# Yuer867/EMO-Disentanger

Measured on AMD Instinct MI355X. Metric: train tokens/sec (+ AR gen tokens/sec in "gen"), stage2 Performer d512 L12 seq2048, higher is better.
Workload: dtype bf16; 1 GPU; BASELINE configs[1]: stage2 Performer d_model=512 n_layer=12 n_head=8 favor_dims=128 seq=2048, B=64/GPU, dropout 0.1, omega redraw every_forward, fwd+bwd+allreduce+clip+Adam; global_batch=64, seq_len=2048, parallelism=dp1

## Files before the change

emo-disentanger_amd/_lib.py:

```python
import ctypes
import os

import torch

_HERE = os.path.dirname(os.path.abspath(__file__))
LIB_PATH = os.path.join(_HERE, 'libemo_hip.so')

F32, BF16, I64 = 0, 1, 2
ACT_NONE, ACT_RELU, ACT_GELU_NEW, ACT_GELU = 0, 1, 2, 3
MUL_NONE, MUL_NONZERO, MUL_DGELU_NEW, MUL_BITMASK, MUL_DGELU = 0, 1, 2, 3, 4

if not os.path.exists(LIB_PATH):
    raise ImportError('libemo_hip.so not built: run `python -c "import __graft_entry__ as g; g.build()"` '
                      'or `make -C emo-disentanger_amd/csrc` (hipcc --offload-arch=gfx950)')
lib = ctypes.CDLL(LIB_PATH)

c_p, c_i, c_l, c_f, c_u64 = ctypes.c_void_p, ctypes.c_int, ctypes.c_int64, ctypes.c_float, ctypes.c_uint64


class Epilogue(ctypes.Structure):
    _fields_ = [('bias', c_p), ('act', c_i), ('aux_out', c_p), ('mul_aux', c_p), ('mul_mode', c_i), ('mul_scale', c_f),
                ('p_drop', c_f), ('seed', c_u64), ('offset', c_u64), ('residual', c_p),
                ('ln_c1', c_p), ('ln_eps', c_f), ('ln_stats_out', c_p), ('rln_x', c_p), ('rln_stats', c_p), ('rln_gamma', c_p), ('rln_beta', c_p), ('a_rowsum', c_p), ('b_rowsum', c_p),
                ('mask_out', c_p), ('workspace', c_p), ('workspace_bytes', c_l),
                ('lna_gamma', c_p), ('lna_beta', c_p), ('lna_out', c_p), ('lna_mean', c_p), ('lna_rstd', c_p), ('hdiv', c_p), ('hdiv_T', c_l)]


_SIG = {
    'emo_version': (c_i, []),
    'emo_build_flags': (c_i, []),
    'emo_last_error': (ctypes.c_char_p, []),
    'emo_device_cus': (c_i, []),
    'emo_gemm': (c_i, [c_p, c_i, c_l, c_p, c_i, c_l, c_p, c_l, c_l, c_l, c_l, c_i, c_i, c_i, ctypes.POINTER(Epilogue), c_p]),
    'emo_gemm_last_kernel': (c_i, []),
    'emo_epilogue_size': (c_i, []),
    'emo_gemm_workspace_bytes': (c_l, [c_l, c_l, c_l, c_i, c_i]),
    'emo_ffn_fwd_supported': (c_i, [c_i, c_l, c_l, c_l]),
    'emo_ffn_fwd': (c_i, [c_p, c_p, c_p, c_f, c_p, c_p, c_p, c_p, c_p, c_p, c_p, c_p, c_p, c_p, c_l, c_l, c_l, c_i, c_f, c_u64, c_u64, c_u64, c_p]),
    'emo_colsum': (c_i, [c_p, c_i, c_l, c_l, c_l, c_p, c_i, c_p]),
    'emo_embed_fwd': (c_i, [c_p, c_p, c_p, c_p, c_p, c_p, c_i, c_l, c_l, c_l, c_l, c_l, c_l, c_p, c_f, c_f, c_u64, c_u64, c_p]),
    'emo_embed_bwd': (c_i, [c_p, c_p, c_p, c_i, c_p, c_p, c_l, c_l, c_l, c_l, c_l, c_f, c_f, c_u64, c_u64, c_p]),
    'emo_layernorm_fwd': (c_i, [c_p, c_p, c_p, c_p, c_p, c_p, c_i, c_l, c_l, c_f, c_p]),
    'emo_layernorm_bwd': (c_i, [c_p, c_p, c_p, c_p, c_p, c_p, c_p, c_p, c_p, c_p, c_p, c_i, c_l, c_l, c_f, c_u64, c_u64, c_p]),
    'emo_layernorm_bwd_workspace_bytes': (c_l, [c_i, c_l, c_l]),
    'emo_layernorm_bwd_ws': (c_i, [c_p, c_p, c_p, c_p, c_p, c_p, c_p, c_p, c_p, c_p, c_p, c_i, c_l, c_l, c_f, c_u64, c_u64, c_p, c_l, c_p]),
    'emo_dropout_apply': (c_i, [c_p, c_p, c_i, c_l, c_f, c_u64, c_u64, c_p]),
    'emo_favor_attn_workspace_bytes': (c_l, [c_l, c_l, c_l, c_l, c_l]),
    'emo_favor_attn_fwd': (c_i, [c_p, c_p, c_p, c_l, c_p, c_p, c_l, c_p, c_p, c_p, c_i, c_l, c_l, c_l, c_l, c_l, c_f, c_p, c_l, c_p]),
    'emo_favor_attn_bwd': (c_i, [c_p, c_p, c_p, c_l, c_p, c_p, c_p, c_l, c_p, c_p, c_p, c_p, c_l, c_i, c_l, c_l, c_l, c_l, c_l, c_f, c_p, c_l, c_p]),
    'emo_favor_attn_bwd_kstate': (c_i, [c_p, c_p, c_p, c_l, c_p, c_p, c_p, c_l, c_p, c_p, c_p, c_p, c_l, c_i, c_l, c_l, c_l, c_l, c_l, c_f, c_p, c_l, c_i, c_p]),
    'emo_favor_attn_bwd_dn_supported': (c_i, [c_i, c_l, c_l, c_l, c_l, c_l]),
    'emo_favor_attn_bwd_dn': (c_i, [c_p, c_p, c_p, c_l, c_p, c_p, c_p, c_l, c_p, c_p, c_p, c_l, c_i, c_l, c_l, c_l, c_l, c_l, c_f, c_p]),
    'emo_favor_decode_step': (c_i, [c_p, c_p, c_p, c_l, c_p, c_p, c_p, c_p, c_l, c_i, c_l, c_l, c_l, c_l, c_f, c_p]),
    'emo_performer_decode_step_workspace_bytes': (c_l, []),
    'emo_performer_decode_step_supported': (c_i, []),
    'emo_performer_decode_step': (c_i, [c_p, c_l, c_p, c_p, c_p, c_p, c_p, c_f, c_l, c_p, c_p, c_p, c_l, c_p, c_l, c_l, c_l, c_l, c_l, c_p, c_l, c_f, c_f, c_p, c_p]),
    'emo_performer_decode_step_sampled': (c_i, [c_p, c_l, c_p, c_p, c_p, c_p, c_f, c_l, c_p, c_p, c_l, c_p, c_l, c_l, c_l, c_l, c_l, c_l, c_p, c_l, c_f, c_f,
                                                c_f, c_f, c_p, c_p, c_p, c_l, c_l, c_p, c_p]),
    'emo_gpt2_decode_step_supported': (c_i, []),
    'emo_gpt2_decode_step': (c_i, [c_p, c_l, c_p, c_p, c_p, c_p, c_p, c_f, c_l, c_p, c_p, c_l, c_p, c_p, c_l, c_p, c_l, c_l, c_l, c_l, c_p, c_l, c_f, c_p, c_p]),
    'emo_gpt2_decode_step_sampled': (c_i, [c_p, c_l, c_p, c_p, c_p, c_p, c_f, c_l, c_p, c_l, c_p, c_p, c_l, c_p, c_l, c_l, c_l, c_l, c_l, c_p, c_l, c_f,
                                           c_f, c_f, c_p, c_p, c_p, c_l, c_l, c_p, c_p]),
    'emo_favor_draw_omega': (c_i, [c_p, c_p, c_l, c_l, c_l, c_p]),
    'emo_softmax_attn_fwd': (c_i, [c_p, c_p, c_p, c_l, c_p, c_l, c_p, c_i, c_l, c_l, c_l, c_l, c_f, c_u64, c_u64, c_p]),
    'emo_softmax_attn_bwd': (c_i, [c_p, c_p, c_p, c_l, c_p, c_p, c_l, c_p, c_p, c_p, c_p, c_p, c_l, c_i, c_l, c_l, c_l, c_l, c_f, c_u64, c_u64, c_p]),
    'emo_softmax_attn_keep_bytes': (c_l, [c_i, c_l, c_l, c_l, c_l, c_f]),
    'emo_softmax_attn_fwd_keep': (c_i, [c_p, c_p, c_p, c_l, c_p, c_l, c_p, c_i, c_l, c_l, c_l, c_l, c_f, c_u64, c_u64, c_p, c_l, c_p]),
    'emo_softmax_attn_bwd_keep': (c_i, [c_p, c_p, c_p, c_l, c_p, c_p, c_l, c_p, c_p, c_p, c_p, c_p, c_l, c_i, c_l, c_l, c_l, c_l, c_f, c_u64, c_u64, c_p, c_l, c_p]),
    'emo_relpos_attn_fwd': (c_i, [c_p, c_p, c_p, c_l, c_p, c_l, c_l, c_p, c_p, c_p, c_l, c_p, c_p, c_i, c_l, c_l, c_l, c_l, c_f, c_u64, c_u64, c_p]),
    'emo_relpos_attn_bwd_kv': (c_i, [c_p, c_p, c_l, c_p, c_p, c_l, c_p, c_l, c_l, c_p, c_l, c_p, c_p, c_p, c_p, c_p, c_l, c_i, c_l, c_l, c_l, c_l, c_f, c_u64, c_u64, c_p]),
    'emo_relpos_attn_bwd': (c_i, [c_p, c_p, c_p, c_l, c_p, c_l, c_l, c_p, c_p, c_p, c_p, c_l, c_p, c_p, c_p, c_l, c_p, c_l, c_p, c_i, c_l, c_l, c_l, c_l, c_f, c_u64, c_u64, c_p]),
    'emo_relpos_attn_bwd_r': (c_i, [c_p, c_p, c_l, c_p, c_p, c_l, c_p, c_l, c_l, c_p, c_l, c_p, c_p, c_p, c_p, c_l, c_p, c_l, c_i, c_l, c_l, c_l, c_l, c_f, c_u64, c_u64, c_p]),
    'emo_relpos_attn_bwd_r_workspace_bytes': (c_l, [c_l, c_l, c_l, c_l]),
    'emo_relpos_attn_decode': (c_i, [c_p, c_l, c_p, c_p, c_l, c_p, c_l, c_l, c_p, c_p, c_l, c_p, c_l, c_l, c_p, c_p, c_p, c_l, c_i, c_l, c_l, c_l, c_p]),
    'emo_softmax_attn_decode': (c_i, [c_p, c_l, c_p, c_p, c_l, c_p, c_l, c_p, c_p, c_l, c_p, c_l, c_i, c_l, c_l, c_l, c_p]),
    'emo_softmax_attn_decode_layout': (c_i, [c_p, c_l, c_p, c_p, c_l, c_p, c_l, c_p, c_p, c_l, c_p, c_l, c_i, c_l, c_l, c_l, c_i, c_p]),
    'emo_xent_fwd': (c_i, [c_p, c_p, c_l, c_l, c_l, c_p, c_p, c_p]),
    'emo_xent_bwd': (c_i, [c_p, c_p, c_p, c_p, c_p, c_l, c_i, c_l, c_l, c_l, c_p]),
    'emo_argmax': (c_i, [c_p, c_l, c_l, c_p, c_p]),
    'emo_sample_nucleus': (c_i, [c_p, c_l, c_l, c_f, c_f, c_p, c_p, c_p]),
    'emo_sample_nucleus_step': (c_i, [c_p, c_l, c_l, c_f, c_f, c_p, c_p, c_p, c_l, c_l, c_p, c_p]),
    'emo_txl_grammar_step': (c_i, [c_p, c_l, c_l, c_f, c_f, c_f, c_f, c_p, c_l, c_p, c_p, c_p, c_p, c_p, c_l, c_p, c_p, c_p]),
    'emo_acc_grammar_step': (c_i, [c_p, c_l, c_l, c_f, c_f, c_p, c_l, c_p, c_p, c_p, c_p, c_p, c_p, c_p, c_p, c_l, c_l, c_l, c_l, c_p, c_p, c_p, c_p]),
    'emo_accuracy_counts': (c_i, [c_p, c_p, c_p, c_p, c_l, c_l, c_l, c_p, c_p]),
    'emo_sumsq': (c_i, [c_p, c_l, c_p, c_p]),
    'emo_clip_coef': (c_i, [c_p, c_f, c_f, c_p, c_p, c_p]),
    'emo_adam_step': (c_i, [c_p, c_p, c_p, c_p, c_p, c_l, c_f, c_f, c_f, c_f, c_l, c_p, c_p]),
    'emo_cast': (c_i, [c_p, c_i, c_p, c_i, c_l, c_p]),
    'emo_add_bias2': (c_i, [c_p, c_l, c_p, c_p, c_p, c_p, c_i, c_l, c_l, c_p]),
    'emo_transpose_batch': (c_i, [c_p, c_i, c_l, c_p]),
    'emo_stream_wait': (c_i, [c_p, c_p]),
    'emo_comm_bind': (c_i, []),
    'emo_comm_unique_id': (c_i, [c_p]),
    'emo_comm_init': (c_i, [c_p, c_i, c_i]),
    'emo_comm_world': (c_i, []),
    'emo_comm_rank': (c_i, []),
    'emo_comm_allreduce': (c_i, [c_p, c_l, c_i, c_p]),
    'emo_comm_broadcast': (c_i, [c_p, c_l, c_i, c_i, c_p]),
    'emo_comm_destroy': (c_i, []),
}
for _name, (_res, _args) in _SIG.items():
    _fn = getattr(lib, _name)
    _fn.restype, _fn.argtypes = _res, _args
if lib.emo_epilogue_size() != ctypes.sizeof(Epilogue):
    raise ImportError('libemo_hip.so was built with an emo_epilogue_t of %d bytes, this binding has %d: rebuild (python -c "import __graft_entry__ as g; g.build()")'
                      % (lib.emo_epilogue_size(), ctypes.sizeof(Epilogue)))


class EmoError(RuntimeError):
    pass


def check(rc):
    if rc != 0:
        raise EmoError('libemo_hip error %d: %s' % (rc, lib.emo_last_error().decode()))


def dtype_code(t):
    if t == torch.float32:
        return F32
    if t == torch.bfloat16:
        return BF16
    raise EmoError('unsupported dtype %s (float32 / bfloat16 only)' % t)


def ptr(t):
    if t is None:
        return None
    if not t.is_cuda:
        raise EmoError('emo-disentanger_amd ops need GPU tensors (the HIP path has no CPU fallback)')
    return t.data_ptr()


def stream():
    return _raw_stream(_cur_device())


_raw_stream = getattr(torch._C, '_cuda_getCurrentRawStream', None)
_cur_device = getattr(torch._C, '_cuda_getDevice', None)
if _raw_stream is None or _cur_device is None:
    def stream():
        return torch.cuda.current_stream().cuda_stream
```

emo-disentanger_amd/csrc/emo_favor.hip:

```cpp
#include "emo_common.h"

#include "emo_lds_mma.h"

constexpr int FT = 512, FW = FT / 64;
#ifndef FAVOR_CFB
#define FAVOR_CFB 64
#endif
#ifndef FAVOR_CQB
#define FAVOR_CQB 64
#endif
#ifndef FAVOR_CKB
#define FAVOR_CKB 64
#endif
#ifndef FAVOR_PAD16
#define FAVOR_PAD16 0
#endif

template <typename CT, int DH, int C>
__device__ __forceinline__ void row_offsets(const CT* X, int ld, float* off, float c2, float half_ln_f, int tid) {
    constexpr int TPR = FT / C;
    constexpr int EPT = CMax<DH / TPR, 1>::v;
    const int r = tid / TPR, part = tid % TPR;
    float s = 0.f;
    if constexpr (sizeof(CT) == 2 && EPT == 8 && DH % 8 == 0) {
// ... 840 lines not shown
        }
        __syncthreads();
        zero_adiff_pad<CT, MF, MFP, C>(Adiff, LDM, tid);
        if (!(abl & 32)) {
            constexpr int NP = (MF / 16) * (C / 16);
            const int jt = wave % (C / 16);
            Frags<CT, CP> pmf;
            Frags<CT, DHP> vrf;
            pmf.load(PmT, LDC, jt * 16, lane);
            vrf.load(Vr, LDX, jt * 16, lane);
            _Pragma("unroll") for (int pr_i = 0; pr_i < (NP + FW - 1) / FW; ++pr_i) {
            const int pr = wave + FW * pr_i;
            if (NP % FW != 0 && pr >= NP) break;
                const int ft = pr / (C / 16);
                f32x4 aP = {0.f, 0.f, 0.f, 0.f}, aM = {0.f, 0.f, 0.f, 0.f};
                mm16_c<CT, CP>(aP, QfT, LDC, ft * 16, pmf, lane);
                mm16_c<CT, DHP>(aP, RF, LDX, ft * 16, vrf, lane);
                mm16_c<CT, CP>(aM, QfT, LDC, MF + ft * 16, pmf, lane);
                mm16_c<CT, DHP>(aM, RF, LDX, MF + ft * 16, vrf, lane);
                const int j = jt * 16 + (lane & 15), m0 = ft * 16 + (lane >> 4) * 4;
                jac_epilogue<CT, MF>(aP, aM, Kf, LDF, Adiff, LDM, sumA, rr, 1.f, j, m0, lane);
            }
        }
        if (!(abl & 2)) {
            constexpr int NT = (DH / 16) * (C / 16);
            const int jt = wave % (C / 16);
            Frags<CT, CP> amf;
            Frags<CT, F> kff;
            amf.load(AmT, LDC, jt * 16, lane);
            kff.load(Kf, LDF, jt * 16, lane);
            _Pragma("unroll") for (int tile_i = 0; tile_i < (NT + FW - 1) / FW; ++tile_i) {
            const int tile = wave + FW * tile_i;
            if (NT % FW != 0 && tile >= NT) break;
                const int dt = tile / (C / 16);
                f32x4 acc = {0.f, 0.f, 0.f, 0.f};
                mm16_c<CT, CP>(acc, GT, LDC, dt * 16, amf, lane);
                mm16_c<CT, F>(acc, RT, LDF, dt * 16, kff, lane);
                const int j = jt * 16 + (lane & 15), d0 = dt * 16 + (lane >> 4) * 4;
                if (j < valid) Img<CT>::store4(dvb + (t0 + j) * ld_d + d0, acc[0], acc[1], acc[2], acc[3]);
            }
        }
        __syncthreads();
        if (!(abl & 64)) dx_from_adiff<CT, DH, MFP, C>(W, LDM, Adiff, LDM, sumA, kb + t0 * ld, ld, dkb + t0 * ld_d, ld_d, cs, valid, wave, lane);
        }
        if (!(abl & 128)) {
        constexpr bool SH = FW % (F / 16) == 0;
        Frags<CT, CP> qtf;
        if constexpr (SH) qtf.load(QfT, LDC, (wave % (F / 16)) * 16, lane);
#pragma unroll
        for (int i = 0; i < NTS_W; ++i) {
            const int tile = wave + FW * i;
            if (tile < NTS) {
                const int dt = tile / (F / 16), ft = tile % (F / 16);
                if constexpr (SH) mm16_c<CT, CP>(racc[i], GT, LDC, dt * 16, qtf, lane);
                else mm16<CT, CP>(racc[i], GT, LDC, dt * 16, QfT, LDC, ft * 16, lane);
            }
        }
        }
        if constexpr (!SO) {
        __syncthreads();
#pragma unroll
        for (int i = 0; i < NTS_W; ++i) {
            const int tile = wave + FW * i;
            if (tile < NTS) {
                const int dt = tile / (F / 16), ft = tile % (F / 16);
                const int f = ft * 16 + (lane & 15), d0 = dt * 16 + (lane >> 4) * 4;
                Img<CT>::store4(RF + f * LDX + d0, racc[i][0], racc[i][1], racc[i][2], racc[i][3]);
#pragma unroll
                for (int r = 0; r < 4; ++r) RT[(d0 + r) * LDF + f] = from_f32<CT>(racc[i][r]);
            }
        }
        }
        if constexpr (sizeof(CT) == 2 && C == 64 && 4 * F <= FT) {
            const int f = tid >> 2, part = tid & 3;
            if (f < F) {
                float s = dot_contig<CT, 16>(QfT + f * LDC + part * 16, dD + part * 16);
                s += __shfl_xor(s, 1, 64);
                s += __shfl_xor(s, 2, 64);
                if (part == 0) rr[f] += s;
            }
        } else {
            for (int f = tid; f < F; f += FT) {
                float s = 0.f;
                for (int t = 0; t < C; ++t) s += to_f32<CT>(QfT[f * LDC + t]) * dD[t];
                rr[f] += s;
            }
        }
    }
    if constexpr (SO) {
        __syncthreads();
        float* Ro = R_ws + (bh * P + p_seg) * (int64_t)F * DH;
#pragma unroll
        for (int i = 0; i < NTS_W; ++i) {
            const int tile = wave + FW * i;
            if (tile < NTS) {
                const int dt = tile / (F / 16), ft = tile % (F / 16);
                const int f = ft * 16 + (lane & 15), d0 = dt * 16 + (lane >> 4) * 4;
                *(f32x4*)(Ro + f * DH + d0) = racc[i];
            }
        }
        for (int f = tid; f < F; f += FT) r_ws[(bh * P + p_seg) * (int64_t)F + f] = rr[f];
    }
}

template <typename CT>
__global__ __launch_bounds__(256) void favor_decode_kernel(const CT* __restrict__ q, const CT* __restrict__ k, const CT* __restrict__ v, int64_t ld,
                                                           const float* __restrict__ omega, float* __restrict__ state_S, float* __restrict__ state_z,
                                                           CT* __restrict__ out, int64_t ld_out, int64_t H, int dh, int mf, float eps) {
    __shared__ float xq[64], xk[64], xv[64], fq[128], fk[128], num[16][64], dpart[4];
    const int tid = threadIdx.x, F = 2 * mf;
    const int64_t sh = blockIdx.x, s = sh / H, h = sh % H;
    if (tid < dh) {
        xq[tid] = to_f32<CT>(q[s * ld + h * dh + tid]);
        xk[tid] = to_f32<CT>(k[s * ld + h * dh + tid]);
        xv[tid] = to_f32<CT>(v[s * ld + h * dh + tid]);
    }
    __syncthreads();
    const float cs = rsqrtf(sqrtf((float)dh)), half_ln_f = 0.5f * logf((float)F);
    float dn = 0.f;
    if (tid < F) {
        const int m = tid % mf;
        const float sgn = tid < mf ? 1.f : -1.f;
        float uq = 0.f, uk = 0.f, nq = 0.f, nk = 0.f;
        for (int d = 0; d < dh; ++d) {
            const float w = omega[d * mf + m];
            uq += xq[d] * w; uk += xk[d] * w;
            nq += xq[d] * xq[d]; nk += xk[d] * xk[d];
        }
        const float pq = __expf(sgn * cs * uq - (0.5f * cs * cs * nq + half_ln_f));
        const float pk = __expf(sgn * cs * uk - (0.5f * cs * cs * nk + half_ln_f));
        fq[tid] = pq;
        fk[tid] = pk;
        const float z = state_z[sh * F + tid] + pk;
        state_z[sh * F + tid] = z;
        dn = pq * z;
    }
    dn = wave_sum(dn);
    if ((tid & 63) == 0) dpart[tid >> 6] = dn;
    __syncthreads();
    const int G = 256 / dh, d = tid % dh, g = tid / dh;
    float acc = 0.f;
    float* Sb = state_S + sh * F * dh;
    const float vd = xv[d];
    for (int f = g; f < F; f += G) {
        const float sv = Sb[f * dh + d] + fk[f] * vd;
        Sb[f * dh + d] = sv;
        acc += fq[f] * sv;
    }
    num[g][d] = acc;
    __syncthreads();
    if (tid < dh) {
        float a = 0.f;
        for (int p = 0; p < G; ++p) a += num[p][tid];
        out[s * ld_out + h * dh + tid] = from_f32<CT>(a / (dpart[0] + dpart[1] + dpart[2] + dpart[3] + eps));
    }
}

template <typename CT, int DH, int MF>
__global__ __launch_bounds__(256) void favor_decode_fast_kernel(const CT* __restrict__ q, const CT* __restrict__ k, const CT* __restrict__ v, int64_t ld,
                                                                const float* __restrict__ omega, float* __restrict__ state_S,
                                                                float* __restrict__ state_z, CT* __restrict__ out, int64_t ld_out, int64_t H, float eps) {
    constexpr int F = 2 * MF, TPRW = DH / 4, R = 256 / TPRW, NP = (F + R - 1) / R;
    __shared__ float xq[DH], xk[DH], xv[DH], fq[F], fk[F], dpart[4];
    __shared__ f32x4 num[R][TPRW];
    const int tid = threadIdx.x;
    const int64_t sh = blockIdx.x, s = sh / H, h = sh % H;
    const int d4 = (tid % TPRW) * 4, g = tid / TPRW;
    float* Sb = state_S + sh * F * DH;
    f32x4 st[NP];
#pragma unroll
    for (int i = 0; i < NP; ++i) {
        const int f = g + R * i;
        st[i] = f < F ? *(const f32x4*)(Sb + f * DH + d4) : (f32x4){0.f, 0.f, 0.f, 0.f};
    }
    float wcol[DH], zold = 0.f;
    if (tid < F) {
#pragma unroll
        for (int d = 0; d < DH; ++d) wcol[d] = omega[d * MF + (tid % MF)];
        zold = state_z[sh * F + tid];
    }
    if (tid < DH) {
        xq[tid] = to_f32<CT>(q[s * ld + h * DH + tid]);
        xk[tid] = to_f32<CT>(k[s * ld + h * DH + tid]);
        xv[tid] = to_f32<CT>(v[s * ld + h * DH + tid]);
    }
    __syncthreads();
    const float cs = rsqrtf(sqrtf((float)DH)), half_ln_f = 0.5f * logf((float)F);
    float dn = 0.f;
    if (tid < F) {
        const float sgn = tid < MF ? 1.f : -1.f;
        float uq = 0.f, uk = 0.f, nq = 0.f, nk = 0.f;
#pragma unroll
        for (int d = 0; d < DH; ++d) {
            const float w = wcol[d];
            uq += xq[d] * w; uk += xk[d] * w;
            nq += xq[d] * xq[d]; nk += xk[d] * xk[d];
        }
        const float pq = __expf(sgn * cs * uq - (0.5f * cs * cs * nq + half_ln_f));
        const float pk = __expf(sgn * cs * uk - (0.5f * cs * cs * nk + half_ln_f));
        fq[tid] = pq;
        fk[tid] = pk;
        const float z = zold + pk;
        state_z[sh * F + tid] = z;
        dn = pq * z;
    }
    dn = wave_sum(dn);
    if ((tid & 63) == 0) dpart[tid >> 6] = dn;
    __syncthreads();
    const f32x4 vd = {xv[d4], xv[d4 + 1], xv[d4 + 2], xv[d4 + 3]};
    f32x4 acc = {0.f, 0.f, 0.f, 0.f};
#pragma unroll
    for (int i = 0; i < NP; ++i) {
        const int f = g + R * i;
        if (f < F) {
            const f32x4 sv = st[i] + fk[f] * vd;
            *(f32x4*)(Sb + f * DH + d4) = sv;
            acc += fq[f] * sv;
        }
    }
    num[g][tid % TPRW] = acc;
    __syncthreads();
    if (tid < DH) {
        float a = 0.f;
#pragma unroll
        for (int p = 0; p < R; ++p) a += num[p][tid >> 2][tid & 3];
        out[s * ld_out + h * DH + tid] = from_f32<CT>(a / (dpart[0] + dpart[1] + dpart[2] + dpart[3] + eps));
    }
}

__global__ __launch_bounds__(64) void favor_omega_kernel(const float* __restrict__ gauss, float* __restrict__ omega, int dh, int cols, int nblocks) {
    constexpr int LD = 68;
    __shared__ __attribute__((aligned(16))) float Qr[64 * LD];
    __shared__ __attribute__((aligned(16))) float Qc[64 * LD];
    __shared__ __attribute__((aligned(16))) float v[64], cf[64];
    const int lane = threadIdx.x;
    const int layer = blockIdx.x / nblocks, blk = blockIdx.x % nblocks;
    const float* G = gauss + (int64_t)blockIdx.x * dh * dh;
    for (int e = lane; e < 64 * LD; e += 64) { Qr[e] = 0.f; Qc[e] = 0.f; }
    float rn = 0.f;
    if (lane < dh)
        for (int b = 0; b < dh; ++b) { const float g = G[lane * dh + b]; rn += g * g; }
    rn = sqrtf(rn);
    const int start = blk * dh;
    const int ncol = (cols - start) < dh ? (cols - start) : dh;
    __syncthreads();
    for (int j = 0; j < ncol; ++j) {
        float x = lane < dh ? G[lane * dh + j] : 0.f;
        const int j4 = (j + 3) >> 2;
        for (int pass = 0; pass < 2; ++pass) {
            v[lane] = x;
            __syncthreads();
            f32x4 c4 = {0.f, 0.f, 0.f, 0.f};
#pragma unroll 4
            for (int a = 0; a < 16; ++a) c4 += *(const f32x4*)(Qc + lane * LD + 4 * a) * *(const f32x4*)(v + 4 * a);
            cf[lane] = (c4[0] + c4[1]) + (c4[2] + c4[3]);
            __syncthreads();
            f32x4 s4 = {0.f, 0.f, 0.f, 0.f};
            for (int i = 0; i < j4; ++i) s4 += *(const f32x4*)(cf + 4 * i) * *(const f32x4*)(Qr + lane * LD + 4 * i);
            x -= (s4[0] + s4[1]) + (s4[2] + s4[3]);
            __syncthreads();
        }
        const float nrm = sqrtf(wave_sum(lane < dh ? x * x : 0.f));
        const float qv = x / nrm;
        if (lane < dh) { Qr[lane * LD + j] = qv; Qc[j * LD + lane] = qv; }
        const float scale = __shfl(rn, j, 64);
        if (lane < dh) omega[((int64_t)layer * dh + lane) * cols + start + j] = qv * scale;
        __syncthreads();
    }
}

extern "C" int emo_favor_draw_omega(const float* gauss, float* omega, int64_t n_layers, int64_t dh, int64_t n_feat, emo_stream_t stream) {
    EMO_CHECK(gauss && omega && dh > 0 && dh <= 64 && n_feat % 2 == 0, "emo_favor_draw_omega: bad args (d_head <= 64)");
    const int cols = (int)(n_feat / 2);
    const int nblocks = (cols + (int)dh - 1) / (int)dh;
    hipLaunchKernelGGL(favor_omega_kernel, dim3((unsigned)(n_layers * nblocks)), dim3(64), 0, (hipStream_t)stream, gauss, omega, (int)dh, cols, nblocks);
    EMO_LAUNCH_CHECK();
    return EMO_OK;
}

template <typename CT, int DH, int MF, int C> static size_t fwd_lds() {
    typedef FavorDims<CT, DH, MF, C, 0> D;
    if (sizeof(CT) == 2 && C == 64)
        return sizeof(CT) * (size_t)(MF * D::LDX + C * CMax<D::LDX, D::LDC>::v + C * D::LDX + 2 * C * D::LDF + DH * D::LDF) + sizeof(float) * (size_t)(3 * C + D::F);
    return sizeof(CT) * (size_t)(MF * D::LDX + C * CMax<D::LDX, D::LDC>::v + C * D::LDX + DH * D::LDC + 2 * C * D::LDF + D::F * D::LDC + C * D::LDC + DH * D::LDF) +
           sizeof(float) * (size_t)(3 * C + D::F);
}
template <typename CT, int DH, int MF, int C> static size_t dq_lds() {
    typedef FavorDims<CT, DH, MF, C, 1> D;
    return sizeof(CT) * (size_t)(MF * D::LDX + DH * D::LDM + C * D::LDX + C * CMax<D::LDX, D::LDM>::v + C * D::LDX + DH * D::LDC + C * D::LDX +
                                 C * D::LDF + D::F * D::LDC + C * D::LDC + D::F * D::LDX) +
           sizeof(float) * (size_t)(4 * C + D::F);
}
template <typename CT, int DH, int MF, int C> static size_t dkv_lds() {
    typedef FavorDims<CT, DH, MF, C, 2> D;
    return sizeof(CT) * (size_t)(MF * D::LDX + DH * D::LDM + 2 * C * CMax<D::LDX, D::LDC>::v + C * D::LDX + C * CMax<D::LDX, D::LDM>::v + DH * D::LDC +
                                 2 * C * D::LDF + D::F * D::LDC + D::F * D::LDX + DH * D::LDF) +
           sizeof(float) * (size_t)(4 * C + D::F);
}

#define EMO_MAX_LDS (160 * 1024)

int emo_favor_fs_try(int which, int stage, const bf16_t* q, const bf16_t* k, const bf16_t* v, int64_t ld, const float* omega, bf16_t* out, int64_t ld_out,
                     float* den, float* sS, float* sz, const bf16_t* dout, bf16_t* dq, bf16_t* dk, bf16_t* dv, int64_t ld_d, int64_t B, int64_t T, int64_t H,
                     float eps, const float* ws_S, const float* ws_z, int P, int64_t Ts, hipStream_t st);

#define EMO_FAVOR_SEG_ALIGN 64
#define EMO_FAVOR_MAX_SEGMENTS 16
static void favor_segments(int64_t B, int64_t T, int64_t H, int* P_out, int64_t* Ts_out) {
    int64_t want = 1;
    const char* e = getenv("EMO_FAVOR_SEGMENTS");
    if (e && atoi(e) > 0) want = atoi(e);
    else if (B * H < 256) want = (256 + B * H - 1) / (B * H);
    if (want > EMO_FAVOR_MAX_SEGMENTS) want = EMO_FAVOR_MAX_SEGMENTS;
    const int64_t max_p = T / (2 * EMO_FAVOR_SEG_ALIGN);
    if (want > max_p) want = max_p;
    if (want < 1) want = 1;
    int64_t Ts = (T + want - 1) / want;
    Ts = (Ts + EMO_FAVOR_SEG_ALIGN - 1) / EMO_FAVOR_SEG_ALIGN * EMO_FAVOR_SEG_ALIGN;
    if (Ts < EMO_FAVOR_SEG_ALIGN) Ts = EMO_FAVOR_SEG_ALIGN;
    const int64_t P = T > 0 ? (T + Ts - 1) / Ts : 1;
    *P_out = (int)(P < 1 ? 1 : P);
    *Ts_out = Ts;
}

extern "C" int64_t emo_favor_attn_workspace_bytes(int64_t B, int64_t T, int64_t H, int64_t dh, int64_t n_feat) {
    int P; int64_t Ts;
    favor_segments(B, T, H, &P, &Ts);
    if (P <= 1) return 0;
    return B * H * P * (n_feat * dh + n_feat) * (int64_t)sizeof(float);
}

template <typename CT, int DH, int MF, int CF, int CQ, int CK>
static int run_favor(int which, const void* q, const void* k, const void* v, int64_t ld, const float* omega, void* out, int64_t ld_out, float* den,
                     float* sS, float* sz, const void* dout, void* dq, void* dk, void* dv, int64_t ld_d, int64_t B, int64_t T, int64_t H, float eps,
                     void* workspace, int64_t workspace_bytes, hipStream_t st, bool kstate_valid = false) {
    constexpr int F = 2 * MF;
    int P = 1; int64_t Ts = T > 0 ? T : 1;
    if (workspace) {
        favor_segments(B, T, H, &P, &Ts);
        const int64_t need = P > 1 ? B * H * P * (int64_t)(F * DH + F) * (int64_t)sizeof(float) : 0;
        EMO_CHECK(workspace_bytes >= need, "favor attention: workspace %lld B < %lld B (emo_favor_attn_workspace_bytes)", (long long)workspace_bytes,
                  (long long)need);
        EMO_CHECK(((uintptr_t)workspace & 15) == 0, "favor attention: workspace must be 16-B aligned");
    }
    if (P <= 1) { P = 1; Ts = T > 0 ? T : 1; }
    float* wsS = (float*)workspace;
    float* wsz = wsS ? wsS + B * H * P * (int64_t)F * DH : nullptr;
    dim3 grid((unsigned)(B * H * P));
    constexpr bool FS = sizeof(CT) == 2 && DH == 64 && MF == 64;
    auto fs_try = [&](int stage) -> bool {
        if constexpr (FS) {
            if (emo_favor_fs_try(which, stage, (const bf16_t*)q, (const bf16_t*)k, (const bf16_t*)v, ld, omega, (bf16_t*)out, ld_out, den, sS, sz, (const bf16_t*)dout,
                                 (bf16_t*)dq, (bf16_t*)dk, (bf16_t*)dv, ld_d, B, T, H, eps, wsS, wsz, P, Ts, st))
                return true;
        }
        const char* e = getenv("EMO_FAVOR_FS");
        if (e && atoi(e) == 2) emo_set_error("favor attention: EMO_FAVOR_FS=2 but the slice kernels do not cover this call");
        return false;
    };
    auto fs_required_failed = [&]() { const char* e = getenv("EMO_FAVOR_FS"); return e && atoi(e) == 2; };
    if (which == 0) {
        const size_t lds = fwd_lds<CT, DH, MF, CF>();
        EMO_CHECK(lds <= EMO_MAX_LDS, "favor fwd: LDS %zu too large", lds);
        auto kf = favor_fwd_kernel<CT, DH, MF, CF, false>;
        auto ks = favor_fwd_kernel<CT, DH, MF, CF, true>;
        static bool attr = false;
        if (!attr) {
            (void)hipFuncSetAttribute((const void*)kf, hipFuncAttributeMaxDynamicSharedMemorySize, (int)lds);
            (void)hipFuncSetAttribute((const void*)ks, hipFuncAttributeMaxDynamicSharedMemorySize, (int)lds);
            attr = true;
        }
        if (P > 1)
            hipLaunchKernelGGL(ks, grid, dim3(FT), lds, st, (const CT*)q, (const CT*)k, (const CT*)v, ld, omega, (CT*)out, ld_out, den, sS, sz, T, H, eps, wsS,
                               wsz, P, Ts);
        const char* ab = getenv("EMO_FAVOR_ABLATE");
        if (!fs_try(0)) {
            if (fs_required_failed()) return EMO_ERR_INVALID;
            hipLaunchKernelGGL(kf, grid, dim3(FT), lds, st, (const CT*)q, (const CT*)k, (const CT*)v, ld, omega, (CT*)out, ld_out, den, sS, sz, T, H, eps, wsS, wsz,
                               P | (ab ? atoi(ab) << 8 : 0), Ts);
        }
    } else {
        const size_t l0 = fwd_lds<CT, DH, MF, CF>(), l1 = dq_lds<CT, DH, MF, CQ>(), l2 = dkv_lds<CT, DH, MF, CK>();
        EMO_CHECK(l0 <= EMO_MAX_LDS && l1 <= EMO_MAX_LDS && l2 <= EMO_MAX_LDS, "favor bwd: LDS %zu / %zu / %zu too large", l0, l1, l2);
        auto k0 = favor_fwd_kernel<CT, DH, MF, CF, true>;
        auto k1 = favor_bwd_dq_kernel<CT, DH, MF, CQ>;
        auto k2 = favor_bwd_dkv_kernel<CT, DH, MF, CK, false>;
        auto k2s = favor_bwd_dkv_kernel<CT, DH, MF, CK, true>;
        static bool attr = false;
        if (!attr) {
            (void)hipFuncSetAttribute((const void*)k0, hipFuncAttributeMaxDynamicSharedMemorySize, (int)l0);
            (void)hipFuncSetAttribute((const void*)k1, hipFuncAttributeMaxDynamicSharedMemorySize, (int)l1);
            (void)hipFuncSetAttribute((const void*)k2, hipFuncAttributeMaxDynamicSharedMemorySize, (int)l2);
            (void)hipFuncSetAttribute((const void*)k2s, hipFuncAttributeMaxDynamicSharedMemorySize, (int)l2);
            attr = true;
        }
        if (den == nullptr) {
            EMO_CHECK(FS && P == 1, "emo_favor_attn_bwd_dn: needs bf16, d_head 64, 128 features and a single-segment scan (B * H >= 256): emo_favor_attn_bwd_dn_supported()");
            if (!fs_try(1) || !fs_try(2)) {
                emo_set_error("emo_favor_attn_bwd_dn: the slice kernels refused this call (T %% 32, 16-B alignment, EMO_FAVOR_FS / EMO_FAVOR_FS_BWD = 0)");
                return EMO_ERR_UNSUPPORTED;
            }
            EMO_LAUNCH_CHECK();
            return EMO_OK;
        }
        if (P > 1 && !kstate_valid)
            hipLaunchKernelGGL(k0, grid, dim3(FT), l0, st, (const CT*)q, (const CT*)k, (const CT*)v, ld, omega, (CT*)nullptr, ld_out, (float*)nullptr,
                               (float*)nullptr, (float*)nullptr, T, H, eps, wsS, wsz, P, Ts);
        if (!fs_try(1)) {
            if (fs_required_failed()) return EMO_ERR_INVALID;
            hipLaunchKernelGGL(k1, grid, dim3(FT), l1, st, (const CT*)q, (const CT*)k, (const CT*)v, ld, omega, (const CT*)out, (const CT*)dout, ld_out, den,
                               (CT*)dq, ld_d, T, H, (const float*)wsS, (const float*)wsz, P | (getenv("EMO_FAVOR_ABLATE_DQ") ? atoi(getenv("EMO_FAVOR_ABLATE_DQ")) << 8 : 0), Ts);
        }
        if (P > 1)
            hipLaunchKernelGGL(k2s, grid, dim3(FT), l2, st, (const CT*)q, (const CT*)k, (const CT*)v, ld, omega, (const CT*)out, (const CT*)dout, ld_out, den,
                               (CT*)dk, (CT*)dv, ld_d, T, H, wsS, wsz, P, Ts);
        if (!fs_try(2)) {
            if (fs_required_failed()) return EMO_ERR_INVALID;
            hipLaunchKernelGGL(k2, grid, dim3(FT), l2, st, (const CT*)q, (const CT*)k, (const CT*)v, ld, omega, (const CT*)out, (const CT*)dout, ld_out, den,
                               (CT*)dk, (CT*)dv, ld_d, T, H, wsS, wsz, P | (getenv("EMO_FAVOR_ABLATE_DKV") ? atoi(getenv("EMO_FAVOR_ABLATE_DKV")) << 8 : 0), Ts);
        }
    }
    EMO_LAUNCH_CHECK();
    return EMO_OK;
}

static int dispatch_favor(int which, int dtype, int64_t dh, int64_t mf, const void* q, const void* k, const void* v, int64_t ld, const float* omega,
                          void* out, int64_t ld_out, float* den, float* sS, float* sz, const void* dout, void* dq, void* dk, void* dv, int64_t ld_d,
                          int64_t B, int64_t T, int64_t H, float eps, void* ws, int64_t ws_bytes, hipStream_t st, bool kstate_valid = false) {
#define FAVOR_CASE(DHv, MFv, CFb, CQb, CKb, CFf, CQf, CKf)                                                                                   \
    if (dh == DHv && mf == MFv) {                                                                                                            \
        if (dtype == EMO_BF16)                                                                                                               \
            return run_favor<bf16_t, DHv, MFv, CFb, CQb, CKb>(which, q, k, v, ld, omega, out, ld_out, den, sS, sz, dout, dq, dk, dv, ld_d, B, T, H, eps, ws, \
                                                              ws_bytes, st, kstate_valid);                                                   \
        return run_favor<float, DHv, MFv, CFf, CQf, CKf>(which, q, k, v, ld, omega, out, ld_out, den, sS, sz, dout, dq, dk, dv, ld_d, B, T, H, eps, ws,      \
                                                         ws_bytes, st, kstate_valid);                                                        \
    }
    FAVOR_CASE(64, 64, FAVOR_CFB, FAVOR_CQB, FAVOR_CKB, 32, 32, 16)
    FAVOR_CASE(32, 64, 64, 64, 64, 32, 32, 32)
    FAVOR_CASE(32, 32, 64, 64, 64, 32, 32, 32)
    FAVOR_CASE(16, 16, 64, 64, 64, 32, 32, 32)
    FAVOR_CASE(16, 32, 64, 64, 64, 32, 32, 32)
#undef FAVOR_CASE
    emo_set_error("favor attention: unsupported (d_head=%lld, n_feat=%lld); built: (64,128) (32,128) (32,64) (16,32) (16,64)", (long long)dh,
                  (long long)(2 * mf));
    return EMO_ERR_UNSUPPORTED;
}

static int favor_check(const void* q, const void* k, const void* v, int64_t ld, int64_t ld_out, int dtype, int64_t dh, int64_t n_feat) {
    EMO_CHECK(q && k && v, "favor attention: null pointer");
    EMO_CHECK(dtype == EMO_F32 || dtype == EMO_BF16, "favor attention: bad dtype");
    const int64_t ve = dtype == EMO_BF16 ? 8 : 4;
    EMO_CHECK(ld % ve == 0 && ld_out % 4 == 0 && dh % ve == 0, "favor attention: ld/dh must keep rows 16-B aligned");
    EMO_CHECK(((uintptr_t)q & 15) == 0 && ((uintptr_t)k & 15) == 0 && ((uintptr_t)v & 15) == 0, "favor attention: q/k/v must be 16-B aligned");
    EMO_CHECK(n_feat % 2 == 0, "favor attention: n_feat must be even");
    return EMO_OK;
}

extern "C" int emo_favor_attn_fwd(const void* q, const void* k, const void* v, int64_t ld, const float* omega, void* out, int64_t ld_out, float* den,
                                  float* state_S, float* state_z, int dtype, int64_t B, int64_t T, int64_t H, int64_t dh, int64_t n_feat, float eps,
                                  void* workspace, int64_t workspace_bytes, emo_stream_t stream) {
    int rc = favor_check(q, k, v, ld, ld_out, dtype, dh, n_feat);
    if (rc) return rc;
    EMO_CHECK(omega && out && den, "emo_favor_attn_fwd: null pointer");
    EMO_CHECK(((uintptr_t)out & 15) == 0, "emo_favor_attn_fwd: out must be 16-B aligned");
    EMO_CHECK(!(state_S && !state_z), "emo_favor_attn_fwd: state_S without state_z");
    return dispatch_favor(0, dtype, dh, n_feat / 2, q, k, v, ld, omega, out, ld_out, den, state_S, state_z, nullptr, nullptr, nullptr, nullptr, 0, B, T, H,
                          eps, workspace, workspace_bytes, (hipStream_t)stream);
}

extern "C" int emo_favor_attn_bwd_kstate(const void* q, const void* k, const void* v, int64_t ld, const float* omega, const void* out, const void* dout,
                                         int64_t ld_out, const float* den, void* dq, void* dk, void* dv, int64_t ld_d, int dtype, int64_t B, int64_t T, int64_t H,
                                         int64_t dh, int64_t n_feat, float eps, void* workspace, int64_t workspace_bytes, int kstate_valid, emo_stream_t stream) {
    int rc = favor_check(q, k, v, ld, ld_out, dtype, dh, n_feat);
    if (rc) return rc;
    EMO_CHECK(omega && out && dout && den && dq && dk && dv, "emo_favor_attn_bwd: null pointer");
    EMO_CHECK(ld_d % 4 == 0, "emo_favor_attn_bwd: ld_d must be a multiple of 4");
    EMO_CHECK((((uintptr_t)dq | (uintptr_t)dk | (uintptr_t)dv | (uintptr_t)out | (uintptr_t)dout) & 15) == 0, "emo_favor_attn_bwd: pointers must be 16-B aligned");
    return dispatch_favor(1, dtype, dh, n_feat / 2, q, k, v, ld, omega, (void*)out, ld_out, (float*)den, nullptr, nullptr, dout, dq, dk, dv, ld_d, B, T, H,
                          eps, workspace, workspace_bytes, (hipStream_t)stream, kstate_valid != 0 && workspace != nullptr);
}
extern "C" int emo_favor_attn_bwd_dn_supported(int dtype, int64_t B, int64_t T, int64_t H, int64_t dh, int64_t n_feat) {
    if (dtype != EMO_BF16 || dh != 64 || n_feat != 128 || T < 32 || (T % 32) != 0 || B * H <= 0) return 0;
    const char* e = getenv("EMO_FAVOR_FS");
    const char* e2 = getenv("EMO_FAVOR_FS_BWD");
    if ((e && atoi(e) == 0) || (e2 && atoi(e2) == 0)) return 0;
    int P; int64_t Ts;
    favor_segments(B, T, H, &P, &Ts);
    return P <= 1 ? 1 : 0;
}
extern "C" int emo_favor_attn_bwd_dn(const void* q, const void* k, const void* v, int64_t ld, const float* omega, const void* out, const void* dn,
                                     int64_t ld_out, void* dq, void* dk, void* dv, int64_t ld_d, int dtype, int64_t B, int64_t T, int64_t H,
                                     int64_t dh, int64_t n_feat, float eps, emo_stream_t stream) {
    int rc = favor_check(q, k, v, ld, ld_out, dtype, dh, n_feat);
    if (rc) return rc;
    EMO_CHECK(omega && out && dn && dq && dk && dv, "emo_favor_attn_bwd_dn: null pointer");
    EMO_CHECK(emo_favor_attn_bwd_dn_supported(dtype, B, T, H, dh, n_feat), "emo_favor_attn_bwd_dn: problem not in the supported class (emo_favor_attn_bwd_dn_supported)");
    EMO_CHECK(ld_d % 4 == 0, "emo_favor_attn_bwd_dn: ld_d must be a multiple of 4");
    EMO_CHECK((((uintptr_t)dq | (uintptr_t)dk | (uintptr_t)dv | (uintptr_t)out | (uintptr_t)dn) & 15) == 0, "emo_favor_attn_bwd_dn: pointers must be 16-B aligned");
    return dispatch_favor(1, dtype, dh, n_feat / 2, q, k, v, ld, omega, (void*)out, ld_out, (float*)nullptr, nullptr, nullptr, dn, dq, dk, dv, ld_d, B, T, H,
                          eps, nullptr, 0, (hipStream_t)stream, false);
}
extern "C" int emo_favor_attn_bwd(const void* q, const void* k, const void* v, int64_t ld, const float* omega, const void* out, const void* dout,
                                  int64_t ld_out, const float* den, void* dq, void* dk, void* dv, int64_t ld_d, int dtype, int64_t B, int64_t T, int64_t H,
                                  int64_t dh, int64_t n_feat, float eps, void* workspace, int64_t workspace_bytes, emo_stream_t stream) {
    return emo_favor_attn_bwd_kstate(q, k, v, ld, omega, out, dout, ld_out, den, dq, dk, dv, ld_d, dtype, B, T, H, dh, n_feat, eps, workspace, workspace_bytes, 0, stream);
}

extern "C" int emo_favor_decode_step(const void* q, const void* k, const void* v, int64_t ld, const float* omega, float* state_S, float* state_z, void* out,
                                     int64_t ld_out, int dtype, int64_t n_streams, int64_t H, int64_t dh, int64_t n_feat, float eps, emo_stream_t stream) {
    EMO_CHECK(q && k && v && omega && state_S && state_z && out, "emo_favor_decode_step: null pointer");
    EMO_CHECK(dh <= 64 && dh >= 16 && 256 % dh == 0 && n_feat <= 128 && n_feat % 2 == 0, "emo_favor_decode_step: needs 16<=d_head<=64 dividing 256, n_feat<=128");
    dim3 grid((unsigned)(n_streams * H));
    hipStream_t st = (hipStream_t)stream;
#define DECODE_LAUNCH(CTv, DHv, MFv)                                                                                                            \
    hipLaunchKernelGGL((favor_decode_fast_kernel<CTv, DHv, MFv>), grid, dim3(256), 0, st, (const CTv*)q, (const CTv*)k, (const CTv*)v, ld, omega,             \
                       state_S, state_z, (CTv*)out, ld_out, H, eps)
#define DECODE_CASE(DHv, MFv)                                                                                                                   \
    if (dh == DHv && n_feat == 2 * MFv) {                                                                                                       \
        if (dtype == EMO_F32) DECODE_LAUNCH(float, DHv, MFv); else DECODE_LAUNCH(bf16_t, DHv, MFv);                                             \
        EMO_LAUNCH_CHECK();                                                                                                                     \
        return EMO_OK;                                                                                                                          \
    }
    if (getenv("EMO_FAVOR_DECODE_GENERIC") == nullptr && (((uintptr_t)state_S) & 15) == 0) {
        DECODE_CASE(64, 64)
        DECODE_CASE(32, 64)
        DECODE_CASE(32, 32)
        DECODE_CASE(16, 16)
        DECODE_CASE(16, 32)
    }
#undef DECODE_CASE
#undef DECODE_LAUNCH
    if (dtype == EMO_F32)
        hipLaunchKernelGGL(favor_decode_kernel<float>, grid, dim3(256), 0, st, (const float*)q, (const float*)k, (const float*)v, ld, omega, state_S, state_z,
                           (float*)out, ld_out, H, (int)dh, (int)(n_feat / 2), eps);
    else
        hipLaunchKernelGGL(favor_decode_kernel<bf16_t>, grid, dim3(256), 0, st, (const bf16_t*)q, (const bf16_t*)k, (const bf16_t*)v, ld, omega, state_S,
                           state_z, (bf16_t*)out, ld_out, H, (int)dh, (int)(n_feat / 2), eps);
    EMO_LAUNCH_CHECK();
    return EMO_OK;
}
```

emo-disentanger_amd/csrc/emo_favor_fs.hip:

```cpp
#include "emo_common.h"

#include "emo_lds_mma.h"

#ifdef EMO_DIAG
__device__ unsigned long long emo_fs_diag[64];
extern "C" int emo_diag_fetch(unsigned long long* host, int n, int reset) {
    if (hipMemcpyFromSymbol(host, HIP_SYMBOL(emo_fs_diag), sizeof(unsigned long long) * n) != hipSuccess) return -1;
    if (reset) { unsigned long long z[64] = {}; (void)hipMemcpyToSymbol(HIP_SYMBOL(emo_fs_diag), z, sizeof(z)); }
    return 0;
}
#define FSD_BEGIN uint64_t tc_[16] = {}, ts_ = __builtin_readcyclecounter(), tstart_ = ts_;
#define FSD(k) do { const uint64_t tn_ = __builtin_readcyclecounter(); tc_[k] += tn_ - ts_; ts_ = tn_; } while (0)
#define FSD_END(base, nk) do { if (lane == 0) { for (int k_ = 0; k_ < nk; ++k_) atomicAdd(&emo_fs_diag[base + k_], (unsigned long long)tc_[k_]); \
    atomicAdd(&emo_fs_diag[base + 14], (unsigned long long)(__builtin_readcyclecounter() - tstart_)); atomicAdd(&emo_fs_diag[base + 15], 1ull); } } while (0)
#else
#define FSD_BEGIN
#define FSD(k) do {} while (0)
#define FSD_END(base, nk) do {} while (0)
#endif

namespace {
constexpr int FS_NT = 256;
constexpr int FS_C = 32;
constexpr int FS_LDF = 136;
// ... 88 lines not shown
    for (int h = 0; h < 2; ++h) {
        const int row = h * 16 + kc * 4 + (i >> 2), col = col0 + (i & 3) * 4;
        const char* p = tile + row * FS_ROWB + ((((col >> 3)) ^ fs_sw(row)) << 4) + (col & 7) * 2;
        const short4v t = __builtin_amdgcn_ds_read_tr16_b64_v4i16((__attribute__((address_space(3))) short4v*)p);
        const bf16x4 tb = __builtin_bit_cast(bf16x4, t);
        v[h * 4 + 0] = tb[0]; v[h * 4 + 1] = tb[1]; v[h * 4 + 2] = tb[2]; v[h * 4 + 3] = tb[3];
    }
    return v;
}
__device__ __forceinline__ uint32_t fs_lds_addr(const void* p) { return (uint32_t)(uintptr_t)(const __attribute__((address_space(3))) char*)p; }

typedef uint32_t u32x2 __attribute__((ext_vector_type(2)));
__device__ __forceinline__ u32x2 fs_rd8(uint32_t addr, int off) {
    u32x2 r;
    asm volatile("ds_read_b64 %0, %1 offset:%2" : "=v"(r) : "v"(addr), "i"(off));
    return r;
}
__device__ __forceinline__ bf16x8 fs_join(u32x2 lo, u32x2 hi) { return __builtin_bit_cast(bf16x8, (u32x4){lo[0], lo[1], hi[0], hi[1]}); }
template <int N> __device__ __forceinline__ void fs_pin(bf16x8& a, bf16x8& b, bf16x8& c, bf16x8& d) {
    static_assert(N == 0 || N == 4 || N == 8 || N == 12 || N >= 15, "");
    if constexpr (N == 0) asm volatile("s_waitcnt lgkmcnt(0)" : "+v"(a), "+v"(b), "+v"(c), "+v"(d));
    else if constexpr (N == 4) asm volatile("s_waitcnt lgkmcnt(4)" : "+v"(a), "+v"(b), "+v"(c), "+v"(d));
    else if constexpr (N == 8) asm volatile("s_waitcnt lgkmcnt(8)" : "+v"(a), "+v"(b), "+v"(c), "+v"(d));
    else if constexpr (N == 12) asm volatile("s_waitcnt lgkmcnt(12)" : "+v"(a), "+v"(b), "+v"(c), "+v"(d));
    else asm volatile("s_waitcnt lgkmcnt(15)" : "+v"(a), "+v"(b), "+v"(c), "+v"(d));
}
__device__ __forceinline__ uint32_t fs_lp_lane(int g, int c) { return (uint32_t)((c * FS_LDF + 4 * g) * 2); }
__device__ __forceinline__ bf16x8 fs_lp_asm(uint32_t base, int img_off, int row0, int step) {
    const int o = img_off + (row0 * FS_LDF + 32 * step) * 2;
    return fs_join(fs_rd8(base, o), fs_rd8(base, o + 32));
}
__device__ __forceinline__ void fs_rp_lane(int g, int c, uint32_t (&l)[2][2]) {
    const int P = (g >> 1) ^ fs_sw(c);
#pragma unroll
    for (int s_ = 0; s_ < 2; ++s_)
#pragma unroll
        for (int h = 0; h < 2; ++h) l[s_][h] = (uint32_t)(c * FS_ROWB + (g & 1) * 8 + ((P ^ (4 * s_ + 2 * h)) << 4));
}
__device__ __forceinline__ bf16x8 fs_rp_asm(const uint32_t (&rp)[2][2], int tensor, int row0, int s_) {
    const int o = tensor * FS_TILEB + row0 * FS_ROWB;
    return fs_join(fs_rd8(rp[s_][0], o), fs_rd8(rp[s_][1], o));
}

__global__ __launch_bounds__(FS_NT, 2) void favor_fs_fwd_kernel(const bf16_t* __restrict__ q, const bf16_t* __restrict__ k, const bf16_t* __restrict__ v,
                                                                int64_t ld, const float* __restrict__ omega, bf16_t* __restrict__ out, int64_t ld_out,
                                                                float* __restrict__ den_g, float* __restrict__ state_S, float* __restrict__ state_z,
                                                                int64_t Tfull, int64_t H, float eps, const float* __restrict__ S_ws,
                                                                const float* __restrict__ z_ws, int P, int64_t Ts) {
    extern __shared__ __attribute__((aligned(16))) char smem[];
    char* QKr = smem;
    char* Vr = QKr + 3 * 2 * FS_TILEB;
    bf16_t* QFb = (bf16_t*)(Vr + 4 * FS_TILEB);
    bf16_t* KFb = QFb + 2 * FS_C * FS_LDF;
    const int tid = threadIdx.x, lane = tid & 63, g = lane >> 4, c = lane & 15;
    const int w = __builtin_amdgcn_readfirstlane(tid >> 6);
    const int64_t bh = blockIdx.x / P, b = bh / H, h = bh % H;
    const int p_seg = (int)(blockIdx.x % P);
    const int64_t tbeg = (int64_t)p_seg * Ts, T = (tbeg + Ts < Tfull) ? Ts : Tfull - tbeg;
    const bf16_t* qb = q + (b * Tfull + tbeg) * ld + h * 64;
    const bf16_t* kb = k + (b * Tfull + tbeg) * ld + h * 64;
    const bf16_t* vb = v + (b * Tfull + tbeg) * ld + h * 64;
    bf16_t* ob = out + (b * Tfull + tbeg) * ld_out + h * 64;
    float* dg = den_g + bh * Tfull + tbeg;
    const float cs = rsqrtf(sqrtf(64.f));
    const float cs2 = cs * FS_LOG2E, c2h = 0.5f * cs * cs * FS_LOG2E, hl = 0.5f * logf(128.f) * FS_LOG2E;

    bf16x8 wop[2];
#pragma unroll
    for (int s = 0; s < 2; ++s)
#pragma unroll
        for (int e = 0; e < 8; ++e) wop[s][e] = (bf16_t)omega[(32 * s + 8 * g + e) * 64 + 16 * w + c];
    bf16x8 oneop;
#pragma unroll
    for (int e = 0; e < 8; ++e) oneop[e] = (bf16_t)(c == 0 ? 1.f : 0.f);

    f32x4 S[8][2];
#pragma unroll
    for (int ft = 0; ft < 8; ++ft) { S[ft][0] = zero4(); S[ft][1] = zero4(); }
    for (int pp = 0; pp < p_seg; ++pp) {
        const float* Sp = S_ws + (bh * P + pp) * (int64_t)(128 * 64);
        const float* zp = z_ws + (bh * P + pp) * (int64_t)128;
        float ts[8][4];
        f32x4 tz[8];
#pragma unroll
        for (int ft = 0; ft < 8; ++ft) {
#pragma unroll
            for (int r = 0; r < 4; ++r) ts[ft][r] = Sp[(16 * ft + 4 * g + r) * 64 + 16 * w + c];
            tz[ft] = *(const f32x4*)(zp + 16 * ft + 4 * g);
        }
        const float zm = c == 0 ? 1.f : 0.f;
#pragma unroll
        for (int ft = 0; ft < 8; ++ft)
#pragma unroll
            for (int r = 0; r < 4; ++r) { S[ft][0][r] += ts[ft][r]; S[ft][1][r] += zm * tz[ft][r]; }
    }

    const int nch = (int)(T / FS_C);
    const uint32_t qk_lds = __builtin_amdgcn_readfirstlane(fs_lds_addr(QKr)), vr_lds = __builtin_amdgcn_readfirstlane(fs_lds_addr(Vr));
    const int64_t src_off = (int64_t)(8 * w + (lane >> 3)) * ld + (((lane & 7) ^ fs_sw(8 * w + (lane >> 3))) << 3);
    auto issue = [&](int n) {
        const int64_t o = (int64_t)n * FS_C * ld + src_off;
        const uint32_t qk = qk_lds + (n % 3) * 2 * FS_TILEB + w * 1024;
        fs_dma16(qb + o, qk);
        fs_dma16(kb + o, qk + FS_TILEB);
        fs_dma16(vb + o, vr_lds + (n & 3) * FS_TILEB + w * 1024);
    };
    issue(0);
    if (nch > 1) issue(1);
    if (nch > 2) issue(2);
    if (nch > 2) fs_wait<6>(); else if (nch > 1) fs_wait<3>(); else fs_wait<0>();
    __builtin_amdgcn_s_barrier();
    asm volatile("" ::: "memory");
    bf16x4 o_prev[2] = {};
    float d_prev[2] = {0.f, 0.f};
    const uint32_t lpb0 = fs_lds_addr(QFb) + fs_lp_lane(g, c);
    constexpr int KFO = 2 * FS_C * FS_LDF * 2;
#ifdef EMO_DIAG
    uint64_t tc[8] = {}, ts = __builtin_readcyclecounter(), tstart = ts;
#define FS_STAMP(k) do { const uint64_t tn_ = __builtin_readcyclecounter(); tc[k] += tn_ - ts; ts = tn_; } while (0)
#else
#define FS_STAMP(k) do {} while (0)
#endif
    for (int i = 0; i < nch; ++i) {
        const int64_t t0 = (int64_t)i * FS_C;
        bf16_t* QF = QFb + (i & 1) * FS_C * FS_LDF;
        bf16_t* KF = KFb + (i & 1) * FS_C * FS_LDF;
        const char* Xq = QKr + (i % 3) * 2 * FS_TILEB;
        const char* Xk = Xq + FS_TILEB;
        const char* VB = Vr + (i & 3) * FS_TILEB;
        {
            bf16x8 x[4][2];
#pragma unroll
            for (int j = 0; j < 4; ++j)
#pragma unroll
                for (int s = 0; s < 2; ++s) x[j][s] = fs_ring_frag(j < 2 ? Xq : Xk, 16 * (j & 1), s, g, c);
            float p[4][4], n[4][4];
            fs_features<4>(wop, x, cs2, c2h, hl, g, c, p, n);
#pragma unroll
            for (int j = 0; j < 4; ++j) {
                bf16_t* dst = (j < 2 ? QF : KF) + (16 * (j & 1) + c) * FS_LDF + 16 * w + 4 * g;
                st4(dst, p[j][0], p[j][1], p[j][2], p[j][3]);
                st4(dst + 64, n[j][0], n[j][1], n[j][2], n[j][3]);
            }
        }
        FS_STAMP(0);
        if (i + 2 < nch) fs_wait<3>(); else fs_wait<0>();
        FS_STAMP(1);
        if (i > 0) {
#pragma unroll
            for (int tt = 0; tt < 2; ++tt) {
                *(bf16x4*)(ob + (t0 - FS_C + 16 * tt + c) * ld_out + 16 * w + 4 * g) = o_prev[tt];
                if (w == 0 && g == 0) dg[t0 - FS_C + 16 * tt + c] = d_prev[tt];
            }
        }
        fs_barrier();
        FS_STAMP(2);
        if (i + 3 < nch) issue(i + 3);
#ifdef EMO_DIAG
        FS_STAMP(6);
#endif
        bf16x8 qf[2][4], kf[2][4];
        const uint32_t lpb = lpb0 + (i & 1) * (FS_C * FS_LDF * 2);
#pragma unroll
        for (int hs = 0; hs < 2; ++hs)
#pragma unroll
            for (int u = 0; u < 2; ++u)
#pragma unroll
                for (int tt = 0; tt < 2; ++tt) { qf[tt][2 * hs + u] = fs_lp_asm(lpb, 0, 16 * tt, 2 * hs + u); kf[tt][2 * hs + u] = fs_lp_asm(lpb, KFO, 16 * tt, 2 * hs + u); }
        const bf16x8 vop = fs_ring_perm_tr(VB, 16 * w, lane);
        fs_pin<24>(qf[0][0], kf[0][0], qf[1][0], kf[1][0]);
        fs_pin<16>(qf[0][1], kf[0][1], qf[1][1], kf[1][1]);
#ifdef EMO_DIAG
        asm volatile("s_waitcnt lgkmcnt(0)" ::: "memory");
        asm volatile("" :: "v"(vop), "v"(qf[0][0]), "v"(qf[1][3]), "v"(kf[0][0]), "v"(kf[1][3]));
        FS_STAMP(7);
#endif
        f32x4 aa[3][2];
#pragma unroll
        for (int u = 0; u < 2; ++u) {
            aa[0][u] = mma32(kf[0][u], qf[0][u], zero4());
            aa[1][u] = mma32(kf[0][u], qf[1][u], zero4());
            aa[2][u] = mma32(kf[1][u], qf[1][u], zero4());
        }
        fs_pin<8>(qf[0][2], kf[0][2], qf[1][2], kf[1][2]);
        fs_pin<0>(qf[0][3], kf[0][3], qf[1][3], kf[1][3]);
#pragma unroll
        for (int u = 0; u < 2; ++u) {
            aa[0][u] = mma32(kf[0][2 + u], qf[0][2 + u], aa[0][u]);
            aa[1][u] = mma32(kf[0][2 + u], qf[1][2 + u], aa[1][u]);
            aa[2][u] = mma32(kf[1][2 + u], qf[1][2 + u], aa[2][u]);
        }
        f32x4 a00 = aa[0][0] + aa[0][1], a11 = aa[2][0] + aa[2][1];
        const f32x4 a01 = aa[1][0] + aa[1][1];
#pragma unroll
        for (int r = 0; r < 4; ++r) {
            const bool keep = (4 * g + r) <= c;
            a00[r] = keep ? a00[r] : 0.f;
            a11[r] = keep ? a11[r] : 0.f;
        }
        bf16x8 at[2];
        at[0] = pack8(a00, zero4());
        at[1] = pack8(a01, a11);
#ifdef EMO_DIAG
        asm volatile("" :: "v"(at[0]), "v"(at[1]));
#endif
        FS_STAMP(3);
        f32x4 nm[2][2];
#pragma unroll
        for (int tt = 0; tt < 2; ++tt) { nm[tt][0] = mma32(vop, at[tt], zero4()); nm[tt][1] = mma32(oneop, at[tt], zero4()); }
#pragma unroll
        for (int s = 0; s < 4; ++s) {
            const bf16x8 s0 = pack8(S[2 * s][0], S[2 * s + 1][0]), s1 = pack8(S[2 * s][1], S[2 * s + 1][1]);
#pragma unroll
            for (int tt = 0; tt < 2; ++tt) { nm[tt][0] = mma32(s0, qf[tt][s], nm[tt][0]); nm[tt][1] = mma32(s1, qf[tt][s], nm[tt][1]); }
        }
#pragma unroll
        for (int tt = 0; tt < 2; ++tt) {
            const float dn = __shfl(nm[tt][1][0], c, 64) + eps;
            const float inv = 1.f / dn;
            o_prev[tt] = (bf16x4){(bf16_t)(nm[tt][0][0] * inv), (bf16_t)(nm[tt][0][1] * inv), (bf16_t)(nm[tt][0][2] * inv), (bf16_t)(nm[tt][0][3] * inv)};
            d_prev[tt] = dn;
        }
#ifdef EMO_DIAG
        asm volatile("" :: "v"(o_prev[0]), "v"(o_prev[1]));
#endif
        FS_STAMP(4);
#pragma unroll
        for (int ft = 0; ft < 8; ++ft) {
            const bf16x8 kT = load_perm_tr(KF, FS_LDF, 16 * ft, 0, lane);
            S[ft][0] = mma32(kT, vop, S[ft][0]);
            S[ft][1] = mma32(kT, oneop, S[ft][1]);
        }
#ifdef EMO_DIAG
        asm volatile("" :: "v"(S[0][0]), "v"(S[7][1]), "v"(S[3][0]), "v"(S[5][1]));
#endif
        FS_STAMP(5);
    }
#ifdef EMO_DIAG
    if (state_S && lane == 0) {
        unsigned long long* dgp = (unsigned long long*)state_S;
        for (int k_ = 0; k_ < 8; ++k_) atomicAdd(dgp + k_, (unsigned long long)tc[k_]);
        atomicAdd(dgp + 8, (unsigned long long)(__builtin_readcyclecounter() - tstart));
        atomicAdd(dgp + 9, 1ull);
    }
    if (state_S) return;
#endif
    {
        const int64_t t0 = (int64_t)nch * FS_C;
#pragma unroll
        for (int tt = 0; tt < 2; ++tt) {
            *(bf16x4*)(ob + (t0 - FS_C + 16 * tt + c) * ld_out + 16 * w + 4 * g) = o_prev[tt];
            if (w == 0 && g == 0) dg[t0 - FS_C + 16 * tt + c] = d_prev[tt];
        }
    }
    if (state_S && p_seg == P - 1) {
        float* So = state_S + bh * (int64_t)(128 * 64);
#pragma unroll
        for (int ft = 0; ft < 8; ++ft)
#pragma unroll
            for (int r = 0; r < 4; ++r) So[(16 * ft + 4 * g + r) * 64 + 16 * w + c] = S[ft][0][r];
        if (w == 0 && c == 0) {
            float* zo = state_z + bh * 128;
#pragma unroll
            for (int ft = 0; ft < 8; ++ft)
#pragma unroll
                for (int r = 0; r < 4; ++r) zo[16 * ft + 4 * g + r] = S[ft][1][r];
        }
    }
}

constexpr int FS_SLOTB = 5 * FS_TILEB;
template <> __device__ __forceinline__ void fs_wait<12>() { asm volatile("s_waitcnt vmcnt(12)" ::: "memory"); }
__device__ __forceinline__ void fs_dma4(const void* gsrc, uint32_t lds_dst) {
    uint32_t keep;
    asm volatile("s_mov_b32 %0, m0\n\ts_mov_b32 m0, %2\n\ts_nop 0\n\tglobal_load_lds_dword %1, off\n\ts_mov_b32 m0, %0"
                 : "=&s"(keep) : "v"(gsrc), "s"(lds_dst) : "memory");
}
__device__ __forceinline__ f32x4 mma16(bf16x4 a, bf16x4 b, f32x4 c) {
    return __builtin_amdgcn_mfma_f32_16x16x16bf16_1k(__builtin_bit_cast(short4v, a), __builtin_bit_cast(short4v, b), c, 0, 0, 0);
}
__device__ __forceinline__ bf16x8 fs_ring_perm(const char* tile, int row0, int s, int g, int c) {
    const int row = row0 + c, ch = 4 * s + (g >> 1), sw = fs_sw(row);
    const char* base = tile + fs_opaque(row0 * FS_ROWB) + c * FS_ROWB + (g & 1) * 8;
    const bf16x4 lo = *(const bf16x4*)(base + ((ch ^ sw) << 4)), hi = *(const bf16x4*)(base + (((ch + 2) ^ sw) << 4));
    return (bf16x8){lo[0], lo[1], lo[2], lo[3], hi[0], hi[1], hi[2], hi[3]};
}
__device__ __forceinline__ float fs_diag_sum_rows(const f32x4& gm, int g, int c) {
    const int r = c & 3;
    const float d = r == 0 ? gm[0] : r == 1 ? gm[1] : r == 2 ? gm[2] : gm[3];
    return fs_sum_rows(g == (c >> 2) ? d : 0.f);
}
__device__ __forceinline__ bf16x8 fs_scale8(const bf16x8& x, float a) {
    bf16x8 r;
#pragma unroll
    for (int e = 0; e < 8; ++e) r[e] = (bf16_t)((float)x[e] * a);
    return r;
}

template <bool PRE>
__global__ __launch_bounds__(FS_NT, 2) void favor_fs_dq_kernel(const bf16_t* __restrict__ q, const bf16_t* __restrict__ k, const bf16_t* __restrict__ v,
                                                               int64_t ld, const float* __restrict__ omega, const bf16_t* __restrict__ out,
                                                               const bf16_t* __restrict__ dout, int64_t ld_out, const float* __restrict__ den_g,
                                                               bf16_t* __restrict__ dq, int64_t ld_d, int64_t Tfull, int64_t H,
                                                               const float* __restrict__ S_ws, const float* __restrict__ z_ws, int P, int64_t Ts) {
    extern __shared__ __attribute__((aligned(16))) char smem[];
    char* RING = smem;
    char* DEN = RING + 3 * FS_SLOTB;
    char* KP = DEN + 3 * 256;
    char* DU = KP + 4 * 2048;
    float* SA = (float*)(DU + 2 * FS_TILEB);
    const int tid = threadIdx.x, lane = tid & 63, g = lane >> 4, c = lane & 15;
    const int w = __builtin_amdgcn_readfirstlane(tid >> 6);
    const int64_t bh = blockIdx.x / P, b = bh / H, h = bh % H;
    const int p_seg = (int)(blockIdx.x % P);
    const int64_t tbeg = (int64_t)p_seg * Ts, T = (tbeg + Ts < Tfull) ? Ts : Tfull - tbeg;
    const bf16_t* qb = q + (b * Tfull + tbeg) * ld + h * 64;
    const bf16_t* kb = k + (b * Tfull + tbeg) * ld + h * 64;
    const bf16_t* vb = v + (b * Tfull + tbeg) * ld + h * 64;
    const bf16_t* ob = out + (b * Tfull + tbeg) * ld_out + h * 64;
    const bf16_t* gb = dout + (b * Tfull + tbeg) * ld_out + h * 64;
    bf16_t* dqb = dq + (b * Tfull + tbeg) * ld_d + h * 64;
    const float* dnb = den_g + bh * Tfull + tbeg;
    const float cs = rsqrtf(sqrtf(64.f));
    const float cs2 = cs * FS_LOG2E, c2h = 0.5f * cs * cs * FS_LOG2E, hl = 0.5f * logf(128.f) * FS_LOG2E;

    bf16x8 wop[2], wrow[2];
#pragma unroll
    for (int s = 0; s < 2; ++s)
#pragma unroll
        for (int e = 0; e < 8; ++e) {
            wop[s][e] = (bf16_t)omega[(32 * s + 8 * g + e) * 64 + 16 * w + c];
            wrow[s][e] = (bf16_t)omega[(16 * w + c) * 64 + 32 * s + 8 * g + e];
        }
    bf16x8 oneop;
#pragma unroll
    for (int e = 0; e < 8; ++e) oneop[e] = (bf16_t)(c == 0 ? 1.f : 0.f);

    f32x4 ST[5][2];
#pragma unroll
    for (int dl = 0; dl < 5; ++dl) { ST[dl][0] = zero4(); ST[dl][1] = zero4(); }
    for (int pp = 0; pp < p_seg; ++pp) {
        const float* Sp = S_ws + (bh * P + pp) * (int64_t)(128 * 64);
        const float* zp = z_ws + (bh * P + pp) * (int64_t)128;
        f32x4 t4[2][4];
        float tz[2];
#pragma unroll
        for (int ph = 0; ph < 2; ++ph) {
            const int f = 64 * ph + 16 * w + c;
#pragma unroll
            for (int dl = 0; dl < 4; ++dl) t4[ph][dl] = *(const f32x4*)(Sp + f * 64 + 16 * dl + 4 * g);
            tz[ph] = zp[f];
        }
        const float gm = g == 0 ? 1.f : 0.f;
#pragma unroll
        for (int ph = 0; ph < 2; ++ph) {
#pragma unroll
            for (int dl = 0; dl < 4; ++dl) ST[dl][ph] += t4[ph][dl];
            ST[4][ph][0] += gm * tz[ph];
        }
    }

    const int nch = (int)(T / FS_C);
    const uint32_t ring_lds = __builtin_amdgcn_readfirstlane(fs_lds_addr(RING)), den_lds = __builtin_amdgcn_readfirstlane(fs_lds_addr(DEN));
    const int srow = 8 * w + (lane >> 3), spc = ((lane & 7) ^ fs_sw(srow)) << 3;
    const int64_t so_qkv = (int64_t)srow * ld + spc, so_o = (int64_t)srow * ld_out + spc;
    auto issue_part = [&](int n, int part) {
        if (n >= nch) return;
        const int64_t t0n = (int64_t)n * FS_C;
        const uint32_t dst = ring_lds + (n % 3) * FS_SLOTB + w * 1024;
        if (part == 0) fs_dma16(qb + t0n * ld + so_qkv, dst);
        else if (part == 1) fs_dma16(kb + t0n * ld + so_qkv, dst + FS_TILEB);
        else if (part == 2) fs_dma16(vb + t0n * ld + so_qkv, dst + 2 * FS_TILEB);
        else if (part == 3) fs_dma16(gb + t0n * ld_out + so_o, dst + 3 * FS_TILEB);
        else if (part == 4) fs_dma16(ob + t0n * ld_out + so_o, dst + 4 * FS_TILEB);
        else if (!PRE) {
            const int64_t tl = t0n + lane;
            fs_dma4(dnb + (tl < T ? tl : T - 1), den_lds + (n % 3) * 256);
        }
    };
    constexpr int NPART = PRE ? 5 : 6;
    auto issue = [&](int n) {
#pragma unroll
        for (int part = 0; part < 6; ++part) issue_part(n, part);
    };
    issue(0);
    if (nch > 1) issue(1);
    if (nch > 2) issue(2);
    if (nch > 2) fs_wait<2 * NPART>(); else if (nch > 1) fs_wait<NPART>(); else fs_wait<0>();
    __builtin_amdgcn_s_barrier();
    asm volatile("" ::: "memory");
    char* KPw = KP + w * 2048;
    bf16x4 o_prev[2] = {};
    uint32_t rpl[2][2];
    fs_rp_lane(g, c, rpl);
    FSD_BEGIN
    for (int i = 0; i < nch; ++i) {
        const int64_t t0 = (int64_t)i * FS_C;
        const char* Xq = RING + (i % 3) * FS_SLOTB;
        const char* Xk = Xq + FS_TILEB;
        const char* Xv = Xq + 2 * FS_TILEB;
        const char* Xg = Xq + 3 * FS_TILEB;
        const char* Xo = Xq + 4 * FS_TILEB;
        const float* dens = (const float*)(DEN + (i % 3) * 256);
        char* DUb = DU + (i & 1) * FS_TILEB;
        float* SAb = SA + (i & 1) * 128;
        bf16x8 dfr[2][2], ofr[2][2], vr[2][2];
        f32x4 gmm[2];
        uint32_t rp[2][2];
        {
            const uint32_t slot = ring_lds + (i % 3) * FS_SLOTB;
#pragma unroll
            for (int s_ = 0; s_ < 2; ++s_)
#pragma unroll
                for (int h_ = 0; h_ < 2; ++h_) rp[s_][h_] = rpl[s_][h_] + slot;
        }
#pragma unroll
        for (int tt = 0; tt < 2; ++tt)
#pragma unroll
            for (int s_ = 0; s_ < 2; ++s_) { dfr[tt][s_] = fs_rp_asm(rp, 3, 16 * tt, s_); ofr[tt][s_] = fs_rp_asm(rp, 4, 16 * tt, s_); }
#pragma unroll
        for (int jt = 0; jt < 2; ++jt)
#pragma unroll
            for (int s_ = 0; s_ < 2; ++s_) vr[jt][s_] = fs_rp_asm(rp, 2, 16 * jt, s_);
        fs_pin<16>(dfr[0][0], ofr[0][0], dfr[0][1], ofr[0][1]);
        fs_pin<8>(dfr[1][0], ofr[1][0], dfr[1][1], ofr[1][1]);
#pragma unroll
        for (int tt = 0; tt < 2; ++tt) {
            gmm[tt] = mma32(ofr[tt][0], dfr[tt][0], zero4());
            gmm[tt] = mma32(ofr[tt][1], dfr[tt][1], gmm[tt]);
        }
        float pq[2][4], nq[2][4];
        {
            bf16x8 x[4][2];
#pragma unroll
            for (int j = 0; j < 4; ++j)
#pragma unroll
                for (int s = 0; s < 2; ++s) x[j][s] = fs_ring_frag(j < 2 ? Xq : Xk, 16 * (j & 1), s, g, c);
            float p[4][4], n[4][4];
            fs_features<4>(wop, x, cs2, c2h, hl, g, c, p, n);
#pragma unroll
            for (int tt = 0; tt < 2; ++tt)
#pragma unroll
                for (int r = 0; r < 4; ++r) { pq[tt][r] = p[tt][r]; nq[tt][r] = n[tt][r]; }
#pragma unroll
            for (int jt = 0; jt < 2; ++jt) {
                const int row = 16 * jt + c, sw = ((row >> 2) & 1) << 2;
                st4((bf16_t*)(KPw + row * 64 + ((g ^ sw) << 3)), p[2 + jt][0], p[2 + jt][1], p[2 + jt][2], p[2 + jt][3]);
                st4((bf16_t*)(KPw + row * 64 + (((4 + g) ^ sw) << 3)), n[2 + jt][0], n[2 + jt][1], n[2 + jt][2], n[2 + jt][3]);
            }
        }
        FSD(0);
        if (i > 0) issue_part(i + 2, 3);
        bf16x4 xown[2];
#pragma unroll
        for (int tt = 0; tt < 2; ++tt) {
            const int row = 16 * tt + c;
            xown[tt] = *(const bf16x4*)(Xq + row * FS_ROWB + (((2 * w + (g >> 1)) ^ fs_sw(row)) << 4) + (g & 1) * 8);
        }
        bf16x8 gop[2][2];
        float dD[2];
#pragma unroll
        for (int tt = 0; tt < 2; ++tt) {
            if constexpr (PRE) {
                dD[tt] = -fs_diag_sum_rows(gmm[tt], g, c);
                gop[tt][0] = dfr[tt][0];
                gop[tt][1] = dfr[tt][1];
            } else {
                const float inv = 1.f / dens[16 * tt + c];
                dD[tt] = -fs_diag_sum_rows(gmm[tt], g, c) * inv;
                gop[tt][0] = fs_scale8(dfr[tt][0], inv);
                gop[tt][1] = fs_scale8(dfr[tt][1], inv);
            }
        }
        FSD(1);
        if (i > 0) issue_part(i + 2, 4);
        bf16x8 at[2];
        {
            fs_pin<0>(vr[0][0], vr[0][1], vr[1][0], vr[1][1]);
            f32x4 p00 = mma32(vr[0][0], gop[0][0], zero4()), p01 = mma32(vr[0][0], gop[1][0], zero4()), p11 = mma32(vr[1][0], gop[1][0], zero4());
            p00 = mma32(vr[0][1], gop[0][1], p00);
            p01 = mma32(vr[0][1], gop[1][1], p01);
            p11 = mma32(vr[1][1], gop[1][1], p11);
#pragma unroll
            for (int r = 0; r < 4; ++r) {
                const bool keep = (4 * g + r) <= c;
                p00[r] = keep ? p00[r] + dD[0] : 0.f;
                p01[r] = p01[r] + dD[1];
                p11[r] = keep ? p11[r] + dD[1] : 0.f;
            }
            at[0] = pack8(p00, zero4());
            at[1] = pack8(p01, p11);
        }
        FSD(2);
        if (i > 0) issue_part(i + 2, 5);
        bf16x8 kfT[2];
#pragma unroll
        for (int ph = 0; ph < 2; ++ph) {
#pragma unroll
            for (int hh = 0; hh < 2; ++hh) {
                const int row = hh * 16 + g * 4 + (c >> 2), pc = (4 * ph + (c & 3)) ^ (((row >> 2) & 1) << 2);
                const short4v t = __builtin_amdgcn_ds_read_tr16_b64_v4i16((__attribute__((address_space(3))) short4v*)(KPw + row * 64 + (pc << 3)));
                const bf16x4 tb = __builtin_bit_cast(bf16x4, t);
                kfT[ph][hh * 4 + 0] = tb[0]; kfT[ph][hh * 4 + 1] = tb[1]; kfT[ph][hh * 4 + 2] = tb[2]; kfT[ph][hh * 4 + 3] = tb[3];
            }
        }
        {
            bf16x8 sop[2][2];
            bf16x4 szop[2];
#pragma unroll
            for (int ph = 0; ph < 2; ++ph) {
                sop[ph][0] = pack8(ST[0][ph], ST[1][ph]);
                sop[ph][1] = pack8(ST[2][ph], ST[3][ph]);
                szop[ph] = (bf16x4){(bf16_t)ST[4][ph][0], (bf16_t)ST[4][ph][1], (bf16_t)ST[4][ph][2], (bf16_t)ST[4][ph][3]};
            }
            f32x4 dph[2][2];
#pragma unroll
            for (int tt = 0; tt < 2; ++tt) {
                const bf16x4 ddop = {(bf16_t)(g == 0 ? dD[tt] : 0.f), (bf16_t)0.f, (bf16_t)0.f, (bf16_t)0.f};
#pragma unroll
                for (int ph = 0; ph < 2; ++ph) {
                    f32x4 a = mma32(kfT[ph], at[tt], zero4());
                    a = mma32(sop[ph][0], gop[tt][0], a);
                    a = mma32(sop[ph][1], gop[tt][1], a);
                    dph[ph][tt] = mma16(szop[ph], ddop, a);
                }
            }
#pragma unroll
            for (int tt = 0; tt < 2; ++tt) {
                float du[4], sa = 0.f;
#pragma unroll
                for (int r = 0; r < 4; ++r) {
                    const float ap = dph[0][tt][r] * pq[tt][r], am = dph[1][tt][r] * nq[tt][r];
                    du[r] = ap - am;
                    sa += ap + am;
                }
                sa = fs_sum_rows(sa);
                const int row = 16 * tt + c;
                st4((bf16_t*)(DUb + row * FS_ROWB + (((2 * w + (g >> 1)) ^ fs_sw(row)) << 4) + (g & 1) * 8), du[0], du[1], du[2], du[3]);
                if (g == 0) SAb[w * 32 + row] = sa;
            }
        }
        FSD(3);
#pragma unroll
        for (int dl = 0; dl < 4; ++dl) {
            const bf16x8 vT = fs_ring_perm_tr(Xv, 16 * dl, lane);
            ST[dl][0] = mma32(vT, kfT[0], ST[dl][0]);
            ST[dl][1] = mma32(vT, kfT[1], ST[dl][1]);
        }
        ST[4][0] = mma32(oneop, kfT[0], ST[4][0]);
        ST[4][1] = mma32(oneop, kfT[1], ST[4][1]);
        FSD(4);
        if (i + 2 < nch) fs_wait<NPART>(); else fs_wait<0>();
        FSD(5);
        if (i > 0) {
#pragma unroll
            for (int tt = 0; tt < 2; ++tt) *(bf16x4*)(dqb + (t0 - FS_C + 16 * tt + c) * ld_d + 16 * w + 4 * g) = o_prev[tt];
        }
        fs_barrier();
        FSD(6);
        issue_part(i + 3, 0);
        FSD(7);
#pragma unroll
        for (int tt = 0; tt < 2; ++tt) {
            issue_part(i + 3, 1 + tt);
            const int row = 16 * tt + c;
            const bf16x8 u0 = *(const bf16x8*)(DUb + row * FS_ROWB + (((g) ^ fs_sw(row)) << 4)), u1 = *(const bf16x8*)(DUb + row * FS_ROWB + (((4 + g) ^ fs_sw(row)) << 4));
            f32x4 dx = mma32(wrow[0], u0, zero4());
            dx = mma32(wrow[1], u1, dx);
            const float sa = (SAb[row] + SAb[32 + row]) + (SAb[64 + row] + SAb[96 + row]);
            float o[4];
#pragma unroll
            for (int r = 0; r < 4; ++r) o[r] = cs * (dx[r] - cs * (float)xown[tt][r] * sa);
            o_prev[tt] = (bf16x4){(bf16_t)o[0], (bf16_t)o[1], (bf16_t)o[2], (bf16_t)o[3]};
        }
        FSD(8);
    }
    FSD_END(16, 9);
    {
        const int64_t t0 = (int64_t)nch * FS_C;
#pragma unroll
        for (int tt = 0; tt < 2; ++tt) *(bf16x4*)(dqb + (t0 - FS_C + 16 * tt + c) * ld_d + 16 * w + 4 * g) = o_prev[tt];
    }
}

template <bool PRE>
__global__ __launch_bounds__(FS_NT, 2) void favor_fs_dkv_kernel(const bf16_t* __restrict__ q, const bf16_t* __restrict__ k, const bf16_t* __restrict__ v,
                                                                int64_t ld, const float* __restrict__ omega, const bf16_t* __restrict__ out,
                                                                const bf16_t* __restrict__ dout, int64_t ld_out, const float* __restrict__ den_g,
                                                                bf16_t* __restrict__ dk, bf16_t* __restrict__ dv, int64_t ld_d, int64_t Tfull, int64_t H,
                                                                const float* __restrict__ R_ws, const float* __restrict__ r_ws, int P, int64_t Ts) {
    extern __shared__ __attribute__((aligned(16))) char smem[];
    char* RING = smem;
    char* DEN = RING + 2 * FS_SLOTB;
    bf16_t* QF = (bf16_t*)(DEN + 2 * 256);
    bf16_t* KF = QF + FS_C * FS_LDF;
    char* DU = (char*)(KF + FS_C * FS_LDF);
    float* SA = (float*)(DU + FS_TILEB);
    float* PV = SA + 128;
    const int tid = threadIdx.x, lane = tid & 63, g = lane >> 4, c = lane & 15;
    const int w = __builtin_amdgcn_readfirstlane(tid >> 6);
    const int64_t bh = blockIdx.x / P, b = bh / H, h = bh % H;
    const int p_seg = (int)(blockIdx.x % P);
    const int64_t tbeg = (int64_t)p_seg * Ts, T = (tbeg + Ts < Tfull) ? Ts : Tfull - tbeg;
    const bf16_t* qb = q + (b * Tfull + tbeg) * ld + h * 64;
    const bf16_t* kb = k + (b * Tfull + tbeg) * ld + h * 64;
    const bf16_t* vb = v + (b * Tfull + tbeg) * ld + h * 64;
    const bf16_t* ob = out + (b * Tfull + tbeg) * ld_out + h * 64;
    const bf16_t* gb = dout + (b * Tfull + tbeg) * ld_out + h * 64;
    bf16_t* dkb = dk + (b * Tfull + tbeg) * ld_d + h * 64;
    bf16_t* dvb = dv + (b * Tfull + tbeg) * ld_d + h * 64;
    const float* dnb = den_g + bh * Tfull + tbeg;
    const float cs = rsqrtf(sqrtf(64.f));
    const float cs2 = cs * FS_LOG2E, c2h = 0.5f * cs * cs * FS_LOG2E, hl = 0.5f * logf(128.f) * FS_LOG2E;

    bf16x8 wop[2], wrow[2];
#pragma unroll
    for (int s = 0; s < 2; ++s)
#pragma unroll
        for (int e = 0; e < 8; ++e) {
            wop[s][e] = (bf16_t)omega[(32 * s + 8 * g + e) * 64 + 16 * w + c];
            wrow[s][e] = (bf16_t)omega[(16 * w + c) * 64 + 32 * s + 8 * g + e];
        }
    const bf16x4 onecol = {(bf16_t)(g == 0 ? 1.f : 0.f), (bf16_t)0.f, (bf16_t)0.f, (bf16_t)0.f};

    f32x4 RT[5][2], RD[8];
#pragma unroll
    for (int dl = 0; dl < 5; ++dl) { RT[dl][0] = zero4(); RT[dl][1] = zero4(); }
#pragma unroll
    for (int ft = 0; ft < 8; ++ft) RD[ft] = zero4();
    for (int pp = p_seg + 1; pp < P; ++pp) {
        const float* Rp = R_ws + (bh * P + pp) * (int64_t)(128 * 64);
        const float* rp = r_ws + (bh * P + pp) * (int64_t)128;
        f32x4 t4[2][4];
        float tr[2], td[8][4];
#pragma unroll
        for (int ph = 0; ph < 2; ++ph) {
            const int f = 64 * ph + 16 * w + c;
#pragma unroll
            for (int dl = 0; dl < 4; ++dl) t4[ph][dl] = *(const f32x4*)(Rp + f * 64 + 16 * dl + 4 * g);
            tr[ph] = rp[f];
        }
#pragma unroll
        for (int ft = 0; ft < 8; ++ft)
#pragma unroll
            for (int r = 0; r < 4; ++r) td[ft][r] = Rp[(16 * ft + 4 * g + r) * 64 + 16 * w + c];
        const float gm = g == 0 ? 1.f : 0.f;
#pragma unroll
        for (int ph = 0; ph < 2; ++ph) {
#pragma unroll
            for (int dl = 0; dl < 4; ++dl) RT[dl][ph] += t4[ph][dl];
            RT[4][ph][0] += gm * tr[ph];
        }
#pragma unroll
        for (int ft = 0; ft < 8; ++ft)
#pragma unroll
            for (int r = 0; r < 4; ++r) RD[ft][r] += td[ft][r];
    }

    const int nch = (int)(T / FS_C);
    const uint32_t ring_lds = __builtin_amdgcn_readfirstlane(fs_lds_addr(RING)), den_lds = __builtin_amdgcn_readfirstlane(fs_lds_addr(DEN));
    const int srow = 8 * w + (lane >> 3), spc = ((lane & 7) ^ fs_sw(srow)) << 3;
    const int64_t so_qkv = (int64_t)srow * ld + spc, so_o = (int64_t)srow * ld_out + spc;
    auto issue = [&](int n) {
        const int64_t t0n = (int64_t)(nch - 1 - n) * FS_C;
        const uint32_t dst = ring_lds + (n & 1) * FS_SLOTB + w * 1024;
        fs_dma16(qb + t0n * ld + so_qkv, dst);
        fs_dma16(kb + t0n * ld + so_qkv, dst + FS_TILEB);
        fs_dma16(vb + t0n * ld + so_qkv, dst + 2 * FS_TILEB);
        fs_dma16(gb + t0n * ld_out + so_o, dst + 3 * FS_TILEB);
        fs_dma16(ob + t0n * ld_out + so_o, dst + 4 * FS_TILEB);
        if constexpr (!PRE) {
            const int64_t tl = t0n + lane;
            fs_dma4(dnb + (tl < T ? tl : T - 1), den_lds + (n & 1) * 256);
        }
    };
    issue(0);
    if (nch > 1) issue(1);
    if (nch > 1) fs_wait<PRE ? 5 : 6>(); else fs_wait<0>();
    __builtin_amdgcn_s_barrier();
    asm volatile("" ::: "memory");
    float* PVw = PV + w * 96;
    bf16x4 dk_prev[2] = {}, dv_prev[2] = {};
    uint32_t rpl[2][2];
    fs_rp_lane(g, c, rpl);
    const uint32_t lpb = fs_lds_addr(QF) + fs_lp_lane(g, c);
    constexpr int KFO = FS_C * FS_LDF * 2;
    FSD_BEGIN
    for (int n = 0; n < nch; ++n) {
        const int64_t t0 = (int64_t)(nch - 1 - n) * FS_C;
        const char* Xq = RING + (n & 1) * FS_SLOTB;
        const char* Xk = Xq + FS_TILEB;
        const char* Xv = Xq + 2 * FS_TILEB;
        const char* Xg = Xq + 3 * FS_TILEB;
        const char* Xo = Xq + 4 * FS_TILEB;
        const float* dens = (const float*)(DEN + (n & 1) * 256);
        {
            bf16x8 x[4][2];
#pragma unroll
            for (int j = 0; j < 4; ++j)
#pragma unroll
                for (int s = 0; s < 2; ++s) x[j][s] = fs_ring_frag(j < 2 ? Xq : Xk, 16 * (j & 1), s, g, c);
            float p[4][4], nn[4][4];
            fs_features<4>(wop, x, cs2, c2h, hl, g, c, p, nn);
#pragma unroll
            for (int j = 0; j < 4; ++j) {
                bf16_t* dst = (j < 2 ? QF : KF) + (16 * (j & 1) + c) * FS_LDF + 16 * w + 4 * g;
                st4(dst, p[j][0], p[j][1], p[j][2], p[j][3]);
                st4(dst + 64, nn[j][0], nn[j][1], nn[j][2], nn[j][3]);
            }
        }
        FSD(0);
        bf16x4 xown[2];
#pragma unroll
        for (int jt = 0; jt < 2; ++jt) {
            const int row = 16 * jt + c;
            xown[jt] = *(const bf16x4*)(Xk + row * FS_ROWB + (((2 * w + (g >> 1)) ^ fs_sw(row)) << 4) + (g & 1) * 8);
        }
        bf16x8 gA[2][2];
        uint32_t rp[2][2];
        {
            const uint32_t slot = ring_lds + (n & 1) * FS_SLOTB;
#pragma unroll
            for (int s_ = 0; s_ < 2; ++s_)
#pragma unroll
                for (int h_ = 0; h_ < 2; ++h_) rp[s_][h_] = rpl[s_][h_] + slot;
        }
        bf16x8 dfr[2][2], ofr[2][2], vB1[2][2];
#pragma unroll
        for (int tt = 0; tt < 2; ++tt)
#pragma unroll
            for (int s_ = 0; s_ < 2; ++s_) { dfr[tt][s_] = fs_rp_asm(rp, 3, 16 * tt, s_); ofr[tt][s_] = fs_rp_asm(rp, 4, 16 * tt, s_); }
#pragma unroll
        for (int jt = 0; jt < 2; ++jt)
#pragma unroll
            for (int s_ = 0; s_ < 2; ++s_) vB1[jt][s_] = fs_rp_asm(rp, 2, 16 * jt, s_);
        fs_pin<16>(dfr[0][0], ofr[0][0], dfr[0][1], ofr[0][1]);
        fs_pin<8>(dfr[1][0], ofr[1][0], dfr[1][1], ofr[1][1]);
#pragma unroll
        for (int tt = 0; tt < 2; ++tt) {
            const bf16x8 d0 = dfr[tt][0], d1 = dfr[tt][1];
            const bf16x8 o0 = ofr[tt][0], o1 = ofr[tt][1];
            f32x4 gm = mma32(o0, d0, zero4());
            gm = mma32(o1, d1, gm);
            const float dot = fs_diag_sum_rows(gm, g, c);
            if constexpr (PRE) {
                if (g == 0) PVw[16 * tt + c] = -dot;
                gA[tt][0] = d0;
                gA[tt][1] = d1;
            } else {
                const float inv = 1.f / dens[16 * tt + c];
                if (g == 0) { PVw[16 * tt + c] = -dot * inv; PVw[32 + 16 * tt + c] = -dot; PVw[64 + 16 * tt + c] = inv; }
                gA[tt][0] = fs_scale8(d0, inv);
                gA[tt][1] = fs_scale8(d1, inv);
            }
        }
        FSD(1);
        bf16x8 pb[2];
        {
            fs_pin<0>(vB1[0][0], vB1[0][1], vB1[1][0], vB1[1][1]);
            bf16x8 (&vB)[2][2] = vB1;
            f32x4 p00 = mma32(gA[0][0], vB[0][0], zero4()), p10 = mma32(gA[1][0], vB[0][0], zero4()), p11 = mma32(gA[1][0], vB[1][0], zero4());
            p00 = mma32(gA[0][1], vB[0][1], p00);
            p10 = mma32(gA[1][1], vB[0][1], p10);
            p11 = mma32(gA[1][1], vB[1][1], p11);
            const f32x4 dd0 = *(const f32x4*)(PVw + 4 * g), dd1 = *(const f32x4*)(PVw + 16 + 4 * g);
#pragma unroll
            for (int r = 0; r < 4; ++r) {
                const bool keep = (4 * g + r) >= c;
                p00[r] = keep ? p00[r] + dd0[r] : 0.f;
                p10[r] = p10[r] + dd1[r];
                p11[r] = keep ? p11[r] + dd1[r] : 0.f;
            }
            pb[0] = pack8(p00, p10);
            pb[1] = pack8(zero4(), p11);
        }
        FSD(2);
        fs_barrier();
        FSD(3);
        bf16x8 ab[2];
        {
            bf16x8 qfA[2][4], kfB[2][4];
#pragma unroll
            for (int hs = 0; hs < 2; ++hs)
#pragma unroll
                for (int u = 0; u < 2; ++u)
#pragma unroll
                    for (int tt = 0; tt < 2; ++tt) { qfA[tt][2 * hs + u] = fs_lp_asm(lpb, 0, 16 * tt, 2 * hs + u); kfB[tt][2 * hs + u] = fs_lp_asm(lpb, KFO, 16 * tt, 2 * hs + u); }
            fs_pin<24>(qfA[0][0], kfB[0][0], qfA[1][0], kfB[1][0]);
            fs_pin<16>(qfA[0][1], kfB[0][1], qfA[1][1], kfB[1][1]);
            f32x4 aa[3][2];
#pragma unroll
            for (int u = 0; u < 2; ++u) {
                aa[0][u] = mma32(qfA[0][u], kfB[0][u], zero4());
                aa[1][u] = mma32(qfA[1][u], kfB[0][u], zero4());
                aa[2][u] = mma32(qfA[1][u], kfB[1][u], zero4());
            }
            fs_pin<8>(qfA[0][2], kfB[0][2], qfA[1][2], kfB[1][2]);
            fs_pin<0>(qfA[0][3], kfB[0][3], qfA[1][3], kfB[1][3]);
#pragma unroll
            for (int u = 0; u < 2; ++u) {
                aa[0][u] = mma32(qfA[0][2 + u], kfB[0][2 + u], aa[0][u]);
                aa[1][u] = mma32(qfA[1][2 + u], kfB[0][2 + u], aa[1][u]);
                aa[2][u] = mma32(qfA[1][2 + u], kfB[1][2 + u], aa[2][u]);
            }
            f32x4 a00 = aa[0][0] + aa[0][1], a11 = aa[2][0] + aa[2][1];
            const f32x4 a10 = aa[1][0] + aa[1][1];
#pragma unroll
            for (int r = 0; r < 4; ++r) {
                const bool keep = (4 * g + r) >= c;
                a00[r] = keep ? a00[r] : 0.f;
                a11[r] = keep ? a11[r] : 0.f;
            }
            ab[0] = pack8(a00, a10);
            ab[1] = pack8(zero4(), a11);
        }
        FSD(4);
        f32x4 iv0 = {}, iv1 = {};
        if constexpr (!PRE) { iv0 = *(const f32x4*)(PVw + 64 + 4 * g); iv1 = *(const f32x4*)(PVw + 64 + 16 + 4 * g); }
        auto scale_t = [&](const bf16x8& x) {
            if constexpr (PRE) return x;
            else return (bf16x8){(bf16_t)((float)x[0] * iv0[0]), (bf16_t)((float)x[1] * iv0[1]), (bf16_t)((float)x[2] * iv0[2]), (bf16_t)((float)x[3] * iv0[3]),
                            (bf16_t)((float)x[4] * iv1[0]), (bf16_t)((float)x[5] * iv1[1]), (bf16_t)((float)x[6] * iv1[2]), (bf16_t)((float)x[7] * iv1[3])};
        };
        bf16x8 qfTs[2];
        {
            bf16x8 qfT[2], vB[2][2];
#pragma unroll
            for (int ph = 0; ph < 2; ++ph) {
                qfT[ph] = load_perm_tr(QF, FS_LDF, 16 * w + 64 * ph, 0, lane);
                qfTs[ph] = scale_t(qfT[ph]);
            }
#pragma unroll
            for (int jt = 0; jt < 2; ++jt)
#pragma unroll
                for (int s = 0; s < 2; ++s) vB[jt][s] = fs_rp_asm(rp, 2, 16 * jt, s);
            f32x4 dph[2][2];
#pragma unroll
            for (int jt = 0; jt < 2; ++jt)
#pragma unroll
                for (int ph = 0; ph < 2; ++ph) dph[jt][ph] = mma32(qfT[ph], pb[jt], zero4());
            fs_pin<0>(vB[0][0], vB[0][1], vB[1][0], vB[1][1]);
#pragma unroll
            for (int s = 0; s < 2; ++s)
#pragma unroll
                for (int ph = 0; ph < 2; ++ph) {
                    const bf16x8 rop = pack8(RT[2 * s][ph], RT[2 * s + 1][ph]);
#pragma unroll
                    for (int jt = 0; jt < 2; ++jt) dph[jt][ph] = mma32(rop, vB[jt][s], dph[jt][ph]);
                }
#pragma unroll
            for (int ph = 0; ph < 2; ++ph) {
                const bf16x4 rzop = {(bf16_t)RT[4][ph][0], (bf16_t)RT[4][ph][1], (bf16_t)RT[4][ph][2], (bf16_t)RT[4][ph][3]};
#pragma unroll
                for (int jt = 0; jt < 2; ++jt) dph[jt][ph] = mma16(rzop, onecol, dph[jt][ph]);
            }
#pragma unroll
            for (int jt = 0; jt < 2; ++jt) {
                const int row = 16 * jt + c;
                const bf16x4 kp = *(const bf16x4*)(KF + row * FS_LDF + 16 * w + 4 * g), kn = *(const bf16x4*)(KF + row * FS_LDF + 64 + 16 * w + 4 * g);
                float du[4], sa = 0.f;
#pragma unroll
                for (int r = 0; r < 4; ++r) {
                    const float ap = dph[jt][0][r] * (float)kp[r], am = dph[jt][1][r] * (float)kn[r];
                    du[r] = ap - am;
                    sa += ap + am;
                }
                sa = fs_sum_rows(sa);
                st4((bf16_t*)(DU + row * FS_ROWB + (((2 * w + (g >> 1)) ^ fs_sw(row)) << 4) + (g & 1) * 8), du[0], du[1], du[2], du[3]);
                if (g == 0) SA[w * 32 + row] = sa;
            }
        }
        FSD(5);
        const bf16x8 gTs = scale_t(fs_ring_perm_tr(Xg, 16 * w, lane));
        {
            bf16x8 kp0[4], kp1[4];
#pragma unroll
            for (int s = 0; s < 4; ++s) { kp0[s] = fs_lp_asm(lpb, KFO, 0, s); kp1[s] = fs_lp_asm(lpb, KFO, 16, s); }
            f32x4 a0 = mma32(gTs, ab[0], zero4()), a1 = mma32(gTs, ab[1], zero4());
            fs_pin<8>(kp0[0], kp1[0], kp0[1], kp1[1]);
#pragma unroll
            for (int s = 0; s < 4; ++s) {
                if (s == 2) fs_pin<0>(kp0[2], kp1[2], kp0[3], kp1[3]);
                const bf16x8 rd = pack8(RD[2 * s], RD[2 * s + 1]);
                a0 = mma32(rd, kp0[s], a0);
                a1 = mma32(rd, kp1[s], a1);
            }
            dv_prev[0] = (bf16x4){(bf16_t)a0[0], (bf16_t)a0[1], (bf16_t)a0[2], (bf16_t)a0[3]};
            dv_prev[1] = (bf16x4){(bf16_t)a1[0], (bf16_t)a1[1], (bf16_t)a1[2], (bf16_t)a1[3]};
        }
        FSD(6);
#pragma unroll
        for (int dl = 0; dl < 4; ++dl) {
            const bf16x8 gT = fs_ring_perm_tr(Xg, 16 * dl, lane);
            RT[dl][0] = mma32(gT, qfTs[0], RT[dl][0]);
            RT[dl][1] = mma32(gT, qfTs[1], RT[dl][1]);
        }
        {
            const f32x4 nd0 = *(const f32x4*)(PVw + (PRE ? 0 : 32) + 4 * g), nd1 = *(const f32x4*)(PVw + (PRE ? 0 : 32) + 16 + 4 * g);
            bf16x8 ndop = pack8(nd0, nd1);
#pragma unroll
            for (int e = 0; e < 8; ++e) ndop[e] = c == 0 ? ndop[e] : (bf16_t)0.f;
            RT[4][0] = mma32(ndop, qfTs[0], RT[4][0]);
            RT[4][1] = mma32(ndop, qfTs[1], RT[4][1]);
        }
#pragma unroll
        for (int ft = 0; ft < 8; ++ft) RD[ft] = mma32(load_perm_tr(QF, FS_LDF, 16 * ft, 0, lane), gTs, RD[ft]);
        FSD(7);
        fs_wait<0>();
        FSD(8);
        if (n > 0) {
            const int64_t tp = t0 + FS_C;
#pragma unroll
            for (int jt = 0; jt < 2; ++jt) *(bf16x4*)(dkb + (tp + 16 * jt + c) * ld_d + 16 * w + 4 * g) = dk_prev[jt];
        }
#pragma unroll
        for (int jt = 0; jt < 2; ++jt) *(bf16x4*)(dvb + (t0 + 16 * jt + c) * ld_d + 16 * w + 4 * g) = dv_prev[jt];
        fs_barrier();
        FSD(9);
        if (n + 2 < nch) issue(n + 2);
        FSD(10);
#pragma unroll
        for (int jt = 0; jt < 2; ++jt) {
            const int row = 16 * jt + c;
            const bf16x8 u0 = *(const bf16x8*)(DU + row * FS_ROWB + ((g ^ fs_sw(row)) << 4)), u1 = *(const bf16x8*)(DU + row * FS_ROWB + (((4 + g) ^ fs_sw(row)) << 4));
            f32x4 dx = mma32(wrow[0], u0, zero4());
            dx = mma32(wrow[1], u1, dx);
            const float sa = (SA[row] + SA[32 + row]) + (SA[64 + row] + SA[96 + row]);
            dk_prev[jt] = (bf16x4){(bf16_t)(cs * (dx[0] - cs * (float)xown[jt][0] * sa)), (bf16_t)(cs * (dx[1] - cs * (float)xown[jt][1] * sa)),
                                   (bf16_t)(cs * (dx[2] - cs * (float)xown[jt][2] * sa)), (bf16_t)(cs * (dx[3] - cs * (float)xown[jt][3] * sa))};
        }
        FSD(11);
    }
    FSD_END(32, 12);
#pragma unroll
    for (int jt = 0; jt < 2; ++jt) *(bf16x4*)(dkb + (16 * jt + c) * ld_d + 16 * w + 4 * g) = dk_prev[jt];
}
}

int emo_favor_fs_try(int which, int stage, const bf16_t* q, const bf16_t* k, const bf16_t* v, int64_t ld, const float* omega, bf16_t* out, int64_t ld_out,
                     float* den, float* sS, float* sz, const bf16_t* dout, bf16_t* dq, bf16_t* dk, bf16_t* dv, int64_t ld_d, int64_t B, int64_t T, int64_t H,
                     float eps, const float* ws_S, const float* ws_z, int P, int64_t Ts, hipStream_t st) {
    const char* e = getenv("EMO_FAVOR_FS");
    if (e && atoi(e) == 0) return 0;
    if (T < FS_C || (T % FS_C) != 0 || B * H <= 0 || P < 1 || (P > 1 && (Ts % FS_C) != 0)) return 0;
    if ((ld & 7) || (ld_out & 7) || (ld_d & 3)) return 0;
    if ((((uintptr_t)q | (uintptr_t)k | (uintptr_t)v | (uintptr_t)out | (uintptr_t)dout) & 15) || (((uintptr_t)dq | (uintptr_t)dk | (uintptr_t)dv) & 15)) return 0;
    if (P == 1) Ts = T;
    dim3 grid((unsigned)(B * H * P));
    if (which == 0) {
        const size_t lds = (size_t)(3 * 2 + 4) * FS_TILEB + sizeof(bf16_t) * (size_t)(4 * FS_C * FS_LDF);
        static bool attr = false;
        if (!attr) { (void)hipFuncSetAttribute((const void*)favor_fs_fwd_kernel, hipFuncAttributeMaxDynamicSharedMemorySize, (int)lds); attr = true; }
        hipLaunchKernelGGL(favor_fs_fwd_kernel, grid, dim3(FS_NT), lds, st, q, k, v, ld, omega, out, ld_out, den, sS, sz, T, H, eps, ws_S, ws_z, P, Ts);
        return 1;
    }
    const char* e2 = getenv("EMO_FAVOR_FS_BWD");
    if (e2 && atoi(e2) == 0) return 0;
    const bool pre = den == nullptr;
    if (stage == 0 || stage == 1) {
        const size_t lds = (size_t)3 * FS_SLOTB + 3 * 256 + 4 * 2048 + 2 * FS_TILEB + 2 * 4 * 32 * sizeof(float);
        static bool attr = false;
        if (!attr) {
            (void)hipFuncSetAttribute((const void*)favor_fs_dq_kernel<false>, hipFuncAttributeMaxDynamicSharedMemorySize, (int)lds);
            (void)hipFuncSetAttribute((const void*)favor_fs_dq_kernel<true>, hipFuncAttributeMaxDynamicSharedMemorySize, (int)lds);
            attr = true;
        }
        if (pre)
            hipLaunchKernelGGL(favor_fs_dq_kernel<true>, grid, dim3(FS_NT), lds, st, q, k, v, ld, omega, (const bf16_t*)out, dout, ld_out, (const float*)nullptr, dq, ld_d, T, H,
                               ws_S, ws_z, P, Ts);
        else
            hipLaunchKernelGGL(favor_fs_dq_kernel<false>, grid, dim3(FS_NT), lds, st, q, k, v, ld, omega, (const bf16_t*)out, dout, ld_out, (const float*)den, dq, ld_d, T, H,
                               ws_S, ws_z, P, Ts);
    }
    if (stage == 0 || stage == 2) {
        const size_t lds2 = (size_t)2 * FS_SLOTB + 2 * 256 + sizeof(bf16_t) * (size_t)(2 * FS_C * FS_LDF) + FS_TILEB + sizeof(float) * (128 + 4 * 96);
        static bool attr2 = false;
        if (!attr2) {
            (void)hipFuncSetAttribute((const void*)favor_fs_dkv_kernel<false>, hipFuncAttributeMaxDynamicSharedMemorySize, (int)lds2);
            (void)hipFuncSetAttribute((const void*)favor_fs_dkv_kernel<true>, hipFuncAttributeMaxDynamicSharedMemorySize, (int)lds2);
            attr2 = true;
        }
        if (pre)
            hipLaunchKernelGGL(favor_fs_dkv_kernel<true>, grid, dim3(FS_NT), lds2, st, q, k, v, ld, omega, (const bf16_t*)out, dout, ld_out, (const float*)nullptr, dk, dv, ld_d, T, H,
                               ws_S, ws_z, P, Ts);
        else
            hipLaunchKernelGGL(favor_fs_dkv_kernel<false>, grid, dim3(FS_NT), lds2, st, q, k, v, ld, omega, (const bf16_t*)out, dout, ld_out, (const float*)den, dk, dv, ld_d, T, H,
                               ws_S, ws_z, P, Ts);
    }
    return 1;
}
```

emo-disentanger_amd/ops.py:

```python
import ctypes

import os

import torch

from . import _lib
from ._lib import (ACT_GELU, ACT_GELU_NEW, ACT_NONE, ACT_RELU, BF16, F32, MUL_BITMASK, MUL_DGELU, MUL_DGELU_NEW, MUL_NONE, MUL_NONZERO, Epilogue, check,
                   dtype_code, lib, ptr, stream)

__all__ = ['gemm', 'colsum', 'embed_fwd', 'embed_bwd', 'layernorm_fwd', 'layernorm_bwd', 'dropout_apply', 'favor_attn_fwd',
           'favor_attn_bwd', 'favor_decode_step', 'performer_decode_step', 'performer_decode_step_sampled', 'favor_draw_omega', 'softmax_attn_fwd', 'softmax_attn_bwd', 'softmax_attn_decode', 'relpos_attn_fwd', 'relpos_attn_bwd', 'relpos_attn_decode', 'xent_fwd',
           'xent_bwd', 'argmax', 'sample_nucleus', 'sample_nucleus_step', 'txl_grammar_step', 'acc_grammar_step', 'accuracy_counts', 'sumsq', 'clip_coef', 'adam_step', 'cast', 'add_bias2',
           'ACT_NONE', 'ACT_RELU', 'ACT_GELU_NEW', 'ACT_GELU', 'MUL_NONE', 'MUL_NONZERO', 'MUL_DGELU_NEW', 'MUL_DGELU', 'MUL_BITMASK', 'gemm_bitmask_ok', 'gemm_lna_ok', 'bitmask_rows', 'favor_bwd_dn_ok', 'ffn_fwd', 'ffn_fwd_ok']


def _c(t):
    if t is None:
        return None
    assert t.dtype == torch.int64
    return t if t.is_contiguous() else t.contiguous()


def _rows(t):
    assert t.dim() == 2 and t.stride(1) == 1, 'need a 2-D tensor with unit column stride'
    return t.stride(0)


_stream = stream
_ws_cache = {}
_ws_need = {}
GEMM_TIMING = None
KERNEL_TIMING = None


class _timed:

    def __init__(self, kind, flops, nbytes):
        self.kind, self.flops, self.nbytes = kind, flops, nbytes

    def __enter__(self):
        if KERNEL_TIMING is not None:
            self.e0, self.e1 = torch.cuda.Event(enable_timing=True), torch.cuda.Event(enable_timing=True)
            self.e0.record()
        return self

    def __exit__(self, *a):
        if KERNEL_TIMING is not None:
            self.e1.record()
            KERNEL_TIMING.setdefault(self.kind, []).append((self.e0, self.e1, self.flops, self.nbytes))
        return False


def _workspace(kind, device, need, st=None):
    if need == 0:
        return None, 0
    key = (kind, device, st if st is not None else stream())
    buf = _ws_cache.get(key)
    if buf is None or buf.numel() < need:
        if buf is not None and st is not None and st != stream():
            buf.record_stream(torch.cuda.ExternalStream(st))
        buf = torch.empty(need, device=device, dtype=torch.uint8)
        _ws_cache[key] = buf
    return buf, need


def gemm(A, B, *, a_trans=False, b_trans=False, out=None, out_dtype=None, accumulate=False, bias=None, act=ACT_NONE,
         aux_out=None, mul_aux=None, mul_mode=MUL_NONE, mul_scale=1.0, p_drop=0.0, seed=0, offset=0, residual=None,
         ln_c1=None, ln_eps=1e-5, ln_stats_out=None, rln=None, a_rowsum=None, b_rowsum=None, mask_out=None, stream=None, lna=None, lna_out=None, hdiv=None):
    st = stream if stream is not None else _stream()
    K, M = (A.shape if a_trans else A.shape[::-1])
    Kb, N = (B.shape if b_trans else B.shape[::-1])
    assert K == Kb, 'inner dims differ: %s vs %s' % (tuple(A.shape), tuple(B.shape))
    assert A.dtype == B.dtype
    if out is None:
        out = torch.empty(M, N, device=A.device, dtype=out_dtype or A.dtype)
    ws, ws_bytes = None, 0
    plain = bias is None and residual is None and aux_out is None and mul_aux is None and act == ACT_NONE and p_drop == 0.0
    if (out.dtype == torch.float32 and plain) or (out.dtype == torch.bfloat16 and not accumulate and M > 32):
        wkey = (M, N, K, A.dtype, out.dtype)
        need = _ws_need.get(wkey)
        if need is None:
            need = _ws_need[wkey] = lib.emo_gemm_workspace_bytes(M, N, K, dtype_code(A.dtype), dtype_code(out.dtype))
        ws, ws_bytes = _workspace('gemm', A.device, need, st)
    rx, rstats, rgamma, rbeta = rln if rln is not None else (None, None, None, None)
    assert rx is None or (rx.dtype == out.dtype and _rows(rx) == _rows(out))
    ln_out = ln_mean = ln_rstd = None
    if lna is not None:
        assert gemm_lna_ok(M, N, K, A.dtype) and not a_trans and not b_trans and lna[0].dtype == torch.float32 and lna[1].dtype == torch.float32
        assert _rows(A) % 8 == 0 and _rows(B) % 8 == 0 and _rows(out) % 8 == 0 and (A.data_ptr() | B.data_ptr() | out.data_ptr()) % 16 == 0, \
            'lna=: the A-stationary kernel needs 16-B aligned operands and row strides that are multiples of 8 elements'
        ln_eps = lna[2]
        if lna_out is not None:
            ln_out, ln_mean, ln_rstd = lna_out
            assert ln_out.shape == (M, K) and ln_out.is_contiguous() and ln_out.dtype == A.dtype and ln_mean.numel() == M and ln_rstd.numel() == M
        else:
            ln_out = torch.empty(M, K, device=A.device, dtype=A.dtype)
            ln_mean = torch.empty(M, device=A.device, dtype=torch.float32)
            ln_rstd = torch.empty(M, device=A.device, dtype=torch.float32)
    epi = Epilogue(ptr(bias), act, ptr(aux_out), ptr(mul_aux), mul_mode, mul_scale, p_drop, seed, offset, ptr(residual),
                   ptr(ln_c1), ln_eps, ptr(ln_stats_out), ptr(rx), ptr(rstats), ptr(rgamma), ptr(rbeta), ptr(a_rowsum), ptr(b_rowsum), ptr(mask_out), ptr(ws), ws_bytes,
                   ptr(lna[0]) if lna is not None else None, ptr(lna[1]) if lna is not None else None, ptr(ln_out), ptr(ln_mean), ptr(ln_rstd),
                   ptr(hdiv[0]) if hdiv is not None else None, int(hdiv[1]) if hdiv is not None else 0)
    if hdiv is not None:
        assert hdiv[0].dtype == torch.float32 and hdiv[0].is_contiguous() and hdiv[0].numel() == M * (N // 64) and plain and mask_out is None and lna is None
    if not plain or mask_out is not None:
        for t in (aux_out, residual) + (() if mul_mode == MUL_BITMASK else (mul_aux,)):
            assert t is None or (t.dtype == out.dtype and _rows(t) == _rows(out))
        for t in (mask_out,) + ((mul_aux,) if mul_mode == MUL_BITMASK else ()):
            assert t is None or (t.dtype == torch.uint8 and t.is_contiguous() and t.shape == (M, N // 8) and gemm_bitmask_ok(M, N, K, A.dtype, out.dtype))
        assert bias is None or bias.dtype == torch.float32
    if GEMM_TIMING is not None:
        e0, e1 = torch.cuda.Event(enable_timing=True), torch.cuda.Event(enable_timing=True)
        tstream = torch.cuda.ExternalStream(st) if stream is not None else torch.cuda.current_stream()
        e0.record(tstream)
    check(lib.emo_gemm(ptr(A), int(a_trans), _rows(A), ptr(B), int(b_trans), _rows(B), ptr(out), _rows(out), M, N, K,
                       dtype_code(A.dtype), dtype_code(out.dtype), int(accumulate), ctypes.byref(epi), st))
    if GEMM_TIMING is not None:
        e1.record(tstream)
        kind = ('T' if a_trans else 'N') + ('N' if b_trans else 'T')
        fam = lib.emo_gemm_last_kernel() & 15
        if fam == 4:
            kind += '/K>1024'
        elif fam == 2:
            tag = [t for t, on in (('relu', act == ACT_RELU), ('gelu', act == ACT_GELU_NEW), ('drop', p_drop > 0), ('res', residual is not None),
                                   ('bits', mul_mode == MUL_BITMASK), ('mul', mul_aux is not None and mul_mode != MUL_BITMASK), ('mask', mask_out is not None),
                                   ('hdiv', hdiv is not None)) if on]
            kind += '/K=512/' + ('+'.join(tag) if tag else 'plain')
        elif fam == 3:
            kind += '/rs' if (a_rowsum is not None or b_rowsum is not None) else '/plain'
        elif kind == 'TN':
            kind += '/128'
        elif fam == 1:
            kind += '/skinny'
        GEMM_TIMING.append((kind, e0, e1, 2.0 * M * N * K,
                            (M * K + N * K) * A.element_size() + M * N * out.element_size(), (M, N, K)))
    if lna is not None:
        return out, ln_out, ln_mean, ln_rstd
    return out


ASTAT_MIN_ROWS = int(os.environ.get('EMO_ASTAT_MIN_ROWS', 0)) or 128 * 32


def gemm_bitmask_ok(M, N, K, in_dtype, out_dtype):
    return in_dtype == torch.bfloat16 and out_dtype == torch.bfloat16 and K == 512 and M % 128 == 0 and M >= ASTAT_MIN_ROWS and N % 64 == 0 and 64 <= N <= 2048


def gemm_lna_ok(M, N, K, in_dtype):
    return (in_dtype == torch.bfloat16 and K == 512 and M % 128 == 0 and M >= ASTAT_MIN_ROWS and N % 64 == 0 and 64 <= N <= 2048
            and os.environ.get('EMO_GEMM_NO_ASTAT') is None and os.environ.get('EMO_LN_IN_GEMM', '1') != '0'
            and os.environ.get('EMO_GEMM_SAFE_TR', '0') in ('', '0'))


def bitmask_rows(mask, M, N):
    t = mask.reshape(M // 32, N // 64, 4, 16, 2, 2)
    return t.permute(0, 4, 3, 1, 5, 2).reshape(M, N // 8)


def ffn_fwd_ok(M, d_model, d_ff, dtype):
    return dtype == torch.bfloat16 and bool(lib.emo_ffn_fwd_supported(dtype_code(dtype), M, d_model, d_ff))


def ffn_fwd(x1, gamma, beta, W1, b1, W2, b2, p_drop=0.0, seed=0, offset_f=0, offset_y=0, eps=1e-5):
    M, D = x1.shape
    Hd = W1.shape[0]
    assert x1.is_contiguous() and W1.is_contiguous() and W2.is_contiguous() and W1.shape == (Hd, D) and W2.shape == (D, Hd)
    assert b1.dtype == torch.float32 and b2.dtype == torch.float32 and gamma.dtype == torch.float32 and beta.dtype == torch.float32
    dev, dt = x1.device, x1.dtype
    h1, x2 = torch.empty_like(x1), torch.empty_like(x1)
    f = torch.empty(M, Hd, device=dev, dtype=dt)
    mean, rstd = torch.empty(M, device=dev, dtype=torch.float32), torch.empty(M, device=dev, dtype=torch.float32)
    mask = torch.empty(M, Hd // 8, device=dev, dtype=torch.uint8)
    flops, nbytes = 2.0 * 2.0 * M * D * Hd, (3.0 * M * D + M * Hd) * x1.element_size() + M * Hd / 8
    with _timed('ffn_fused_fwd', flops, nbytes):
        check(lib.emo_ffn_fwd(ptr(x1), ptr(gamma), ptr(beta), eps, ptr(W1), ptr(b1), ptr(W2), ptr(b2), ptr(h1), ptr(mean), ptr(rstd), ptr(f), ptr(mask),
                              ptr(x2), M, D, Hd, dtype_code(dt), p_drop, seed, offset_f, offset_y, stream()))
    return f, h1, mean, rstd, mask, x2


def colsum(X, out=None, accumulate=False):
    M, N = X.shape
    if out is None:
        out = torch.empty(N, device=X.device, dtype=torch.float32)
    check(lib.emo_colsum(ptr(X), dtype_code(X.dtype), M, N, _rows(X), ptr(out), int(accumulate), stream()))
    return out


def embed_fwd(tok, seg, E, S, pe, dtype, scale, pos0=0, p_drop=0.0, seed=0, offset=0, pos_ids=None):
    B, T = tok.shape
    D = E.shape[1]
    out = torch.empty(B, T, D, device=tok.device, dtype=dtype)
    assert pe.is_contiguous() and pe.shape[-1] == D and pe.numel() >= (pos0 + T) * D
    tok, seg, pos_ids = _c(tok), _c(seg), _c(pos_ids)
    check(lib.emo_embed_fwd(ptr(tok), ptr(seg), ptr(E), ptr(S), ptr(pe), ptr(out),
                            dtype_code(dtype), B, T, D, E.shape[0], 0 if S is None else S.shape[0], pos0, ptr(pos_ids), scale, p_drop, seed,
                            offset, stream()))
    return out


def embed_bwd(tok, seg, dout, dE, dS, scale, p_drop=0.0, seed=0, offset=0):
    B, T = tok.shape
    D = dE.shape[1]
    assert dout.is_contiguous()
    tok, seg = _c(tok), _c(seg)
    check(lib.emo_embed_bwd(ptr(tok), ptr(seg), ptr(dout), dtype_code(dout.dtype),
                            ptr(dE), ptr(dS), B, T, D, dE.shape[0], 0 if dS is None else dS.shape[0], scale, p_drop, seed, offset,
                            stream()))


def layernorm_fwd(x, gamma, beta, eps=1e-5):
    M, D = x.shape
    assert x.is_contiguous()
    y = torch.empty_like(x)
    mean = torch.empty(M, device=x.device, dtype=torch.float32)
    rstd = torch.empty(M, device=x.device, dtype=torch.float32)
    check(lib.emo_layernorm_fwd(ptr(x), ptr(gamma), ptr(beta), ptr(y), ptr(mean), ptr(rstd), dtype_code(x.dtype), M, D, eps, stream()))
    return y, mean, rstd


def layernorm_bwd(dy, x, gamma, mean, rstd, dgamma, dbeta, dres=None, want_drop=False, p_drop=0.0, seed=0, offset=0, dcol=None):
    M, D = x.shape
    assert dy.is_contiguous() and x.is_contiguous() and (dres is None or dres.is_contiguous())
    dx = torch.empty_like(x)
    dxd = torch.empty_like(x) if want_drop else None
    ws, ws_bytes = _workspace('ln_bwd', x.device, lib.emo_layernorm_bwd_workspace_bytes(dtype_code(x.dtype), M, D))
    check(lib.emo_layernorm_bwd_ws(ptr(dy), ptr(x), ptr(gamma), ptr(mean), ptr(rstd), ptr(dres), ptr(dx), ptr(dxd), ptr(dgamma), ptr(dbeta),
                                   ptr(dcol), dtype_code(x.dtype), M, D, p_drop, seed, offset, ptr(ws), ws_bytes, stream()))
    return dx, dxd


def dropout_apply(x, p_drop, seed, offset):
    assert x.is_contiguous()
    out = torch.empty_like(x)
    check(lib.emo_dropout_apply(ptr(x), ptr(out), dtype_code(x.dtype), x.numel(), p_drop, seed, offset, stream()))
    return out


def _favor_workspace(device, B, T, H, dh, n_feat):
    return _workspace('favor', device, lib.emo_favor_attn_workspace_bytes(B, T, H, dh, n_feat))


def favor_attn_fwd(q, k, v, omega, B, T, H, eps=1e-6, want_state=False, keep_ws=False):
    M, HD = q.shape
    dh = HD // H
    n_feat = 2 * omega.shape[1]
    assert M == B * T and omega.shape[0] == dh and omega.dtype == torch.float32 and omega.is_contiguous()
    assert _rows(q) == _rows(k) == _rows(v)
    out = torch.empty(M, HD, device=q.device, dtype=q.dtype)
    den = torch.empty(B, H, T, device=q.device, dtype=torch.float32)
    S = torch.empty(B, H, n_feat, dh, device=q.device, dtype=torch.float32) if want_state else None
    z = torch.empty(B, H, n_feat, device=q.device, dtype=torch.float32) if want_state else None
    if keep_ws:
        ws_bytes = lib.emo_favor_attn_workspace_bytes(B, T, H, dh, n_feat)
        ws = torch.empty(ws_bytes, device=q.device, dtype=torch.uint8) if ws_bytes else None
    else:
        ws, ws_bytes = _favor_workspace(q.device, B, T, H, dh, n_feat)
    with _timed('favor_fwd', 0.0, 4.0 * M * HD * q.element_size()):
        check(lib.emo_favor_attn_fwd(ptr(q), ptr(k), ptr(v), _rows(q), ptr(omega), ptr(out), HD, ptr(den), ptr(S), ptr(z), dtype_code(q.dtype),
                                     B, T, H, dh, n_feat, eps, ptr(ws), ws_bytes, stream()))
    if keep_ws:
        assert not want_state
        return out, den, ws
    return (out, den, S, z) if want_state else (out, den)


def favor_bwd_dn_ok(dtype, B, T, H, dh, n_feat):
    return dtype == torch.bfloat16 and bool(lib.emo_favor_attn_bwd_dn_supported(dtype_code(dtype), B, T, H, dh, n_feat))


def favor_attn_bwd(q, k, v, omega, out, dout, den, B, T, H, dqkv=None, eps=1e-6, ws_saved=None, dn=False):
    M, HD = q.shape
    dh = HD // H
    n_feat = 2 * omega.shape[1]
    assert out.is_contiguous() and dout.is_contiguous()
    if dqkv is None:
        dqkv = torch.empty(M, 3 * HD, device=q.device, dtype=q.dtype)
    dq, dk, dv = dqkv[:, :HD], dqkv[:, HD:2 * HD], dqkv[:, 2 * HD:]
    if dn:
        with _timed('favor_bwd', 0.0, 7.0 * M * HD * q.element_size()):
            check(lib.emo_favor_attn_bwd_dn(ptr(q), ptr(k), ptr(v), _rows(q), ptr(omega), ptr(out), ptr(dout), HD, ptr(dq), ptr(dk), ptr(dv), 3 * HD,
                                            dtype_code(q.dtype), B, T, H, dh, n_feat, eps, stream()))
        return dq, dk, dv
    if ws_saved is not None:
        ws, ws_bytes, kvalid = ws_saved, ws_saved.numel(), 1
        assert ws_bytes == lib.emo_favor_attn_workspace_bytes(B, T, H, dh, n_feat)
    else:
        (ws, ws_bytes), kvalid = _favor_workspace(q.device, B, T, H, dh, n_feat), 0
    with _timed('favor_bwd', 0.0, 7.0 * M * HD * q.element_size()):
        check(lib.emo_favor_attn_bwd_kstate(ptr(q), ptr(k), ptr(v), _rows(q), ptr(omega), ptr(out), ptr(dout), HD, ptr(den), ptr(dq), ptr(dk), ptr(dv),
                                            3 * HD, dtype_code(q.dtype), B, T, H, dh, n_feat, eps, ptr(ws), ws_bytes, kvalid, stream()))
    return dq, dk, dv


def favor_decode_step(q, k, v, omega, state_S, state_z, H, eps=1e-6):
    n, HD = q.shape
    dh = HD // H
    out = torch.empty(n, HD, device=q.device, dtype=q.dtype)
    check(lib.emo_favor_decode_step(ptr(q), ptr(k), ptr(v), _rows(q), ptr(omega), ptr(state_S), ptr(state_z), ptr(out), HD,
                                    dtype_code(q.dtype), n, H, dh, 2 * omega.shape[1], eps, stream()))
    return out


def performer_decode_step(layer_table, n_layers, tok, seg, E, Sg, pe, emb_scale, pos0, pos_ids, wout_packed, bout, n_token, logits, n_streams,
                          d_model, n_head, n_feat, d_ff, sync_ws, eps=1e-6, ln_eps=1e-5, diag=None):
    tok, seg, pos_ids = _c(tok), _c(seg), _c(pos_ids)
    assert logits.dtype == torch.float32 and logits.is_contiguous() and logits.shape == (n_streams, n_token)
    check(lib.emo_performer_decode_step(ptr(layer_table), n_layers, ptr(tok), ptr(seg), ptr(E), ptr(Sg), ptr(pe), emb_scale, pos0, ptr(pos_ids),
                                        ptr(wout_packed), ptr(bout), n_token, ptr(logits), n_streams, d_model, n_head, n_feat, d_ff,
                                        ptr(sync_ws), sync_ws.numel() * sync_ws.element_size(), eps, ln_eps, ptr(diag), stream()))
    return logits


def performer_decode_step_sampled(layer_table, n_layers, seg, E, Sg, pe, emb_scale, pos0, wout_packed, bout, n_token, logits, n_streams, n_real,
                                  d_model, n_head, n_feat, d_ff, sync_ws, temperature, top_p, u_steps, step, seq, col0, tok_out, eps=1e-6, ln_eps=1e-5):
    seg = _c(seg)
    assert logits.dtype == torch.float32 and logits.is_contiguous() and logits.shape == (n_streams, n_token)
    assert u_steps.dtype == torch.float32 and u_steps.is_contiguous() and u_steps.shape[1] == n_real and step.dtype == torch.int64 and tok_out.dtype == torch.int64
    assert seq is None or (seq.dtype == torch.int64 and seq.stride(1) == 1)
    check(lib.emo_performer_decode_step_sampled(ptr(layer_table), n_layers, ptr(seg), ptr(E), ptr(Sg), ptr(pe), emb_scale, pos0, ptr(wout_packed), ptr(bout),
                                                n_token, ptr(logits), n_streams, n_real, d_model, n_head, n_feat, d_ff, ptr(sync_ws),
                                                sync_ws.numel() * sync_ws.element_size(), eps, ln_eps, temperature, top_p, ptr(u_steps), ptr(step), ptr(seq),
                                                0 if seq is None else seq.stride(0), col0, ptr(tok_out), stream()))
    return logits


def gpt2_decode_step(layer_table, n_layers, tok, seg, E, Sg, pe, emb_scale, pos0, pos_ids, ln0, kv_tmax, wout_packed, bout, n_token, logits, n_streams,
                     d_model, n_head, d_ff, sync_ws, ln_eps=1e-5, diag=None):
    tok, seg, pos_ids = _c(tok), _c(seg), _c(pos_ids)
    assert logits.dtype == torch.float32 and logits.is_contiguous() and logits.shape == (n_streams, n_token)
    assert ln0.dtype == torch.float32 and ln0.is_contiguous() and ln0.numel() == 2 * d_model
    check(lib.emo_gpt2_decode_step(ptr(layer_table), n_layers, ptr(tok), ptr(seg), ptr(E), ptr(Sg), ptr(pe), emb_scale, pos0, ptr(pos_ids), ptr(ln0), kv_tmax,
                                   ptr(wout_packed), ptr(bout), n_token, ptr(logits), n_streams, d_model, n_head, d_ff,
                                   ptr(sync_ws), sync_ws.numel() * sync_ws.element_size(), ln_eps, ptr(diag), stream()))
    return logits


def gpt2_decode_step_sampled(layer_table, n_layers, seg, E, Sg, pe, emb_scale, pos0, ln0, kv_tmax, wout_packed, bout, n_token, logits, n_streams, n_real,
                             d_model, n_head, d_ff, sync_ws, temperature, top_p, u_steps, step, seq, col0, tok_out, ln_eps=1e-5):
    seg = _c(seg)
    assert logits.dtype == torch.float32 and logits.is_contiguous() and logits.shape == (n_streams, n_token)
    assert ln0.dtype == torch.float32 and ln0.is_contiguous() and ln0.numel() == 2 * d_model
    assert u_steps.dtype == torch.float32 and u_steps.is_contiguous() and u_steps.shape[1] == n_real and step.dtype == torch.int64 and tok_out.dtype == torch.int64
    assert seq is None or (seq.dtype == torch.int64 and seq.stride(1) == 1)
    check(lib.emo_gpt2_decode_step_sampled(ptr(layer_table), n_layers, ptr(seg), ptr(E), ptr(Sg), ptr(pe), emb_scale, pos0, ptr(ln0), kv_tmax, ptr(wout_packed),
                                           ptr(bout), n_token, ptr(logits), n_streams, n_real, d_model, n_head, d_ff, ptr(sync_ws),
                                           sync_ws.numel() * sync_ws.element_size(), ln_eps, temperature, top_p, ptr(u_steps), ptr(step), ptr(seq),
                                           0 if seq is None else seq.stride(0), col0, ptr(tok_out), stream()))
    return logits


def favor_draw_omega(gauss, omega):
    L, nb, dh, _ = gauss.shape
    assert gauss.is_contiguous() and omega.is_contiguous() and omega.shape[:2] == (L, dh)
    check(lib.emo_favor_draw_omega(ptr(gauss), ptr(omega), L, dh, 2 * omega.shape[2], stream()))
    return omega


def softmax_attn_fwd(q, k, v, B, T, H, p_drop=0.0, seed=0, offset=0, want_keep=False):
    M, HD = q.shape
    dh = HD // H
    assert M == B * T and _rows(q) == _rows(k) == _rows(v)
    out = torch.empty(M, HD, device=q.device, dtype=q.dtype)
    lse = torch.empty(B, H, T, device=q.device, dtype=torch.float32)
    keep, kbytes = None, 0
    if want_keep and all(t.data_ptr() % 16 == 0 for t in (q, k, v)):
        kbytes = lib.emo_softmax_attn_keep_bytes(dtype_code(q.dtype), B, T, H, dh, p_drop)
        if kbytes:
            keep = torch.empty(kbytes // 4, device=q.device, dtype=torch.int32)
    with _timed('sattn_fwd', 0.5 * 2 * 2.0 * B * H * T * T * dh, 4.0 * M * HD * q.element_size()):
        check(lib.emo_softmax_attn_fwd_keep(ptr(q), ptr(k), ptr(v), _rows(q), ptr(out), HD, ptr(lse), dtype_code(q.dtype), B, T, H, dh, p_drop,
                                            seed, offset, ptr(keep), kbytes, stream()))
    return (out, lse, keep) if want_keep else (out, lse)


def softmax_attn_bwd(q, k, v, out, dout, lse, B, T, H, p_drop=0.0, seed=0, offset=0, dqkv=None, keep=None):
    M, HD = q.shape
    dh = HD // H
    assert out.is_contiguous() and dout.is_contiguous()
    if dqkv is None:
        dqkv = torch.empty(M, 3 * HD, device=q.device, dtype=q.dtype)
    dq, dk, dv = dqkv[:, :HD], dqkv[:, HD:2 * HD], dqkv[:, 2 * HD:]
    delta = torch.empty(B, H, T, device=q.device, dtype=torch.float32)
    with _timed('sattn_bwd', 0.5 * 7 * 2.0 * B * H * T * T * dh, 8.0 * M * HD * q.element_size()):
        check(lib.emo_softmax_attn_bwd_keep(ptr(q), ptr(k), ptr(v), _rows(q), ptr(out), ptr(dout), HD, ptr(lse), ptr(delta), ptr(dq), ptr(dk), ptr(dv), 3 * HD,
                                            dtype_code(q.dtype), B, T, H, dh, p_drop, seed, offset, ptr(keep), 0 if keep is None else keep.numel() * 4, stream()))
    return dq, dk, dv


def softmax_attn_decode(q, kcache, vcache, lens, H, lens_off=0, k_new=None, v_new=None):
    n, HD = q.shape
    head_major = kcache.dim() == 4
    T_max = kcache.shape[2] if head_major else kcache.shape[1]
    assert kcache.is_contiguous() and vcache.is_contiguous() and lens.dtype == torch.int64 and kcache.shape == vcache.shape
    assert not head_major or (kcache.shape[1] == H and kcache.shape[3] == HD // H)
    assert (k_new is None) == (v_new is None) and (k_new is None or _rows(k_new) == _rows(v_new))
    out = torch.empty(n, HD, device=q.device, dtype=q.dtype)
    check(lib.emo_softmax_attn_decode_layout(ptr(q), _rows(q), ptr(kcache), ptr(vcache), T_max, ptr(lens), lens_off, ptr(k_new), ptr(v_new),
                                             0 if k_new is None else _rows(k_new), ptr(out), HD, dtype_code(q.dtype), n, H, HD // H, int(head_major), stream()))
    return out


def relpos_attn_fwd(q, k, v, r_dist, r_w_bias, r_r_bias, B, T, H, p_drop=0.0, seed=0, offset=0):
    M, HD = q.shape
    dh = HD // H
    assert M == B * T and _rows(q) == _rows(k) == _rows(v) and r_dist.shape[0] >= T and r_dist.dtype == q.dtype
    assert r_w_bias.dtype == torch.float32 and r_r_bias.dtype == torch.float32 and r_w_bias.is_contiguous() and r_r_bias.is_contiguous()
    out = torch.empty(M, HD, device=q.device, dtype=q.dtype)
    lse = torch.empty(B, H, T, device=q.device, dtype=torch.float32)
    zden = torch.empty(B, H, T, device=q.device, dtype=torch.float32)
    check(lib.emo_relpos_attn_fwd(ptr(q), ptr(k), ptr(v), _rows(q), ptr(r_dist), _rows(r_dist), r_dist.shape[0], ptr(r_w_bias), ptr(r_r_bias), ptr(out), HD,
                                  ptr(lse), ptr(zden), dtype_code(q.dtype), B, T, H, dh, p_drop, seed, offset, stream()))
    return out, lse, zden


def relpos_attn_bwd(qkv, r_dist, r_w_bias, r_r_bias, out, dout, lse, zden, B, T, H, p_drop=0.0, seed=0, offset=0, acc_dq=None, acc_rr=None, dR_out=None, dq_rel_out=None):
    M, D3 = qkv.shape
    D = D3 // 3
    dh = D // H
    dt, dev = qkv.dtype, qkv.device
    assert M == B * T and out.is_contiguous() and dout.is_contiguous() and qkv.is_contiguous()
    dqkv = torch.empty(M, D3, device=dev, dtype=dt)
    dq_rel = dq_rel_out if dq_rel_out is not None else torch.empty(M, D, device=dev, dtype=dt)
    assert dq_rel.shape == (M, D) and dq_rel.dtype == dt and dq_rel.is_contiguous()
    delta = torch.empty(B, H, T, device=dev, dtype=torch.float32)
    q, k, v = qkv[:, :D], qkv[:, D:2 * D], qkv[:, 2 * D:]
    check(lib.emo_relpos_attn_bwd(ptr(q), ptr(k), ptr(v), D3, ptr(r_dist), _rows(r_dist), r_dist.shape[0], ptr(r_w_bias), ptr(r_r_bias), ptr(out),
                                  ptr(dout), D, ptr(lse), ptr(zden), ptr(dqkv), D3, ptr(dq_rel), D, ptr(delta), dtype_code(dt), B, T, H, dh, p_drop,
                                  seed, offset, stream()))
    if acc_rr is not None:
        if acc_dq is not None:
            colsum(dqkv[:, :D], out=acc_dq, accumulate=True)
        if dq_rel_out is None:
            colsum(dq_rel, out=acc_rr, accumulate=True)
        d_rr = d_rw = None
    else:
        d_rr = colsum(dq_rel)
        d_rw = (colsum(dqkv[:, :D]) - d_rr).view(H, dh)
        d_rr = d_rr.view(H, dh)
    qu, qv = add_bias2(q, r_w_bias, r_r_bias)
    check(lib.emo_relpos_attn_bwd_kv(ptr(qu), ptr(qv), D, ptr(k), ptr(v), D3, ptr(r_dist), _rows(r_dist), r_dist.shape[0], ptr(dout), D, ptr(lse),
                                     ptr(zden), ptr(delta), ptr(dqkv[:, D:2 * D]), ptr(dqkv[:, 2 * D:]), D3, dtype_code(dt), B, T, H, dh, p_drop, seed,
                                     offset, stream()))
    if dR_out is not None:
        assert dR_out.dtype == torch.float32 and dR_out.shape[1] == D and dR_out.shape[0] >= T and dR_out.stride(1) == 1
        dR = dR_out
    else:
        dR = torch.empty(T, D, device=dev, dtype=torch.float32)
    ws, ws_bytes = _workspace('relpos_dr', dev, lib.emo_relpos_attn_bwd_r_workspace_bytes(B, T, H, dh))
    check(lib.emo_relpos_attn_bwd_r(ptr(qu), ptr(qv), D, ptr(k), ptr(v), D3, ptr(r_dist), _rows(r_dist), r_dist.shape[0], ptr(dout), D, ptr(lse),
                                    ptr(zden), ptr(delta), ptr(dR), _rows(dR), ptr(ws), ws_bytes, dtype_code(dt), B, T, H, dh, p_drop, seed, offset, stream()))
    return dqkv, dR, d_rw, d_rr


def relpos_attn_decode(q, kcache, vcache, lens, H, r_dist, r_w_bias, r_r_bias, mem_len=0, lens_off=0, k_new=None, v_new=None):
    n, HD = q.shape
    T_max = kcache.shape[1]
    assert kcache.is_contiguous() and vcache.is_contiguous() and lens.dtype == torch.int64 and r_dist.shape[0] >= T_max
    out = torch.empty(n, HD, device=q.device, dtype=q.dtype)
    check(lib.emo_relpos_attn_decode(ptr(q), _rows(q), ptr(kcache), ptr(vcache), T_max, ptr(lens), lens_off, mem_len, ptr(k_new), ptr(v_new),
                                     0 if k_new is None else _rows(k_new), ptr(r_dist), _rows(r_dist), r_dist.shape[0], ptr(r_w_bias), ptr(r_r_bias),
                                     ptr(out), HD, dtype_code(q.dtype), n, H, HD // H, stream()))
    return out


def xent_fwd(logits, tgt, ignore_index):
    M, V = logits.shape
    assert logits.is_contiguous() and logits.dtype == torch.float32
    lse = torch.empty(M, device=logits.device, dtype=torch.float32)
    acc = torch.zeros(2, device=logits.device, dtype=torch.float32)
    tgt = _c(tgt)
    check(lib.emo_xent_fwd(ptr(logits), ptr(tgt), M, V, ignore_index, ptr(lse), ptr(acc), stream()))
    return lse, acc


def xent_bwd(logits, tgt, lse, gscale, ignore_index, out_dtype, ld_out=None):
    M, V = logits.shape
    ld_out = ld_out or ((V + 7) // 8) * 8
    dl = torch.empty(M, ld_out, device=logits.device, dtype=out_dtype)
    tgt = _c(tgt)
    check(lib.emo_xent_bwd(ptr(logits), ptr(tgt), ptr(lse), ptr(gscale), ptr(dl), ld_out, dtype_code(out_dtype), M, V,
                           ignore_index, stream()))
    return dl


def argmax(logits):
    rows, V = logits.shape
    assert logits.is_contiguous() and logits.dtype == torch.float32
    out = torch.empty(rows, device=logits.device, dtype=torch.int64)
    check(lib.emo_argmax(ptr(logits), rows, V, ptr(out), stream()))
    return out


def sample_nucleus(logits, temperature, top_p, u):
    rows, V = logits.shape
    assert logits.is_contiguous() and logits.dtype == torch.float32 and u.dtype == torch.float32 and u.numel() == rows
    out = torch.empty(rows, device=logits.device, dtype=torch.int64)
    check(lib.emo_sample_nucleus(ptr(logits), rows, V, temperature, top_p, ptr(u), ptr(out), stream()))
    return out


def sample_nucleus_step(logits, temperature, top_p, u_steps, step, seq=None, col0=0, out=None):
    rows, V = logits.shape
    assert logits.is_contiguous() and logits.dtype == torch.float32 and u_steps.dtype == torch.float32 and u_steps.is_contiguous()
    assert u_steps.shape[-1] == rows and step.dtype == torch.int64 and step.numel() == rows
    assert seq is None or (seq.dtype == torch.int64 and seq.stride(1) == 1 and seq.shape[0] == rows)
    if out is None:
        out = torch.empty(rows, device=logits.device, dtype=torch.int64)
    check(lib.emo_sample_nucleus_step(ptr(logits), rows, V, temperature, top_p, ptr(u_steps), ptr(step), ptr(seq), 0 if seq is None else seq.stride(0),
                                      col0, ptr(out), stream()))
    return out


TXL_PARAM_WORDS = TXL_STATE_WORDS = 8


def txl_grammar_step(logits, temperature, top_p, key_temperature, key_top_p, u_steps, ev_flags, ev_beat, params, state, seq, tok_out, running):
    n, V = logits.shape
    assert logits.is_contiguous() and logits.dtype == torch.float32
    assert u_steps.dtype == torch.float32 and u_steps.is_contiguous() and u_steps.dim() == 2 and u_steps.shape[1] == n
    for t, dt in ((ev_flags, torch.int32), (ev_beat, torch.int32), (params, torch.int32), (state, torch.int32), (running, torch.int32),
                  (seq, torch.int64), (tok_out, torch.int64)):
        assert t.dtype == dt and t.is_contiguous()
    assert ev_flags.numel() >= V and ev_beat.numel() >= V and running.numel() >= 1 and tok_out.numel() == n
    assert params.shape == (n, TXL_PARAM_WORDS) and state.shape == (n, TXL_STATE_WORDS) and seq.dim() == 2 and seq.shape[0] == n
    check(lib.emo_txl_grammar_step(ptr(logits), n, V, temperature, top_p, key_temperature, key_top_p, ptr(u_steps), u_steps.shape[0], ptr(ev_flags),
                                   ptr(ev_beat), ptr(params), ptr(state), ptr(seq), seq.shape[1], ptr(tok_out), ptr(running), stream()))
    return tok_out


ACC_PARAM_WORDS = ACC_STATE_WORDS = 8


def acc_grammar_step(logits, temperature, top_p, u_steps, ev_flags, ev_beat, lead_tok, lead_off, params, state, seq, segs, max_len, track_full, pad,
                     tok_out, seg_out, running):
    n, V = logits.shape
    assert V <= 1024 and temperature > 0
    assert logits.is_contiguous() and logits.dtype == torch.float32
    assert u_steps.dtype == torch.float32 and u_steps.is_contiguous() and u_steps.dim() == 2 and u_steps.shape[1] == n
    for t, dt in ((ev_flags, torch.int32), (ev_beat, torch.int32), (lead_off, torch.int32), (params, torch.int32), (state, torch.int32),
                  (running, torch.int32), (lead_tok, torch.int64), (seq, torch.int64), (segs, torch.int64), (tok_out, torch.int64), (seg_out, torch.int64)):
        assert t.dtype == dt and t.is_contiguous()
    assert ev_flags.numel() >= V and ev_beat.numel() >= V and running.numel() >= 1 and tok_out.numel() == n and seg_out.numel() == n
    assert params.shape == (n, ACC_PARAM_WORDS) and state.shape == (n, ACC_STATE_WORDS)
    assert seq.dim() == 2 and seq.shape[0] == n and segs.shape == seq.shape and lead_tok.numel() >= 1 and lead_off.numel() >= 1
    check(lib.emo_acc_grammar_step(ptr(logits), n, V, temperature, top_p, ptr(u_steps), u_steps.shape[0], ptr(ev_flags), ptr(ev_beat), ptr(lead_tok),
                                   ptr(lead_off), ptr(params), ptr(state), ptr(seq), ptr(segs), seq.shape[1], max_len, track_full, pad, ptr(tok_out),
                                   ptr(seg_out), ptr(running), stream()))
    return tok_out


def accuracy_counts(logits, tgt, chord, melody, pad):
    M, V = logits.shape
    counts = torch.zeros(6, device=logits.device, dtype=torch.int64)
    assert logits.is_contiguous() and logits.dtype == torch.float32
    tgt, chord, melody = _c(tgt), _c(chord), _c(melody)
    check(lib.emo_accuracy_counts(ptr(logits), ptr(tgt), ptr(chord), ptr(melody), M, V, pad, ptr(counts), stream()))
    return counts


SUMSQ_FLOATS = 1026


def sumsq(x, acc):
    assert acc.dtype == torch.float32 and acc.numel() >= SUMSQ_FLOATS
    check(lib.emo_sumsq(ptr(x), x.numel(), ptr(acc), stream()))


def clip_coef(sumsq_t, max_norm, pre, coef, denom=None):
    assert denom is None or (denom.dtype == torch.float32 and denom.numel() >= 1)
    check(lib.emo_clip_coef(ptr(sumsq_t), max_norm, pre, ptr(denom), ptr(coef), stream()))


def adam_step(p, g, m, v, p_bf16, lr, beta1, beta2, eps, step, gscale):
    check(lib.emo_adam_step(ptr(p), ptr(g), ptr(m), ptr(v), ptr(p_bf16), p.numel(), lr, beta1, beta2, eps, step, ptr(gscale), stream()))


def transpose_batch(desc, n, total_tiles):
    check(lib.emo_transpose_batch(ptr(desc), n, total_tiles, stream()))


def add_bias2(x, b1, b2):
    M, D = x.shape
    assert b1.dtype == torch.float32 and b2.dtype == torch.float32 and b1.numel() == D and b2.numel() == D and b1.is_contiguous() and b2.is_contiguous()
    o1, o2 = torch.empty(M, D, device=x.device, dtype=x.dtype), torch.empty(M, D, device=x.device, dtype=x.dtype)
# ... 9 lines not shown
```

include/emo_hip.h:

```cpp
#ifndef EMO_HIP_H
#define EMO_HIP_H
#include <stdint.h>

#ifdef __cplusplus
extern "C" {
#endif

typedef void* emo_stream_t;

enum { EMO_OK = 0, EMO_ERR_INVALID = -1, EMO_ERR_LAUNCH = -2, EMO_ERR_UNSUPPORTED = -3 };
enum { EMO_F32 = 0, EMO_BF16 = 1, EMO_I64 = 2  };
enum { EMO_ACT_NONE = 0, EMO_ACT_RELU = 1, EMO_ACT_GELU_NEW = 2, EMO_ACT_GELU = 3 };
enum { EMO_MUL_NONE = 0, EMO_MUL_NONZERO = 1, EMO_MUL_DGELU_NEW = 2, EMO_MUL_BITMASK = 3, EMO_MUL_DGELU = 4 };

int emo_version(void);
int emo_build_flags(void);
const char* emo_last_error(void);
int emo_device_cus(void);

typedef struct {
    const float* bias;
    int act;
    void* aux_out;
    const void* mul_aux;
    int mul_mode;
    float mul_scale;
    float p_drop;
    uint64_t seed, offset;
    const void* residual;
    const float* ln_c1;
    float ln_eps;
    float* ln_stats_out;
    const void* rln_x;
    const float* rln_stats;
    const float* rln_gamma;
    const float* rln_beta;
    float* a_rowsum;
    float* b_rowsum;
    uint8_t* mask_out;
    void* workspace;
    int64_t workspace_bytes;
    const float* lna_gamma;
    const float* lna_beta;
    void* lna_out;
    float* lna_mean;
    float* lna_rstd;
    const float* hdiv;
    int64_t hdiv_T;
} emo_epilogue_t;

int emo_gemm_last_kernel(void);
int emo_epilogue_size(void);
int64_t emo_gemm_workspace_bytes(int64_t M, int64_t N, int64_t K, int dtype_in, int dtype_out);

int emo_gemm(const void* A, int a_trans, int64_t lda, const void* B, int b_trans, int64_t ldb,
             void* C, int64_t ldc, int64_t M, int64_t N, int64_t K,
             int dtype_in, int dtype_out, int accumulate ,
             const emo_epilogue_t* epi , emo_stream_t stream);

int emo_ffn_fwd_supported(int dtype, int64_t M, int64_t d_model, int64_t d_ff);
int emo_ffn_fwd(const void* x1, const float* gamma, const float* beta, float ln_eps, const void* W1,
                const float* b1, const void* W2, const float* b2, void* h1_out, float* mean_out,
                float* rstd_out, void* f_out, uint8_t* mask_out, void* x2_out, int64_t M, int64_t d_model,
                int64_t d_ff, int dtype, float p_drop, uint64_t seed, uint64_t offset_f, uint64_t offset_y,
                emo_stream_t stream);

int emo_colsum(const void* X, int dtype, int64_t M, int64_t N, int64_t ld, float* out,
               int accumulate, emo_stream_t stream);

int emo_embed_fwd(const int64_t* tok, const int64_t* seg, const float* E, const float* S,
                  const float* pe, void* out, int dtype, int64_t B, int64_t T, int64_t D,
                  int64_t V, int64_t n_seg, int64_t pos0, const int64_t* pos_ids, float scale,
                  float p_drop, uint64_t seed, uint64_t offset, emo_stream_t stream);
int emo_embed_bwd(const int64_t* tok, const int64_t* seg, const void* dout, int dtype, float* dE,
                  float* dS, int64_t B, int64_t T, int64_t D, int64_t V, int64_t n_seg,
                  float scale, float p_drop, uint64_t seed, uint64_t offset, emo_stream_t stream);

int emo_layernorm_fwd(const void* x, const float* gamma, const float* beta, void* y, float* mean,
                      float* rstd, int dtype, int64_t M, int64_t D, float eps, emo_stream_t stream);
int emo_layernorm_bwd(const void* dy, const void* x, const float* gamma, const float* mean,
                      const float* rstd, const void* dres, void* dx, void* dx_drop, float* dgamma,
                      float* dbeta, float* dcol, int dtype, int64_t M, int64_t D, float p_drop,
                      uint64_t seed, uint64_t offset, emo_stream_t stream);
int64_t emo_layernorm_bwd_workspace_bytes(int dtype, int64_t M, int64_t D);
int emo_layernorm_bwd_ws(const void* dy, const void* x, const float* gamma, const float* mean,
                         const float* rstd, const void* dres, void* dx, void* dx_drop, float* dgamma,
                         float* dbeta, float* dcol, int dtype, int64_t M, int64_t D, float p_drop,
                         uint64_t seed, uint64_t offset, void* workspace, int64_t workspace_bytes,
                         emo_stream_t stream);
int emo_dropout_apply(const void* x, void* out, int dtype, int64_t n, float p_drop, uint64_t seed,
                      uint64_t offset, emo_stream_t stream);

int64_t emo_favor_attn_workspace_bytes(int64_t B, int64_t T, int64_t H, int64_t dh, int64_t n_feat);
int emo_favor_attn_fwd(const void* q, const void* k, const void* v, int64_t ld, const float* omega,
                       void* out, int64_t ld_out, float* den, float* state_S, float* state_z,
                       int dtype, int64_t B, int64_t T, int64_t H, int64_t dh, int64_t n_feat,
                       float eps, void* workspace, int64_t workspace_bytes, emo_stream_t stream);
int emo_favor_attn_bwd(const void* q, const void* k, const void* v, int64_t ld, const float* omega,
                       const void* out, const void* dout, int64_t ld_out, const float* den,
                       void* dq, void* dk, void* dv, int64_t ld_d, int dtype, int64_t B, int64_t T,
                       int64_t H, int64_t dh, int64_t n_feat, float eps, void* workspace,
                       int64_t workspace_bytes, emo_stream_t stream);
int emo_favor_attn_bwd_kstate(const void* q, const void* k, const void* v, int64_t ld, const float* omega,
                              const void* out, const void* dout, int64_t ld_out, const float* den, void* dq,
                              void* dk, void* dv, int64_t ld_d, int dtype, int64_t B, int64_t T, int64_t H,
                              int64_t dh, int64_t n_feat, float eps, void* workspace, int64_t workspace_bytes,
                              int kstate_valid, emo_stream_t stream);
int emo_favor_attn_bwd_dn_supported(int dtype, int64_t B, int64_t T, int64_t H, int64_t dh, int64_t n_feat);
int emo_favor_attn_bwd_dn(const void* q, const void* k, const void* v, int64_t ld, const float* omega,
                          const void* out, const void* dn, int64_t ld_out, void* dq, void* dk, void* dv,
                          int64_t ld_d, int dtype, int64_t B, int64_t T, int64_t H, int64_t dh, int64_t n_feat,
                          float eps, emo_stream_t stream);
int emo_favor_decode_step(const void* q, const void* k, const void* v, int64_t ld, const float* omega,
                          float* state_S, float* state_z, void* out, int64_t ld_out, int dtype,
                          int64_t n_streams, int64_t H, int64_t dh, int64_t n_feat, float eps,
                          emo_stream_t stream);
int64_t emo_performer_decode_step_workspace_bytes(void);
int emo_performer_decode_step_supported(void);
int emo_performer_decode_step(const void* layer_table, int64_t n_layers, const int64_t* tok, const int64_t* seg, const float* E,
                              const float* Sg, const float* pe, float emb_scale, int64_t pos0, const int64_t* pos_ids,
                              const void* wout_packed, const float* bout, int64_t n_token, float* logits, int64_t n_streams,
                              int64_t d_model, int64_t n_head, int64_t n_feat, int64_t d_ff, void* sync_ws, int64_t sync_ws_bytes,
                              float eps, float ln_eps, int64_t* diag, emo_stream_t stream);
int emo_performer_decode_step_sampled(const void* layer_table, int64_t n_layers, const int64_t* seg, const float* E, const float* Sg,
                                      const float* pe, float emb_scale, int64_t pos0, const void* wout_packed, const float* bout,
                                      int64_t n_token, float* logits, int64_t n_streams, int64_t n_real, int64_t d_model, int64_t n_head,
                                      int64_t n_feat, int64_t d_ff, void* sync_ws, int64_t sync_ws_bytes, float eps, float ln_eps,
                                      float temperature, float top_p, const float* u_steps, int64_t* step, int64_t* seq, int64_t ld_seq,
                                      int64_t col0, int64_t* tok_out, emo_stream_t stream);

int emo_gpt2_decode_step_supported(void);
int emo_gpt2_decode_step(const void* layer_table, int64_t n_layers, const int64_t* tok, const int64_t* seg, const float* E, const float* Sg,
                         const float* pe, float emb_scale, int64_t pos0, const int64_t* pos_ids, const float* ln0, int64_t kv_tmax,
                         const void* wout_packed, const float* bout, int64_t n_token, float* logits, int64_t n_streams, int64_t d_model,
                         int64_t n_head, int64_t d_ff, void* sync_ws, int64_t sync_ws_bytes, float ln_eps, int64_t* diag, emo_stream_t stream);
int emo_gpt2_decode_step_sampled(const void* layer_table, int64_t n_layers, const int64_t* seg, const float* E, const float* Sg, const float* pe,
                                 float emb_scale, int64_t pos0, const float* ln0, int64_t kv_tmax, const void* wout_packed, const float* bout,
                                 int64_t n_token, float* logits, int64_t n_streams, int64_t n_real, int64_t d_model, int64_t n_head, int64_t d_ff,
                                 void* sync_ws, int64_t sync_ws_bytes, float ln_eps, float temperature, float top_p, const float* u_steps,
                                 int64_t* step, int64_t* seq, int64_t ld_seq, int64_t col0, int64_t* tok_out, emo_stream_t stream);

int emo_favor_draw_omega(const float* gauss, float* omega, int64_t n_layers, int64_t dh, int64_t n_feat,
                         emo_stream_t stream);

int emo_softmax_attn_fwd(const void* q, const void* k, const void* v, int64_t ld, void* out,
                         int64_t ld_out, float* lse, int dtype, int64_t B, int64_t T, int64_t H,
                         int64_t dh, float p_drop, uint64_t seed, uint64_t offset, emo_stream_t stream);
int emo_softmax_attn_bwd(const void* q, const void* k, const void* v, int64_t ld, const void* out,
                         const void* dout, int64_t ld_out, const float* lse, float* delta_ws,
                         void* dq, void* dk, void* dv, int64_t ld_d, int dtype, int64_t B, int64_t T,
                         int64_t H, int64_t dh, float p_drop, uint64_t seed, uint64_t offset,
                         emo_stream_t stream);
int64_t emo_softmax_attn_keep_bytes(int dtype, int64_t B, int64_t T, int64_t H, int64_t dh, float p_drop);
int emo_softmax_attn_fwd_keep(const void* q, const void* k, const void* v, int64_t ld, void* out,
                              int64_t ld_out, float* lse, int dtype, int64_t B, int64_t T, int64_t H,
                              int64_t dh, float p_drop, uint64_t seed, uint64_t offset, void* keep,
                              int64_t keep_bytes, emo_stream_t stream);
int emo_softmax_attn_bwd_keep(const void* q, const void* k, const void* v, int64_t ld, const void* out,
                              const void* dout, int64_t ld_out, const float* lse, float* delta_ws,
                              void* dq, void* dk, void* dv, int64_t ld_d, int dtype, int64_t B,
                              int64_t T, int64_t H, int64_t dh, float p_drop, uint64_t seed,
                              uint64_t offset, const void* keep, int64_t keep_bytes, emo_stream_t stream);
int emo_softmax_attn_decode(const void* q, int64_t ld_q, void* kcache, void* vcache, int64_t T_max,
                            const int64_t* lens, int64_t lens_off, const void* k_new, const void* v_new,
                            int64_t ld_new, void* out, int64_t ld_out, int dtype, int64_t n_streams,
                            int64_t H, int64_t dh, emo_stream_t stream);
int emo_softmax_attn_decode_layout(const void* q, int64_t ld_q, void* kcache, void* vcache, int64_t T_max,
                                   const int64_t* lens, int64_t lens_off, const void* k_new, const void* v_new,
                                   int64_t ld_new, void* out, int64_t ld_out, int dtype, int64_t n_streams,
                                   int64_t H, int64_t dh, int head_major, emo_stream_t stream);

int emo_relpos_attn_fwd(const void* q, const void* k, const void* v, int64_t ld, const void* r_dist,
                        int64_t ld_r, int64_t n_dist, const float* r_w_bias, const float* r_r_bias,
                        void* out, int64_t ld_out, float* lse, float* zden, int dtype, int64_t B,
                        int64_t T, int64_t H, int64_t dh, float p_drop, uint64_t seed,
                        uint64_t offset, emo_stream_t stream);
int emo_relpos_attn_bwd(const void* q, const void* k, const void* v, int64_t ld, const void* r_dist,
                        int64_t ld_r, int64_t n_dist, const float* r_w_bias, const float* r_r_bias,
                        const void* out, const void* dout, int64_t ld_out, const float* lse,
                        const float* zden, void* dq, int64_t ld_d, void* dq_rel, int64_t ld_rel,
                        float* delta, int dtype, int64_t B, int64_t T, int64_t H, int64_t dh,
                        float p_drop, uint64_t seed, uint64_t offset, emo_stream_t stream);
int64_t emo_relpos_attn_bwd_r_workspace_bytes(int64_t B, int64_t T, int64_t H, int64_t dh);
int emo_relpos_attn_bwd_r(const void* qu, const void* qv, int64_t ld_q, const void* k, const void* v,
                          int64_t ld, const void* r_dist, int64_t ld_r, int64_t n_dist, const void* dout,
                          int64_t ld_out, const float* lse, const float* zden, const float* delta,
                          float* dR, int64_t ld_dr, void* workspace, int64_t workspace_bytes, int dtype,
                          int64_t B, int64_t T, int64_t H, int64_t dh, float p_drop, uint64_t seed,
                          uint64_t offset, emo_stream_t stream);
int emo_relpos_attn_bwd_kv(const void* qu, const void* qv, int64_t ld_q, const void* k, const void* v,
                           int64_t ld, const void* r_dist, int64_t ld_r, int64_t n_dist, const void* dout,
                           int64_t ld_out, const float* lse, const float* zden, const float* delta,
                           void* dk, void* dv, int64_t ld_d, int dtype, int64_t B, int64_t T, int64_t H,
                           int64_t dh, float p_drop, uint64_t seed, uint64_t offset, emo_stream_t stream);
int emo_relpos_attn_decode(const void* q, int64_t ld_q, void* kcache, void* vcache, int64_t T_max,
                           const int64_t* lens, int64_t lens_off, int64_t mem_len, const void* k_new,
                           const void* v_new, int64_t ld_new, const void* r_dist, int64_t ld_r,
                           int64_t n_dist, const float* r_w_bias, const float* r_r_bias, void* out,
                           int64_t ld_out, int dtype, int64_t n_streams, int64_t H, int64_t dh,
                           emo_stream_t stream);

int emo_xent_fwd(const float* logits, const int64_t* tgt, int64_t M, int64_t V, int64_t ignore_index,
                 float* row_lse, float* acc, emo_stream_t stream);
int emo_xent_bwd(const float* logits, const int64_t* tgt, const float* row_lse, const float* gscale,
                 void* dlogits, int64_t ld_out ,
                 int dtype_out, int64_t M, int64_t V, int64_t ignore_index, emo_stream_t stream);

int emo_argmax(const float* logits, int64_t rows, int64_t V, int64_t* out, emo_stream_t stream);
int emo_sample_nucleus(const float* logits, int64_t rows, int64_t V, float temperature, float top_p,
                       const float* u, int64_t* out, emo_stream_t stream);
int emo_sample_nucleus_step(const float* logits, int64_t rows, int64_t V, float temperature,
                            float top_p, const float* u_steps, int64_t* step, int64_t* seq,
                            int64_t ld_seq, int64_t col0, int64_t* out, emo_stream_t stream);
enum { EMO_TXL_P_MAX_BARS = 0, EMO_TXL_P_MAX_EVENTS = 1, EMO_TXL_P_PRIMER_LEN = 2, EMO_TXL_P_KEYED = 3, EMO_TXL_P_KEY_RULE = 4,
       EMO_TXL_P_EMO_MODE = 5 , EMO_TXL_PARAM_WORDS = 8 };
enum { EMO_TXL_S_STATUS = 0, EMO_TXL_S_LEN = 1 , EMO_TXL_S_ACCEPTED = 2, EMO_TXL_S_BEAT = 3, EMO_TXL_S_BARS = 4,
       EMO_TXL_S_FAILED = 5 , EMO_TXL_S_FEED = 6 , EMO_TXL_S_DRAWS = 7, EMO_TXL_STATE_WORDS = 8 };
enum { EMO_TXL_RUNNING = 0, EMO_TXL_DONE = 1, EMO_TXL_STUCK = 2, EMO_TXL_KEY_ERROR = 3, EMO_TXL_OVERFLOW = 4  };
enum { EMO_TXL_EV_BEAT = 1, EMO_TXL_EV_BAR = 2, EMO_TXL_EV_PAD = 4, EMO_TXL_EV_EOS = 8, EMO_TXL_EV_KEY = 16, EMO_TXL_EV_MAJOR = 32, EMO_TXL_EV_MINOR = 64 };
int emo_txl_grammar_step(const float* logits, int64_t n, int64_t V, float temperature, float top_p,
                         float key_temperature, float key_top_p, const float* u_steps, int64_t n_u,
                         const int32_t* ev_flags, const int32_t* ev_beat, const int32_t* params,
                         int32_t* state, int64_t* seq, int64_t ld_seq, int64_t* tok_out, int32_t* running,
                         emo_stream_t stream);
enum { EMO_ACC_P_TARGET_BARS = 0, EMO_ACC_P_MAX_EVENTS = 1, EMO_ACC_P_SKIP_CHECK = 2, EMO_ACC_P_BAR0 = 3, EMO_ACC_P_N_BARS = 4, EMO_ACC_PARAM_WORDS = 8 };
enum { EMO_ACC_S_STATUS = 0, EMO_ACC_S_LEN = 1 , EMO_ACC_S_CONSUMED = 2 ,
       EMO_ACC_S_BARS = 3 , EMO_ACC_S_CUR_POS = 4, EMO_ACC_S_FAILED = 5 , EMO_ACC_S_DRAWS = 6,
       EMO_ACC_S_ACCEPTED = 7 , EMO_ACC_STATE_WORDS = 8 };
enum { EMO_ACC_RUNNING = 0, EMO_ACC_DONE = 1, EMO_ACC_STUCK = 2, EMO_ACC_WINDOW = 3, EMO_ACC_OUT_OF_DRAWS = 4, EMO_ACC_OVERFLOW = 5 };
enum { EMO_ACC_EV_BEAT = 1, EMO_ACC_EV_TRACK_LS = 2, EMO_ACC_EV_PAD = 4, EMO_ACC_EV_EOS = 8 };
int emo_acc_grammar_step(const float* logits, int64_t n, int64_t V, float temperature, float top_p,
                         const float* u_steps, int64_t n_u, const int32_t* ev_flags, const int32_t* ev_beat,
                         const int64_t* lead_tok, const int32_t* lead_off, const int32_t* params, int32_t* state,
                         int64_t* seq, int64_t* segs, int64_t ld_seq, int64_t max_len, int64_t track_full,
                         int64_t pad, int64_t* tok_out, int64_t* seg_out, int32_t* running, emo_stream_t stream);
int emo_accuracy_counts(const float* logits, const int64_t* tgt, const int64_t* chord,
                        const int64_t* melody, int64_t M, int64_t V, int64_t pad, int64_t* counts,
                        emo_stream_t stream);

#define EMO_SUMSQ_FLOATS 1026
int emo_sumsq(const float* x, int64_t n, float* acc, emo_stream_t stream);
int emo_clip_coef(const float* sumsq, float max_norm, float pre, const float* denom, float* coef, emo_stream_t stream);
int emo_adam_step(float* p, const float* g, float* m, float* v, void* p_bf16, int64_t n, float lr,
                  float beta1, float beta2, float eps, int64_t step, const float* gscale,
                  emo_stream_t stream);
int emo_cast(const void* src, int src_dtype, void* dst, int dst_dtype, int64_t n, emo_stream_t stream);
int emo_add_bias2(const void* x, int64_t ld, const float* b1, const float* b2, void* o1, void* o2, int dtype,
                  int64_t M, int64_t D, emo_stream_t stream);
int emo_transpose_batch(const int64_t* desc, int n, int64_t total_tiles, emo_stream_t stream);
int emo_stream_wait(emo_stream_t waiter, emo_stream_t signaler);

int emo_comm_bind(void);
int emo_comm_unique_id(void* id128);
int emo_comm_init(const void* id128, int rank, int world);
int emo_comm_world(void);
int emo_comm_rank(void);
int emo_comm_allreduce(void* buf, int64_t count, int dtype, emo_stream_t stream);
int emo_comm_broadcast(void* buf, int64_t count, int dtype, int root, emo_stream_t stream);
int emo_comm_destroy(void);

#ifdef __cplusplus
}
#endif
#endif
```

Measured before the change: 3.028 million tokens/s.

## Pass dq-kernel row dot products to dk/dv kernel and deepen its ring

In the den-less FAVOR backward path, the dq kernel now writes the per-row -dot(out, dout) values into an fp32 workspace. The dk/dv kernel reads these instead of reloading the output tile and recomputing the dot with MMAs. The LDS freed by dropping the output tile goes to a third ring slot, so prefetch runs deeper. The path also launches through stage 0 instead of two separate stage calls, and callers must now allocate a B*H*T float workspace.

New measurement: 3.039 million tokens/s, median of 6. Within noise of the previous version (+0.4%).

```diff
diff --git a/emo-disentanger_amd/_lib.py b/emo-disentanger_amd/_lib.py
--- a/emo-disentanger_amd/_lib.py
+++ b/emo-disentanger_amd/_lib.py
@@ -50,7 +50,8 @@
     'emo_favor_attn_bwd': (c_i, [c_p, c_p, c_p, c_l, c_p, c_p, c_p, c_l, c_p, c_p, c_p, c_p, c_l, c_i, c_l, c_l, c_l, c_l, c_l, c_f, c_p, c_l, c_p]),
     'emo_favor_attn_bwd_kstate': (c_i, [c_p, c_p, c_p, c_l, c_p, c_p, c_p, c_l, c_p, c_p, c_p, c_p, c_l, c_i, c_l, c_l, c_l, c_l, c_l, c_f, c_p, c_l, c_i, c_p]),
     'emo_favor_attn_bwd_dn_supported': (c_i, [c_i, c_l, c_l, c_l, c_l, c_l]),
-    'emo_favor_attn_bwd_dn': (c_i, [c_p, c_p, c_p, c_l, c_p, c_p, c_p, c_l, c_p, c_p, c_p, c_l, c_i, c_l, c_l, c_l, c_l, c_l, c_f, c_p]),
+    'emo_favor_attn_bwd_dn_workspace_bytes': (c_l, [c_l, c_l, c_l]),
+    'emo_favor_attn_bwd_dn': (c_i, [c_p, c_p, c_p, c_l, c_p, c_p, c_p, c_l, c_p, c_p, c_p, c_l, c_i, c_l, c_l, c_l, c_l, c_l, c_f, c_p, c_l, c_p]),
     'emo_favor_decode_step': (c_i, [c_p, c_p, c_p, c_l, c_p, c_p, c_p, c_p, c_l, c_i, c_l, c_l, c_l, c_l, c_f, c_p]),
     'emo_performer_decode_step_workspace_bytes': (c_l, []),
     'emo_performer_decode_step_supported': (c_i, []),
diff --git a/emo-disentanger_amd/csrc/emo_favor.hip b/emo-disentanger_amd/csrc/emo_favor.hip
--- a/emo-disentanger_amd/csrc/emo_favor.hip
+++ b/emo-disentanger_amd/csrc/emo_favor.hip
@@ -1166,7 +1166,7 @@
 
 int emo_favor_fs_try(int which, int stage, const bf16_t* q, const bf16_t* k, const bf16_t* v, int64_t ld, const float* omega, bf16_t* out, int64_t ld_out,
                      float* den, float* sS, float* sz, const bf16_t* dout, bf16_t* dq, bf16_t* dk, bf16_t* dv, int64_t ld_d, int64_t B, int64_t T, int64_t H,
-                     float eps, const float* ws_S, const float* ws_z, int P, int64_t Ts, hipStream_t st);
+                     float eps, const float* ws_S, const float* ws_z, int P, int64_t Ts, float* dd_ws, hipStream_t st);
 
 #define EMO_FAVOR_SEG_ALIGN 64
 #define EMO_FAVOR_MAX_SEGMENTS 16
@@ -1200,6 +1200,14 @@
                      void* workspace, int64_t workspace_bytes, hipStream_t st, bool kstate_valid = false) {
     constexpr int F = 2 * MF;
     int P = 1; int64_t Ts = T > 0 ? T : 1;
+    float* dd_ws = nullptr;
+    if (which != 0 && den == nullptr) {
+        EMO_CHECK(workspace && workspace_bytes >= B * H * T * (int64_t)sizeof(float), "emo_favor_attn_bwd_dn: workspace %lld B < %lld B (emo_favor_attn_bwd_dn_workspace_bytes)",
+                  (long long)workspace_bytes, (long long)(B * H * T * (int64_t)sizeof(float)));
+        EMO_CHECK(((uintptr_t)workspace & 15) == 0, "emo_favor_attn_bwd_dn: workspace must be 16-B aligned");
+        dd_ws = (float*)workspace;
+        workspace = nullptr;
+    }
     if (workspace) {
         favor_segments(B, T, H, &P, &Ts);
         const int64_t need = P > 1 ? B * H * P * (int64_t)(F * DH + F) * (int64_t)sizeof(float) : 0;
@@ -1215,7 +1223,7 @@
     auto fs_try = [&](int stage) -> bool {
         if constexpr (FS) {
             if (emo_favor_fs_try(which, stage, (const bf16_t*)q, (const bf16_t*)k, (const bf16_t*)v, ld, omega, (bf16_t*)out, ld_out, den, sS, sz, (const bf16_t*)dout,
-                                 (bf16_t*)dq, (bf16_t*)dk, (bf16_t*)dv, ld_d, B, T, H, eps, wsS, wsz, P, Ts, st))
+                                 (bf16_t*)dq, (bf16_t*)dk, (bf16_t*)dv, ld_d, B, T, H, eps, wsS, wsz, P, Ts, dd_ws, st))
                 return true;
         }
         const char* e = getenv("EMO_FAVOR_FS");
@@ -1260,7 +1268,7 @@
         }
         if (den == nullptr) {
             EMO_CHECK(FS && P == 1, "emo_favor_attn_bwd_dn: needs bf16, d_head 64, 128 features and a single-segment scan (B * H >= 256): emo_favor_attn_bwd_dn_supported()");
-            if (!fs_try(1) || !fs_try(2)) {
+            if (!fs_try(0)) {
                 emo_set_error("emo_favor_attn_bwd_dn: the slice kernels refused this call (T %% 32, 16-B alignment, EMO_FAVOR_FS / EMO_FAVOR_FS_BWD = 0)");
                 return EMO_ERR_UNSUPPORTED;
             }
@@ -1352,9 +1360,10 @@
     favor_segments(B, T, H, &P, &Ts);
     return P <= 1 ? 1 : 0;
 }
+extern "C" int64_t emo_favor_attn_bwd_dn_workspace_bytes(int64_t B, int64_t T, int64_t H) { return B * H * T * (int64_t)sizeof(float); }
 extern "C" int emo_favor_attn_bwd_dn(const void* q, const void* k, const void* v, int64_t ld, const float* omega, const void* out, const void* dn,
                                      int64_t ld_out, void* dq, void* dk, void* dv, int64_t ld_d, int dtype, int64_t B, int64_t T, int64_t H,
-                                     int64_t dh, int64_t n_feat, float eps, emo_stream_t stream) {
+                                     int64_t dh, int64_t n_feat, float eps, void* workspace, int64_t workspace_bytes, emo_stream_t stream) {
     int rc = favor_check(q, k, v, ld, ld_out, dtype, dh, n_feat);
     if (rc) return rc;
     EMO_CHECK(omega && out && dn && dq && dk && dv, "emo_favor_attn_bwd_dn: null pointer");
@@ -1362,7 +1371,7 @@
     EMO_CHECK(ld_d % 4 == 0, "emo_favor_attn_bwd_dn: ld_d must be a multiple of 4");
     EMO_CHECK((((uintptr_t)dq | (uintptr_t)dk | (uintptr_t)dv | (uintptr_t)out | (uintptr_t)dn) & 15) == 0, "emo_favor_attn_bwd_dn: pointers must be 16-B aligned");
     return dispatch_favor(1, dtype, dh, n_feat / 2, q, k, v, ld, omega, (void*)out, ld_out, (float*)nullptr, nullptr, nullptr, dn, dq, dk, dv, ld_d, B, T, H,
-                          eps, nullptr, 0, (hipStream_t)stream, false);
+                          eps, workspace, workspace_bytes, (hipStream_t)stream, false);
 }
 extern "C" int emo_favor_attn_bwd(const void* q, const void* k, const void* v, int64_t ld, const float* omega, const void* out, const void* dout,
                                   int64_t ld_out, const float* den, void* dq, void* dk, void* dv, int64_t ld_d, int dtype, int64_t B, int64_t T, int64_t H,
diff --git a/emo-disentanger_amd/csrc/emo_favor_fs.hip b/emo-disentanger_amd/csrc/emo_favor_fs.hip
--- a/emo-disentanger_amd/csrc/emo_favor_fs.hip
+++ b/emo-disentanger_amd/csrc/emo_favor_fs.hip
@@ -414,7 +414,8 @@
                                                                int64_t ld, const float* __restrict__ omega, const bf16_t* __restrict__ out,
                                                                const bf16_t* __restrict__ dout, int64_t ld_out, const float* __restrict__ den_g,
                                                                bf16_t* __restrict__ dq, int64_t ld_d, int64_t Tfull, int64_t H,
-                                                               const float* __restrict__ S_ws, const float* __restrict__ z_ws, int P, int64_t Ts) {
+                                                               const float* __restrict__ S_ws, const float* __restrict__ z_ws, int P, int64_t Ts,
+                                                               float* __restrict__ dd_g) {
     extern __shared__ __attribute__((aligned(16))) char smem[];
     char* RING = smem;
     char* DEN = RING + 3 * FS_SLOTB;
@@ -433,6 +434,8 @@
     const bf16_t* gb = dout + (b * Tfull + tbeg) * ld_out + h * 64;
     bf16_t* dqb = dq + (b * Tfull + tbeg) * ld_d + h * 64;
     const float* dnb = den_g + bh * Tfull + tbeg;
+    float* ddb = PRE ? dd_g + bh * Tfull + tbeg + (lane & 31) : nullptr;
+    const bool dd_lane = PRE && w == 0 && g < 2;
     const float cs = rsqrtf(sqrtf(64.f));
     const float cs2 = cs * FS_LOG2E, c2h = 0.5f * cs * cs * FS_LOG2E, hl = 0.5f * logf(128.f) * FS_LOG2E;
 
@@ -503,6 +506,7 @@
     asm volatile("" ::: "memory");
     char* KPw = KP + w * 2048;
     bf16x4 o_prev[2] = {};
+    float dd_prev = 0.f, dd_cur = 0.f;
     uint32_t rpl[2][2];
     fs_rp_lane(g, c, rpl);
     FSD_BEGIN
@@ -584,6 +588,7 @@
                 gop[tt][1] = fs_scale8(dfr[tt][1], inv);
             }
         }
+        if constexpr (PRE) dd_cur = g == 0 ? dD[0] : dD[1];
         FSD(1);
         if (i > 0) issue_part(i + 2, 4);
         bf16x8 at[2];
@@ -667,7 +672,9 @@
         if (i > 0) {
 #pragma unroll
             for (int tt = 0; tt < 2; ++tt) *(bf16x4*)(dqb + (t0 - FS_C + 16 * tt + c) * ld_d + 16 * w + 4 * g) = o_prev[tt];
-        }
+            if constexpr (PRE) { if (dd_lane) ddb[t0 - FS_C] = dd_prev; }
+        }
+        dd_prev = dd_cur;
         fs_barrier();
         FSD(6);
         issue_part(i + 3, 0);
@@ -692,19 +699,28 @@
         const int64_t t0 = (int64_t)nch * FS_C;
 #pragma unroll
         for (int tt = 0; tt < 2; ++tt) *(bf16x4*)(dqb + (t0 - FS_C + 16 * tt + c) * ld_d + 16 * w + 4 * g) = o_prev[tt];
-    }
-}
-
+        if constexpr (PRE) { if (dd_lane) ddb[t0 - FS_C] = dd_prev; }
+    }
+}
+
+template <bool PRE> struct FsDkvRing {
+    static constexpr int NSLOT = PRE ? 3 : 2;
+    static constexpr int SLOTB = (PRE ? 4 : 5) * FS_TILEB;
+    static constexpr int NPART = PRE ? 5 : 6;
+    static constexpr size_t LDS = (size_t)NSLOT * SLOTB + NSLOT * 256 + sizeof(bf16_t) * (size_t)(2 * FS_C * FS_LDF) + FS_TILEB + sizeof(float) * (128 + 4 * 96);
+};
 template <bool PRE>
 __global__ __launch_bounds__(FS_NT, 2) void favor_fs_dkv_kernel(const bf16_t* __restrict__ q, const bf16_t* __restrict__ k, const bf16_t* __restrict__ v,
                                                                 int64_t ld, const float* __restrict__ omega, const bf16_t* __restrict__ out,
                                                                 const bf16_t* __restrict__ dout, int64_t ld_out, const float* __restrict__ den_g,
                                                                 bf16_t* __restrict__ dk, bf16_t* __restrict__ dv, int64_t ld_d, int64_t Tfull, int64_t H,
-                                                                const float* __restrict__ R_ws, const float* __restrict__ r_ws, int P, int64_t Ts) {
+                                                                const float* __restrict__ R_ws, const float* __restrict__ r_ws, int P, int64_t Ts,
+                                                                const float* __restrict__ dd_g) {
+    constexpr int NSLOT = FsDkvRing<PRE>::NSLOT, SLOTB = FsDkvRing<PRE>::SLOTB, NPART = FsDkvRing<PRE>::NPART;
     extern __shared__ __attribute__((aligned(16))) char smem[];
     char* RING = smem;
-    char* DEN = RING + 2 * FS_SLOTB;
-    bf16_t* QF = (bf16_t*)(DEN + 2 * 256);
+    char* DEN = RING + NSLOT * SLOTB;
+    bf16_t* QF = (bf16_t*)(DEN + NSLOT * 256);
     bf16_t* KF = QF + FS_C * FS_LDF;
     char* DU = (char*)(KF + FS_C * FS_LDF);
     float* SA = (float*)(DU + FS_TILEB);
@@ -721,7 +737,7 @@
     const bf16_t* gb = dout + (b * Tfull + tbeg) * ld_out + h * 64;
     bf16_t* dkb = dk + (b * Tfull + tbeg) * ld_d + h * 64;
     bf16_t* dvb = dv + (b * Tfull + tbeg) * ld_d + h * 64;
-    const float* dnb = den_g + bh * Tfull + tbeg;
+    const float* dnb = (PRE ? dd_g : den_g) + bh * Tfull + tbeg;
     const float cs = rsqrtf(sqrtf(64.f));
     const float cs2 = cs * FS_LOG2E, c2h = 0.5f * cs * cs * FS_LOG2E, hl = 0.5f * logf(128.f) * FS_LOG2E;
 
@@ -775,20 +791,19 @@
     const int64_t so_qkv = (int64_t)srow * ld + spc, so_o = (int64_t)srow * ld_out + spc;
     auto issue = [&](int n) {
         const int64_t t0n = (int64_t)(nch - 1 - n) * FS_C;
-        const uint32_t dst = ring_lds + (n & 1) * FS_SLOTB + w * 1024;
+        const uint32_t dst = ring_lds + (n % NSLOT) * SLOTB + w * 1024;
         fs_dma16(qb + t0n * ld + so_qkv, dst);
         fs_dma16(kb + t0n * ld + so_qkv, dst + FS_TILEB);
         fs_dma16(vb + t0n * ld + so_qkv, dst + 2 * FS_TILEB);
         fs_dma16(gb + t0n * ld_out + so_o, dst + 3 * FS_TILEB);
-        fs_dma16(ob + t0n * ld_out + so_o, dst + 4 * FS_TILEB);
-        if constexpr (!PRE) {
-            const int64_t tl = t0n + lane;
-            fs_dma4(dnb + (tl < T ? tl : T - 1), den_lds + (n & 1) * 256);
-        }
+        if constexpr (!PRE) fs_dma16(ob + t0n * ld_out + so_o, dst + 4 * FS_TILEB);
+        const int64_t tl = t0n + lane;
+        fs_dma4(dnb + (tl < T ? tl : T - 1), den_lds + (n % NSLOT) * 256);
     };
     issue(0);
     if (nch > 1) issue(1);
-    if (nch > 1) fs_wait<PRE ? 5 : 6>(); else fs_wait<0>();
+    if (NSLOT == 3 && nch > 2) issue(2);
+    if (NSLOT == 3 && nch > 2) fs_wait<2 * NPART>(); else if (nch > 1) fs_wait<NPART>(); else fs_wait<0>();
     __builtin_amdgcn_s_barrier();
     asm volatile("" ::: "memory");
     float* PVw = PV + w * 96;
@@ -800,12 +815,11 @@
     FSD_BEGIN
     for (int n = 0; n < nch; ++n) {
         const int64_t t0 = (int64_t)(nch - 1 - n) * FS_C;
-        const char* Xq = RING + (n & 1) * FS_SLOTB;
+        const char* Xq = RING + (n % NSLOT) * SLOTB;
         const char* Xk = Xq + FS_TILEB;
         const char* Xv = Xq + 2 * FS_TILEB;
         const char* Xg = Xq + 3 * FS_TILEB;
-        const char* Xo = Xq + 4 * FS_TILEB;
-        const float* dens = (const float*)(DEN + (n & 1) * 256);
+        const float* dens = (const float*)(DEN + (n % NSLOT) * 256);
         {
             bf16x8 x[4][2];
 #pragma unroll
@@ -831,41 +845,49 @@
         bf16x8 gA[2][2];
         uint32_t rp[2][2];
         {
-            const uint32_t slot = ring_lds + (n & 1) * FS_SLOTB;
+            const uint32_t slot = ring_lds + (n % NSLOT) * SLOTB;
 #pragma unroll
             for (int s_ = 0; s_ < 2; ++s_)
 #pragma unroll
                 for (int h_ = 0; h_ < 2; ++h_) rp[s_][h_] = rpl[s_][h_] + slot;
         }
-        bf16x8 dfr[2][2], ofr[2][2], vB1[2][2];
-#pragma unroll
-        for (int tt = 0; tt < 2; ++tt)
-#pragma unroll
-            for (int s_ = 0; s_ < 2; ++s_) { dfr[tt][s_] = fs_rp_asm(rp, 3, 16 * tt, s_); ofr[tt][s_] = fs_rp_asm(rp, 4, 16 * tt, s_); }
-#pragma unroll
-        for (int jt = 0; jt < 2; ++jt)
-#pragma unroll
-            for (int s_ = 0; s_ < 2; ++s_) vB1[jt][s_] = fs_rp_asm(rp, 2, 16 * jt, s_);
-        fs_pin<16>(dfr[0][0], ofr[0][0], dfr[0][1], ofr[0][1]);
-        fs_pin<8>(dfr[1][0], ofr[1][0], dfr[1][1], ofr[1][1]);
-#pragma unroll
-        for (int tt = 0; tt < 2; ++tt) {
-            const bf16x8 d0 = dfr[tt][0], d1 = dfr[tt][1];
-            const bf16x8 o0 = ofr[tt][0], o1 = ofr[tt][1];
-            f32x4 gm = mma32(o0, d0, zero4());
-            gm = mma32(o1, d1, gm);
-            const float dot = fs_diag_sum_rows(gm, g, c);
-            if constexpr (PRE) {
-                if (g == 0) PVw[16 * tt + c] = -dot;
-                gA[tt][0] = d0;
-                gA[tt][1] = d1;
-            } else {
+        bf16x8 vB1[2][2];
+        if constexpr (PRE) {
+#pragma unroll
+            for (int tt = 0; tt < 2; ++tt)
+#pragma unroll
+                for (int s_ = 0; s_ < 2; ++s_) gA[tt][s_] = fs_rp_asm(rp, 3, 16 * tt, s_);
+#pragma unroll
+            for (int jt = 0; jt < 2; ++jt)
+#pragma unroll
+                for (int s_ = 0; s_ < 2; ++s_) vB1[jt][s_] = fs_rp_asm(rp, 2, 16 * jt, s_);
+            fs_pin<8>(gA[0][0], gA[0][1], gA[1][0], gA[1][1]);
+        } else {
+            bf16x8 dfr[2][2], ofr[2][2];
+#pragma unroll
+            for (int tt = 0; tt < 2; ++tt)
+#pragma unroll
+                for (int s_ = 0; s_ < 2; ++s_) { dfr[tt][s_] = fs_rp_asm(rp, 3, 16 * tt, s_); ofr[tt][s_] = fs_rp_asm(rp, 4, 16 * tt, s_); }
+#pragma unroll
+            for (int jt = 0; jt < 2; ++jt)
+#pragma unroll
+                for (int s_ = 0; s_ < 2; ++s_) vB1[jt][s_] = fs_rp_asm(rp, 2, 16 * jt, s_);
+            fs_pin<16>(dfr[0][0], ofr[0][0], dfr[0][1], ofr[0][1]);
+            fs_pin<8>(dfr[1][0], ofr[1][0], dfr[1][1], ofr[1][1]);
+#pragma unroll
+            for (int tt = 0; tt < 2; ++tt) {
+                const bf16x8 d0 = dfr[tt][0], d1 = dfr[tt][1];
+                const bf16x8 o0 = ofr[tt][0], o1 = ofr[tt][1];
+                f32x4 gm = mma32(o0, d0, zero4());
+                gm = mma32(o1, d1, gm);
+                const float dot = fs_diag_sum_rows(gm, g, c);
                 const float inv = 1.f / dens[16 * tt + c];
                 if (g == 0) { PVw[16 * tt + c] = -dot * inv; PVw[32 + 16 * tt + c] = -dot; PVw[64 + 16 * tt + c] = inv; }
                 gA[tt][0] = fs_scale8(d0, inv);
                 gA[tt][1] = fs_scale8(d1, inv);
             }
         }
+        const float* ddrow = PRE ? dens : PVw;
         FSD(1);
         bf16x8 pb[2];
         {
@@ -875,7 +897,7 @@
             p00 = mma32(gA[0][1], vB[0][1], p00);
             p10 = mma32(gA[1][1], vB[0][1], p10);
             p11 = mma32(gA[1][1], vB[1][1], p11);
-            const f32x4 dd0 = *(const f32x4*)(PVw + 4 * g), dd1 = *(const f32x4*)(PVw + 16 + 4 * g);
+            const f32x4 dd0 = *(const f32x4*)(ddrow + 4 * g), dd1 = *(const f32x4*)(ddrow + 16 + 4 * g);
 #pragma unroll
             for (int r = 0; r < 4; ++r) {
                 const bool keep = (4 * g + r) >= c;
@@ -1008,7 +1030,7 @@
             RT[dl][1] = mma32(gT, qfTs[1], RT[dl][1]);
         }
         {
-            const f32x4 nd0 = *(const f32x4*)(PVw + (PRE ? 0 : 32) + 4 * g), nd1 = *(const f32x4*)(PVw + (PRE ? 0 : 32) + 16 + 4 * g);
+            const f32x4 nd0 = *(const f32x4*)(ddrow + (PRE ? 0 : 32) + 4 * g), nd1 = *(const f32x4*)(ddrow + (PRE ? 0 : 32) + 16 + 4 * g);
             bf16x8 ndop = pack8(nd0, nd1);
 #pragma unroll
             for (int e = 0; e < 8; ++e) ndop[e] = c == 0 ? ndop[e] : (bf16_t)0.f;
@@ -1018,7 +1040,7 @@
 #pragma unroll
         for (int ft = 0; ft < 8; ++ft) RD[ft] = mma32(load_perm_tr(QF, FS_LDF, 16 * ft, 0, lane), gTs, RD[ft]);
         FSD(7);
-        fs_wait<0>();
+        if (NSLOT == 3 && n + 2 < nch) fs_wait<NPART>(); else fs_wait<0>();
         FSD(8);
         if (n > 0) {
             const int64_t tp = t0 + FS_C;
@@ -1029,7 +1051,7 @@
         for (int jt = 0; jt < 2; ++jt) *(bf16x4*)(dvb + (t0 + 16 * jt + c) * ld_d + 16 * w + 4 * g) = dv_prev[jt];
         fs_barrier();
         FSD(9);
-        if (n + 2 < nch) issue(n + 2);
+        if (n + NSLOT < nch) issue(n + NSLOT);
         FSD(10);
 #pragma unroll
         for (int jt = 0; jt < 2; ++jt) {
@@ -1049,9 +1071,10 @@
 }
 }
 
+static_assert(FsDkvRing<true>::LDS <= 80 * 1024 && FsDkvRing<false>::LDS <= 80 * 1024, "dk / dv: two workgroups must share a CU's 160 KB of LDS");
 int emo_favor_fs_try(int which, int stage, const bf16_t* q, const bf16_t* k, const bf16_t* v, int64_t ld, const float* omega, bf16_t* out, int64_t ld_out,
                      float* den, float* sS, float* sz, const bf16_t* dout, bf16_t* dq, bf16_t* dk, bf16_t* dv, int64_t ld_d, int64_t B, int64_t T, int64_t H,
-                     float eps, const float* ws_S, const float* ws_z, int P, int64_t Ts, hipStream_t st) {
+                     float eps, const float* ws_S, const float* ws_z, int P, int64_t Ts, float* dd_ws, hipStream_t st) {
     const char* e = getenv("EMO_FAVOR_FS");
     if (e && atoi(e) == 0) return 0;
     if (T < FS_C || (T % FS_C) != 0 || B * H <= 0 || P < 1 || (P > 1 && (Ts % FS_C) != 0)) return 0;
@@ -1069,6 +1092,7 @@
     const char* e2 = getenv("EMO_FAVOR_FS_BWD");
     if (e2 && atoi(e2) == 0) return 0;
     const bool pre = den == nullptr;
+    if (pre && (stage != 0 || P != 1 || dd_ws == nullptr || ((uintptr_t)dd_ws & 3))) return 0;
     if (stage == 0 || stage == 1) {
         const size_t lds = (size_t)3 * FS_SLOTB + 3 * 256 + 4 * 2048 + 2 * FS_TILEB + 2 * 4 * 32 * sizeof(float);
         static bool attr = false;
@@ -1079,25 +1103,25 @@
         }
         if (pre)
             hipLaunchKernelGGL(favor_fs_dq_kernel<true>, grid, dim3(FS_NT), lds, st, q, k, v, ld, omega, (const bf16_t*)out, dout, ld_out, (const float*)nullptr, dq, ld_d, T, H,
-                               ws_S, ws_z, P, Ts);
+                               ws_S, ws_z, P, Ts, dd_ws);
         else
             hipLaunchKernelGGL(favor_fs_dq_kernel<false>, grid, dim3(FS_NT), lds, st, q, k, v, ld, omega, (const bf16_t*)out, dout, ld_out, (const float*)den, dq, ld_d, T, H,
-                               ws_S, ws_z, P, Ts);
+                               ws_S, ws_z, P, Ts, (float*)nullptr);
     }
     if (stage == 0 || stage == 2) {
-        const size_t lds2 = (size_t)2 * FS_SLOTB + 2 * 256 + sizeof(bf16_t) * (size_t)(2 * FS_C * FS_LDF) + FS_TILEB + sizeof(float) * (128 + 4 * 96);
+        const size_t lds2 = pre ? FsDkvRing<true>::LDS : FsDkvRing<false>::LDS;
         static bool attr2 = false;
         if (!attr2) {
-            (void)hipFuncSetAttribute((const void*)favor_fs_dkv_kernel<false>, hipFuncAttributeMaxDynamicSharedMemorySize, (int)lds2);
-            (void)hipFuncSetAttribute((const void*)favor_fs_dkv_kernel<true>, hipFuncAttributeMaxDynamicSharedMemorySize, (int)lds2);
+            (void)hipFuncSetAttribute((const void*)favor_fs_dkv_kernel<false>, hipFuncAttributeMaxDynamicSharedMemorySize, (int)FsDkvRing<false>::LDS);
+            (void)hipFuncSetAttribute((const void*)favor_fs_dkv_kernel<true>, hipFuncAttributeMaxDynamicSharedMemorySize, (int)FsDkvRing<true>::LDS);
             attr2 = true;
         }
         if (pre)
             hipLaunchKernelGGL(favor_fs_dkv_kernel<true>, grid, dim3(FS_NT), lds2, st, q, k, v, ld, omega, (const bf16_t*)out, dout, ld_out, (const float*)nullptr, dk, dv, ld_d, T, H,
-                               ws_S, ws_z, P, Ts);
+                               ws_S, ws_z, P, Ts, (const float*)dd_ws);
         else
             hipLaunchKernelGGL(favor_fs_dkv_kernel<false>, grid, dim3(FS_NT), lds2, st, q, k, v, ld, omega, (const bf16_t*)out, dout, ld_out, (const float*)den, dk, dv, ld_d, T, H,
-                               ws_S, ws_z, P, Ts);
+                               ws_S, ws_z, P, Ts, (const float*)nullptr);
     }
     return 1;
 }
diff --git a/emo-disentanger_amd/ops.py b/emo-disentanger_amd/ops.py
--- a/emo-disentanger_amd/ops.py
+++ b/emo-disentanger_amd/ops.py
@@ -277,9 +277,11 @@
         dqkv = torch.empty(M, 3 * HD, device=q.device, dtype=q.dtype)
     dq, dk, dv = dqkv[:, :HD], dqkv[:, HD:2 * HD], dqkv[:, 2 * HD:]
     if dn:
+        ws_bytes = lib.emo_favor_attn_bwd_dn_workspace_bytes(B, T, H)
+        ws = torch.empty(ws_bytes, device=q.device, dtype=torch.uint8)
         with _timed('favor_bwd', 0.0, 7.0 * M * HD * q.element_size()):
             check(lib.emo_favor_attn_bwd_dn(ptr(q), ptr(k), ptr(v), _rows(q), ptr(omega), ptr(out), ptr(dout), HD, ptr(dq), ptr(dk), ptr(dv), 3 * HD,
-                                            dtype_code(q.dtype), B, T, H, dh, n_feat, eps, stream()))
+                                            dtype_code(q.dtype), B, T, H, dh, n_feat, eps, ptr(ws), ws_bytes, stream()))
         return dq, dk, dv
     if ws_saved is not None:
         ws, ws_bytes, kvalid = ws_saved, ws_saved.numel(), 1
diff --git a/include/emo_hip.h b/include/emo_hip.h
--- a/include/emo_hip.h
+++ b/include/emo_hip.h
@@ -107,10 +107,11 @@
                               int64_t dh, int64_t n_feat, float eps, void* workspace, int64_t workspace_bytes,
                               int kstate_valid, emo_stream_t stream);
 int emo_favor_attn_bwd_dn_supported(int dtype, int64_t B, int64_t T, int64_t H, int64_t dh, int64_t n_feat);
+int64_t emo_favor_attn_bwd_dn_workspace_bytes(int64_t B, int64_t T, int64_t H);
 int emo_favor_attn_bwd_dn(const void* q, const void* k, const void* v, int64_t ld, const float* omega,
                           const void* out, const void* dn, int64_t ld_out, void* dq, void* dk, void* dv,
                           int64_t ld_d, int dtype, int64_t B, int64_t T, int64_t H, int64_t dh, int64_t n_feat,
-                          float eps, emo_stream_t stream);
+                          float eps, void* workspace, int64_t workspace_bytes, emo_stream_t stream);
 int emo_favor_decode_step(const void* q, const void* k, const void* v, int64_t ld, const float* omega,
                           float* state_S, float* state_z, void* out, int64_t ld_out, int dtype,
                           int64_t n_streams, int64_t H, int64_t dh, int64_t n_feat, float eps,
```
